# ChenWu98/cycle-diffusion

Measured on AMD Instinct MI355X. Metric: images/sec, SD-v1.4 512px CycleDiffusion 100+100 steps, 1/2/4/8 MI355X, higher is better.
Workload: dtype fp16; 1 GPU; C2: Stable-Diffusion-v1.4-shaped U-Net + KL-f8 VAE, 512x512, custom_steps=99 white_box_steps=100 eta=0.1 skip 0, 1 trial, encoder scale 1, decoder CFG 3; batch_per_gpu=4, global_batch=4, parallelism=dp1, steps_per_launch_set=5, launch_set_cap=16, launch_sets_in_flight_per_gpu=1, images_in_flight_per_gpu=20, distributed=single process, weights=synthetic(seed=0)

## Files before the change

cycle-diffusion_amd/_ffi.py:

```python
import ctypes as C
import os

import numpy as np

_HERE = os.path.dirname(os.path.abspath(__file__))
LIB_PATH = os.path.join(_HERE, "lib", "libcyclediff.so")

CD_NET_UNET_OPENAI, CD_NET_UNET_HO, CD_NET_VAE_KL, CD_NET_CLIP_TEXT, CD_NET_BERT_XTR = 1, 2, 3, 4, 5
CD_NET_OCLIP_TEXT, CD_NET_OCLIP_VISION, CD_NET_INCEPTION_FID = 6, 7, 8
CD_SCHED_DDIM, CD_SCHED_DDPM = 0, 1
CD_PREC_16, CD_PREC_F32, CD_PREC_F32X3 = 0, 1, 2
CD_MASK_QSAMPLE, CD_MASK_ENCODER = 0, 1
MASK_SOURCES = {"q_sample": CD_MASK_QSAMPLE, "encoder": CD_MASK_ENCODER}
ACT_NONE, ACT_SILU, ACT_GELU, ACT_GEGLU, ACT_QGELU, ACT_RELU = 0, 1, 2, 3, 4, 5


class NetDesc(C.Structure):
    _fields_ = [
        ("kind", C.c_int), ("image_size", C.c_int), ("in_channels", C.c_int), ("out_channels", C.c_int),
        ("model_channels", C.c_int), ("num_res_blocks", C.c_int),
        ("n_mult", C.c_int), ("channel_mult", C.c_int * 8),
        ("n_attn", C.c_int), ("attn", C.c_int * 8),
        ("num_heads", C.c_int), ("num_head_channels", C.c_int),
        ("use_spatial_transformer", C.c_int), ("context_dim", C.c_int), ("transformer_depth", C.c_int),
        ("use_scale_shift_norm", C.c_int), ("resblock_updown", C.c_int), ("conv_resample", C.c_int),
        ("z_channels", C.c_int), ("embed_dim", C.c_int), ("double_z", C.c_int),
        ("precision", C.c_int), ("n_embed", C.c_int), ("reserved", C.c_int * 6),
    ]


class StepCoef(C.Structure):
    _fields_ = [("sa", C.c_float), ("s1a", C.c_float), ("sap", C.c_float), ("dirc", C.c_float),
                ("sigma", C.c_float), ("r", C.c_float), ("t_mask", C.c_float), ("t", C.c_int32)]


STEP_COEF_DTYPE = np.dtype([("sa", "<f4"), ("s1a", "<f4"), ("sap", "<f4"), ("dirc", "<f4"), ("sigma", "<f4"),
                            ("r", "<f4"), ("t_mask", "<f4"), ("t", "<i4")])

_VP, _I, _F, _U64, _SZ, _I64 = C.c_void_p, C.c_int, C.c_float, C.c_uint64, C.c_size_t, C.c_int64

SIGNATURES = {
    "cd_last_error": [],
    "cd_version": [],
    "cd_act_format": [],
    "cd_engine_create": [_VP, _SZ, C.POINTER(_VP)],
    "cd_engine_destroy": [_VP],
    "cd_engine_synchronize": [_VP],
    "cd_engine_workspace_high_water": [_VP, C.POINTER(_SZ)],
    "cd_prof_enable": [_VP, _I],
    "cd_prof_collect": [_VP, C.POINTER(_I), C.POINTER(C.c_double), C.POINTER(C.c_double)],
    "cd_net_create": [_VP, C.POINTER(NetDesc), C.POINTER(_I)],
    "cd_net_param_count": [_VP, _I, C.POINTER(_I)],
    "cd_net_param_info": [_VP, _I, _I, C.c_char_p, _I, C.POINTER(_I), C.POINTER(_I64)],
    "cd_net_load_param": [_VP, _I, C.c_char_p, _VP, _I, C.POINTER(_I64)],
    "cd_net_missing_params": [_VP, _I, C.POINTER(_I), C.c_char_p, _I],
    "cd_unet_forward": [_VP, _I, _VP, _VP, _VP, _I, _I, _VP],
    "cd_text_encode": [_VP, _I, _VP, _I, _I, _VP],
    "cd_clip_text_features": [_VP, _I, _VP, _I, _I, _VP],
    "cd_clip_image_features": [_VP, _I, _VP, _I, _VP],
    "cd_inception_features": [_VP, _I, _VP, _I, _I, _VP],
    "cd_vae_encode": [_VP, _I, _VP, _VP, _U64, _I, _I, _I, _F, _VP],
    "cd_vae_decode": [_VP, _I, _VP, _I, _I, _F, _F, _F, _VP],
    "cd_dpm_encode": [_VP, _I, _I, _VP, _VP, _VP, _I, _F, _I, _I, _VP, _VP, _U64, _I, _VP],
    "cd_ddim_decode": [_VP, _I, _I, _VP, _I, _I, _VP, _VP, _I, _F, _I, _I, _VP, _VP, _U64, _VP],
    "cd_ddim_decode_v": [_VP, _I, _I, _VP, _I, _I, _VP, _VP, _I, _VP, _I, _I, _VP, _VP, _U64, _VP],
    "cd_ddim_invert": [_VP, _I, _I, _VP, _VP, _VP, _I, _F, _I, _I, _VP, _VP, _VP],
    "cd_cycle_translate": [_VP, _I, _I, _VP, _VP, _VP, _F, _VP, _VP, _F, _VP, _I, _I, _I, _I, _VP, _VP, _VP, _U64, _I, _VP,
                           _VP],
    "cd_ddim_decode_masked": [_VP, _I, _I, _VP, _I, _I, _VP, _VP, _I, _F, _VP, _I, _I, _VP, _VP, _U64, _VP, _VP, _I, _I, _VP, _VP,
                              _U64, _VP],
    "cd_cycle_translate_masked": [_VP, _I, _I, _VP, _VP, _VP, _F, _VP, _VP, _F, _VP, _I, _I, _I, _I, _VP, _VP, _VP, _U64, _I,
                                  _VP, _VP, _I, _I, _VP, _VP, _U64, _VP, _VP],
    "cd_cycle_translate_ctrl": [_VP, _I, _I, _VP, _VP, _VP, _F, _VP, _VP, _F, _VP, _I, _I, _I, _I, _VP, _VP, _VP, _U64, _I,
                                _VP, _VP, _I, _I, _VP, _VP, _U64, _VP, _VP, _VP, _I, _I, _VP, _VP],
    "cd_ilvr_decode": [_VP, _I, _I, _VP, _I, _I, _I, _I, _VP, _VP, _U64, _VP, _I, _I, _I, _VP, _VP, _U64, _VP],
    "cd_pix_refine": [_VP, _I, _I, _VP, _I, _I, _VP, _VP, _U64],
    "cd_op_pack_conv_weight": [_VP, _VP, _I, _I, _I, _I, _I, C.POINTER(_VP), C.POINTER(_I), C.POINTER(_I)],
    "cd_op_free": [_VP, _VP],
    "cd_op_conv2d": [_VP, _VP, _I, _VP, _I, _I, _I, _I, _VP, _I, _I, _I, _I, _I, _I, _I, _VP, _VP, _VP, _I, _I, _VP],
    "cd_op_conv2d_16": [_VP, _VP, _I, _VP, _I, _I, _I, _I, _VP, _I, _I, _I, _I, _I, _I, _I, _VP, _VP, _VP, _I, _I, _VP,
                        _VP],
    "cd_op_last_gemm_config": [_VP] + [C.POINTER(_I)] * 5,
    "cd_op_up_phase_reorder": [_VP, _VP, _I, _I, _I, _I, _VP],
    "cd_op_groupnorm": [_VP, _VP, _I, _I, _I, _I, _I, _F, _VP, _VP, _VP, _I, _VP],
    "cd_op_groupnorm_ex": [_VP, _VP, _I, _I, _VP, _I, _I, _I, _I, _I, _F, _VP, _VP, _VP, _I, _I, _VP, _VP, _I, _VP],
    "cd_op_layernorm": [_VP, _VP, _I, _I, _VP, _VP, _F, _VP],
    "cd_op_attention": [_VP, _VP, _VP, _VP, _I, _I, _I, _I, _I, _F, _I, _VP],
    "cd_op_cross_attention_ctrl": [_VP, _VP, _VP, _VP, _VP, _VP, _VP, _VP, _VP, _I, _I, _I, _I, _I, _I, _I, _I, _F, _VP],
    "cd_op_lowpass": [_VP, _VP, _I, _I, _I, _I, _VP],
    "cd_op_softmax_rows": [_VP, _VP, _I64, _I, _VP],
    "cd_op_timestep_embedding": [_VP, _VP, _I, _I, _I, _VP],
    "cd_op_sched_step": [_VP, _I, _I, _VP, _VP, _VP, _VP, _I, _F, _VP, _VP, _I, _I, _I, _I, _VP],
    "cd_op_sched_step_masked": [_VP, _I, _VP, _VP, _VP, _I, _F, _VP, _VP, _VP, _I, _I, _F, _F, _VP, _I, _I, _I, _I, _VP, _I],
    "cd_op_bench_conv": [_VP, _I, _I, _I, _I, _I, _I, _I, _I, _I, _I, _I, _I, C.POINTER(C.c_float)],
    "cd_op_bench_mfma_sustained": [_VP, _I, C.POINTER(C.c_float), C.POINTER(C.c_float)],
    "cd_op_probe": [_VP, _I, _VP, _VP, _SZ],
}
_RESTYPES = {"cd_last_error": C.c_char_p}

_lib = None


class EngineError(RuntimeError):
    pass


def load_library(build_if_missing=True):
    global _lib
    if _lib is not None:
        return _lib
    if not os.path.exists(LIB_PATH):
        if not build_if_missing:
            raise EngineError("libcyclediff.so has not been built: run `python -c 'import __graft_entry__ as g; g.build()'`")
        import importlib.util
        spec = importlib.util.spec_from_file_location("_cd_build", os.path.join(_HERE, "build.py"))
        mod = importlib.util.module_from_spec(spec)
        spec.loader.exec_module(mod)
        mod.build()
    os.environ.setdefault("CYCLEDIFF_TUNE_DEFAULT", os.path.join(_HERE, "tune_gfx950.txt"))
    lib = C.CDLL(os.environ.get("CYCLEDIFF_LIB") or LIB_PATH)
    for name, args in SIGNATURES.items():
        fn = getattr(lib, name)
        fn.argtypes = args
        fn.restype = _RESTYPES.get(name, C.c_int)
    _lib = lib
    return lib


def check(rc):
    if rc != 0:
        raise EngineError(load_library().cd_last_error().decode("utf-8", "replace"))


def ptr(t):
    if t is None:
        return None
    if not t.is_contiguous():
        raise EngineError("tensor crossing the C ABI must be contiguous")
    return C.c_void_p(t.data_ptr())


def coef_array(rows):
    arr = np.zeros(len(rows), dtype=STEP_COEF_DTYPE)
    for i, r in enumerate(rows):
        arr[i] = tuple(r)
    return arr
```

cycle-diffusion_amd/csrc/capi.hip:

```cpp
#include <stdlib.h>
#include <string.h>
#include <unistd.h>

#include <algorithm>

#include "engine.h"

using namespace cd;

struct StepPacer {
  static constexpr int kAhead = 2, kRing = kAhead + 1;
  hipEvent_t ev[kRing] = {nullptr, nullptr, nullptr};
  long n = 0;
  bool enabled = true;
  void init() {
    const char* e = getenv("CYCLEDIFF_HOST_PACING");
    enabled = !(e && e[0] == '0');
    for (auto& x : ev) HIP_CHECK(hipEventCreateWithFlags(&x, hipEventBlockingSync | hipEventDisableTiming));
  }
  static void sleep_until_done(hipEvent_t e) {
    for (;;) {
      const hipError_t q = hipEventQuery(e);
      if (q == hipSuccess) return;
      if (q != hipErrorNotReady) HIP_CHECK(q);
// ... 957 lines not shown
    const int r = R / down_n;
    iv.xp = iv.out = s.xt;
    iv.y = ref; iv.y_bmod = B_ref;
    iv.qtab = (const float2*)upload_table(h, qsample_coef_host, (size_t)K * 2 * sizeof(float));
    iv.gauss.seed = ref_seed;
    iv.B = B; iv.C = s.C; iv.R = R;
    iv.D = upload_taps(h, R, r);
    iv.U = upload_taps(h, r, R);
    iv.T = (float*)h->arena.alloc((size_t)B * s.C * r * r * sizeof(float));
    iv.xin = a.xin;
    iv.vec4 = (R % 4 == 0 && aligned16(ref) && aligned16(ref_noise)) ? 1 : 0;
  }
  HIP_CHECK(hipMemcpy2DAsync(s.xt, chw * 4, z, zbs * 4, chw * 4, B, hipMemcpyDeviceToDevice, h->st));
  if (!s.f32) launch_nchw_to_nhwc(h->st, s.xt, s.xin, B, s.C, s.HW, s.cpad, 1.f, 0.f, 0);
  for (int i = 0; i < K; ++i) {
    const int k = K - 1 - i;
    run_unet(h, s, k);
    const float* eps = (i < n_eps) ? z + (int64_t)(1 + i) * chw : nullptr;
    const float* nz = (!eps && noise_tail) ? noise_tail + (int64_t)(i - n_eps) * n : nullptr;
    a.geom.step = k; a.eps.p = eps;
    a.gauss.noise = nz; a.gauss.stream = (uint32_t)(0x1000 + i);
    launch_decode_step(h->st, sched_kind, a);
    if (k > range_t) {
      iv.qrow = k;
      iv.gauss.noise = ref_noise ? ref_noise + (int64_t)i * n : nullptr;
      iv.gauss.stream = (uint32_t)(0x5000 + i);
      launch_ilvr_down(h->st, iv);
      launch_ilvr_up_add(h->st, iv);
    }
    h->pacer.tick(h->st);
  }
  HIP_CHECK(hipMemcpyAsync(x_out, s.xt, (size_t)n * 4, hipMemcpyDeviceToDevice, h->st));
  CD_API_END
}

int cd_op_pack_conv_weight(cd_handle h, const float* w_host, int N, int Cin, int KH, int KW, int geglu,
                           void** packed_dev, int* Npad, int* Cpad) {
  CD_API_BEGIN
  enter_engine(h);
  CD_CHECK(h && w_host && packed_dev, "bad argument");
  static int counter = 0;
  ConvW* c = h->op_params.new_conv(N, Cin, KH, KW, false, geglu != 0);
  const std::string name = "op." + std::to_string(counter++);
  h->op_params.conv_weight(name, c);
  int64_t shape[4] = {N, Cin, KH, KW};
  h->op_params.load(h->st, name, w_host, 4, shape);
  *packed_dev = c;
  if (Npad) *Npad = c->Npad;
  if (Cpad) *Cpad = c->Cpad;
  CD_API_END
}

int cd_op_free(cd_handle, void*) { return 0; }

static void op_conv2d(cd_handle h, const float* x0, int C0, const float* x1, int C1, int B, int H, int W,
                      const void* packed_w, int N, int KH, int KW, int stride, int pad, int asym_pad, int up,
                      const float* bias, const float* rowvec, const float* resid, int act, int tile, bool out16,
                      float* y, float* stats) {
  CD_CHECK(h && x0 && packed_w && y, "bad argument");
  ArenaScope arena_scope(h->arena);
  Ctx c = h->ctx();
  if (up && out16) {
    ConvW* pw = (ConvW*)const_cast<void*>(packed_w);
    h->op_params.add_up_phase(pw);
    h->op_params.refresh_up_phase(h->st, pw);
  }
  ConvW w = *(const ConvW*)packed_w;
  CD_CHECK(w.N == N && w.KH == KH && w.KW == KW, "packed weight does not match the call");
  w.b = const_cast<float*>(bias);
  const int c0p = x1 ? C0 : round_up(C0, 32);
  Act a0 = alloc_act(c, B, H, W, c0p);
  launch_nchw_to_nhwc(h->st, x0, a0.p, B, C0, H * W, c0p, 1.f, 0.f, 0);
  Act a1;
  if (x1) {
    a1 = alloc_act(c, B, H, W, C1);
    launch_nchw_to_nhwc(h->st, x1, a1.p, B, C1, H * W, C1, 1.f, 0.f, 0);
  }
  ConvOpts o; o.stride = stride; o.pad = pad; o.asym = asym_pad != 0; o.up = up != 0; o.tile = tile;
  if (act & 0x400) {
    CD_CHECK(out16 && conv_ln_fold_available(c, w, (int64_t)B * H * W) , "LayerNorm fold needs tile 30 shapes");
    o.ln_fold = true;
    act &= ~0x400;
  }
  o.act = act;
  o.out_f32 = !out16;
  o.want_stats = stats != nullptr;
  const int Hin = up ? 2 * H : H, Win = up ? 2 * W : W;
  const int Ho = asym_pad ? (Hin + 1 - KH) / stride + 1 : (Hin + 2 * pad - KH) / stride + 1;
  const int Wo = asym_pad ? (Win + 1 - KW) / stride + 1 : (Win + 2 * pad - KW) / stride + 1;
  const int Nout = w.geglu ? N / 2 : N;
  if (rowvec) { o.rowvec = rowvec; o.rowvec_ld = N; o.rows_per_vec = Ho * Wo; }
  Act r;
  if (resid) {
    r = alloc_act(c, B, Ho, Wo, Nout);
    launch_nchw_to_nhwc(h->st, resid, r.p, B, Nout, Ho * Wo, Nout, 1.f, 0.f, 0);
    o.resid = &r;
  }
  Act out = conv_fwd(c, w, a0, x1 ? &a1 : nullptr, o);
  launch_nhwc_to_nchw(h->st, out.p, out16 ? 0 : 1, out.ld, y, B, Nout, Ho * Wo, 1.f, 0.f);
  if (stats) {
    CD_CHECK(out.stats, "this convolution produces no GroupNorm statistics (GEGLU, or rows %% 32 != 0)");
    HIP_CHECK(hipMemcpyAsync(stats, out.stats, (size_t)(out.rows() / 32) * 2 * Nout * sizeof(float),
                             hipMemcpyDeviceToDevice, h->st));
  }
}

int cd_op_conv2d(cd_handle h, const float* x0, int C0, const float* x1, int C1, int B, int H, int W,
                 const void* packed_w, int N, int KH, int KW, int stride, int pad, int asym_pad, int up,
                 const float* bias, const float* rowvec, const float* resid, int act, int tile, float* y) {
  CD_API_BEGIN
  enter_engine(h);
  op_conv2d(h, x0, C0, x1, C1, B, H, W, packed_w, N, KH, KW, stride, pad, asym_pad, up, bias, rowvec, resid, act, tile,
            false, y, nullptr);
  CD_API_END
}

int cd_op_conv2d_16(cd_handle h, const float* x0, int C0, const float* x1, int C1, int B, int H, int W,
                    const void* packed_w, int N, int KH, int KW, int stride, int pad, int asym_pad, int up,
                    const float* bias, const float* rowvec, const float* resid, int act, int tile, float* y,
                    float* stats) {
  CD_API_BEGIN
  enter_engine(h);
  op_conv2d(h, x0, C0, x1, C1, B, H, W, packed_w, N, KH, KW, stride, pad, asym_pad, up, bias, rowvec, resid, act, tile,
            true, y, stats);
  CD_API_END
}

int cd_op_up_phase_reorder(cd_handle h, const float* x, int B, int C, int H, int W, float* y) {
  CD_API_BEGIN
  enter_engine(h);
  CD_CHECK(h && x && y && B > 0 && H > 0 && W > 0 && C > 0 && C % 8 == 0, "bad argument");
  ArenaScope arena_scope(h->arena);
  Ctx c = h->ctx();
  Act a = alloc_act(c, 4 * B, H, W, C);
  launch_nchw_to_nhwc(h->st, x, a.p, 4 * B, C, H * W, C, 1.f, 0.f, 0);
  Act o = alloc_act(c, B, 2 * H, 2 * W, C);
  launch_up_phase_reorder(h->st, a.p, o.p, B, H, W, C, o.ld);
  launch_nhwc_to_nchw(h->st, o.p, 0, o.ld, y, B, C, 4 * H * W, 1.f, 0.f);
  CD_API_END
}

int cd_op_last_gemm_config(cd_handle h, int* tile_id, int* bk, int* splitk, int* chm, int* tile_group) {
  CD_API_BEGIN
  CD_CHECK(h, "bad argument");
  const GemmLaunchInfo li = conv_gemm_last_launch();
  if (tile_id) *tile_id = li.tile_id;
  if (bk) *bk = li.bk;
  if (splitk) *splitk = li.splitk;
  if (chm) *chm = li.chm;
  if (tile_group) *tile_group = li.tile_group;
  CD_API_END
}

int cd_op_groupnorm(cd_handle h, const float* x, int B, int C, int H, int W, int G, float eps,
                    const float* gamma, const float* beta, const float* film, int silu, float* y) {
  CD_API_BEGIN
  enter_engine(h);
  CD_CHECK(h && x && y && G == 32, "bad argument (G must be 32)");
  ArenaScope arena_scope(h->arena);
  Ctx c = h->ctx();
  Act a = alloc_act(c, B, H, W, C);
  launch_nchw_to_nhwc(h->st, x, a.p, B, C, H * W, C, 1.f, 0.f, 0);
  GNW w; w.g = const_cast<float*>(gamma); w.b = const_cast<float*>(beta); w.C = C; w.eps = eps;
  Act o = groupnorm_fwd(c, w, a, nullptr, silu != 0, film, film ? 2 * C : 0);
  launch_nhwc_to_nchw(h->st, o.p, 0, o.ld, y, B, C, H * W, 1.f, 0.f);
  CD_API_END
}

int cd_op_groupnorm_ex(cd_handle h, const float* x0, int C0, int pad0, const float* x1, int C1, int pad1, int B, int H,
                       int W, float eps, const float* gamma, const float* beta, const float* film, int film_ld, int silu,
                       const float* stats0, const float* stats1, int precision, void* y) {
  CD_API_BEGIN
  enter_engine(h);
  CD_CHECK(h && x0 && gamma && beta && y && B > 0 && H > 0 && W > 0 && C0 > 0 && pad0 >= 0 && pad1 >= 0, "bad argument");
  CD_CHECK(x1 ? C1 > 0 : (C1 == 0 && !stats1), "bad argument (second source)");
  CD_CHECK(precision >= 0 && precision <= 2 && film_ld >= 0, "bad argument (precision 0 = 16-bit, 1 = fp32, 2 = fp32 split)");
  const int align = precision ? 4 : 8;
  CD_CHECK((C0 + pad0) % align == 0 && (C1 + pad1) % align == 0, "row strides must be multiples of %d elements", align);
  ArenaScope arena_scope(h->arena);
  Ctx c = h->ctx();
  c.f32 = precision != 0; c.x3 = precision == 2;
  const int HW = H * W, C = C0 + C1;
  auto upload = [&](const float* x, int Cs, int pad, const float* stats) {
    Act a; a.B = B; a.H = H; a.W = W; a.C = Cs; a.ld = Cs + pad; a.f32 = c.f32;
    a.p = (bf16_t*)h->arena.alloc((size_t)B * HW * a.ld * (c.f32 ? sizeof(float) : sizeof(bf16_t)));
    const float* src = x;
    if (pad) {
      const size_t n = (size_t)B * a.ld * HW;
      float* t = (float*)h->arena.alloc(n * sizeof(float));
      launch_fill_f32(h->st, t, __builtin_nanf(""), (int64_t)n);
      HIP_CHECK(hipMemcpy2DAsync(t, (size_t)a.ld * HW * 4, x, (size_t)Cs * HW * 4, (size_t)Cs * HW * 4, B,
                                 hipMemcpyDeviceToDevice, h->st));
      src = t;
    }
    if (c.f32) launch_nchw_to_nhwc_f32(h->st, src, a.pf(), B, a.ld, HW, a.ld, 1.f, 0.f);
    else launch_nchw_to_nhwc(h->st, src, a.p, B, a.ld, HW, a.ld, 1.f, 0.f, 0);
    a.stats = const_cast<float*>(stats);
    return a;
  };
  Act a0 = upload(x0, C0, pad0, stats0);
  Act a1;
  if (x1) a1 = upload(x1, C1, pad1, stats1);
  GNW w; w.g = const_cast<float*>(gamma); w.b = const_cast<float*>(beta); w.C = C; w.eps = eps;
  Act o = groupnorm_fwd(c, w, a0, x1 ? &a1 : nullptr, silu != 0, film, film_ld);
  if (precision == 2) {
    CD_CHECK(o.split && o.ld == 2 * C, "groupnorm: split output expected");
    HIP_CHECK(hipMemcpyAsync(y, o.p, (size_t)B * HW * 2 * C * sizeof(bf16_t), hipMemcpyDeviceToDevice, h->st));
    HIP_CHECK(hipStreamSynchronize(h->st));
    h->check_overflow();
  } else {
    launch_nhwc_to_nchw(h->st, o.p, c.f32 ? 1 : 0, o.ld, (float*)y, B, C, HW, 1.f, 0.f);
  }
  CD_API_END
}

int cd_op_layernorm(cd_handle h, const float* x, int rows, int C, const float* gamma, const float* beta,
                    float eps, float* y) {
  CD_API_BEGIN
  enter_engine(h);
  CD_CHECK(h && x && y, "bad argument");
  ArenaScope arena_scope(h->arena);
  bf16_t* a = (bf16_t*)h->arena.alloc((size_t)rows * C * 2);
  bf16_t* o = (bf16_t*)h->arena.alloc((size_t)rows * C * 2);
  launch_nchw_to_nhwc(h->st, x, a, rows, C, 1, C, 1.f, 0.f, 0);
  launch_layernorm(h->st, a, C, o, C, rows, C, gamma, beta, eps);
  launch_nhwc_to_nchw(h->st, o, 0, C, y, rows, C, 1, 1.f, 0.f);
  CD_API_END
}

int cd_op_attention(cd_handle h, const float* q, const float* k, const float* v, int B, int H, int Tq,
                    int Tk, int D, float scale, int use_transpose_kernel, float* o) {
  CD_API_BEGIN
  enter_engine(h);
  CD_CHECK(h && q && k && v && o, "bad argument");
  ArenaScope arena_scope(h->arena);
  const int C = H * D, Tpad = round_up(Tk, 64);
  bf16_t* qb = (bf16_t*)h->arena.alloc((size_t)B * Tq * C * 2);
  bf16_t* kb = (bf16_t*)h->arena.alloc((size_t)B * Tk * C * 2);
  bf16_t* vb = (bf16_t*)h->arena.alloc((size_t)B * Tk * C * 2);
  bf16_t* ob = (bf16_t*)h->arena.alloc((size_t)B * Tq * C * 2);
  launch_nchw_to_nhwc(h->st, q, qb, B * Tq, C, 1, C, 1.f, 0.f, 0);
  launch_nchw_to_nhwc(h->st, k, kb, B * Tk, C, 1, C, 1.f, 0.f, 0);
  launch_nchw_to_nhwc(h->st, v, vb, B * Tk, C, 1, C, 1.f, 0.f, 0);
  AttnParams p;
  p.q = qb; p.k = kb; p.o = ob; p.B = B; p.H = H; p.Tq = Tq; p.Tk = Tk; p.D = D;
  p.ldq = C; p.ldk = C; p.ldo = C; p.q_bs = (int64_t)Tq * C; p.k_bs = (int64_t)Tk * C; p.o_bs = (int64_t)Tq * C;
  p.scale = scale;
  if (use_transpose_kernel) {
    bf16_t* vt = (bf16_t*)h->arena.alloc((size_t)B * C * Tpad * 2);
    launch_transpose_v(h->st, vb, C, (int64_t)Tk * C, vt, B, H, Tk, D, D, Tpad);
    p.vt = vt; p.vt_dpad = D; p.vt_tpad = Tpad;
  } else {
    p.v = vb; p.ldv = C; p.v_bs = (int64_t)Tk * C;
  }
  launch_attention(h->st, p);
  launch_nhwc_to_nchw(h->st, ob, 0, C, o, B * Tq, C, 1, 1.f, 0.f);
  CD_API_END
}

int cd_op_cross_attention_ctrl(cd_handle h, const float* q_own, const float* q_src, const float* k_own, const float* k_src,
                               const float* v_own, const float* mapper, const float* alpha, const float* weight, int B,
                               int B_src, int B_ctrl, int H, int Tq, int L, int L_buf, int D, float scale, float* o) {
  CD_API_BEGIN
  enter_engine(h);
  CD_CHECK(h && q_own && q_src && k_own && k_src && v_own && mapper && alpha && weight && o, "bad argument");
  CD_CHECK(B > 0 && B_src > 0 && B_ctrl > 0 && H > 0 && Tq > 0 && D > 0 && L > 0 && L_buf >= L, "bad argument");
  ArenaScope arena_scope(h->arena);
  const int C = H * D;
  auto to16 = [&](const float* src, int64_t rows) {
    bf16_t* d = (bf16_t*)h->arena.alloc((size_t)rows * C * 2);
    launch_nchw_to_nhwc(h->st, src, d, (int)rows, C, 1, C, 1.f, 0.f, 0);
    return d;
  };
  CtrlAttnParams p;
  p.q_own = to16(q_own, (int64_t)B * Tq); p.q_src = to16(q_src, (int64_t)B_src * Tq);
  p.k_own = to16(k_own, (int64_t)B * L_buf); p.k_src = to16(k_src, (int64_t)B_src * L_buf);
  const bf16_t* vb16 = to16(v_own, (int64_t)B * L);
  bf16_t* va = (bf16_t*)h->arena.alloc((size_t)B * L * C * 2);
  bf16_t* vb = (bf16_t*)h->arena.alloc((size_t)B * L * C * 2);
  launch_ctrl_values(h->st, vb16, mapper, alpha, weight, B, B_ctrl, L, C, va, vb);
  bf16_t* ob = (bf16_t*)h->arena.alloc((size_t)B * Tq * C * 2);
  p.va = va; p.vb = vb; p.o = ob;
  p.B = B; p.B_src = B_src; p.H = H; p.Tq = Tq; p.L = L; p.D = D;
  p.ldq = C; p.ldk = C; p.ldv = C; p.ldo = C;
  p.q_bs = (int64_t)Tq * C; p.k_bs = (int64_t)L_buf * C; p.v_bs = (int64_t)L * C; p.o_bs = (int64_t)Tq * C;
  p.scale = scale;
  launch_cross_attention_ctrl(h->st, p);
  launch_nhwc_to_nchw(h->st, ob, 0, C, o, B * Tq, C, 1, 1.f, 0.f);
  CD_API_END
}

int cd_op_lowpass(cd_handle h, const float* x, int B, int C, int R, int down_n, float* y) {
  CD_API_BEGIN
  enter_engine(h);
  CD_CHECK(h && x && y && B > 0 && C > 0 && R > 0, "bad argument");
  check_lowpass_geometry(R, down_n);
  ArenaScope arena_scope(h->arena);
  const int r = R / down_n;
  IlvrArgs iv;
  iv.out = y; iv.y = x; iv.y_bmod = B;
  iv.B = B; iv.C = C; iv.R = R;
  iv.D = upload_taps(h, R, r);
  iv.U = upload_taps(h, r, R);
  iv.T = (float*)h->arena.alloc((size_t)B * C * r * r * sizeof(float));
  iv.vec4 = (R % 4 == 0 && aligned16(x) && aligned16(y)) ? 1 : 0;
  launch_ilvr_down(h->st, iv);
// ... 255 lines not shown
```

cycle-diffusion_amd/csrc/conv_gemm.hip:

```cpp
#include <stdio.h>
#include <stdlib.h>
#include <string.h>

#include <algorithm>
#include <map>
#include <mutex>
#include <string>

#include "common.h"
#include "kernels.h"

namespace cd {

namespace gemm_detail {

#ifndef CD_EPI_STORE_AUX
#define CD_EPI_STORE_AUX 0
#endif
#ifndef CD_EPI_RESID_AUX
#define CD_EPI_RESID_AUX 0
#endif

typedef const __attribute__((address_space(1))) void* gptr_t;
typedef __attribute__((address_space(3))) void* lptr_t;

template <int BM, int BN, int BK, int WM, int WN, int NSTAGE>
struct TileCfg {
  static constexpr int NW = WM * WN;
  static constexpr int CPR = BK / 8;
  static constexpr int RPI = 64 / CPR;
  static constexpr int A_IPW = BM / RPI / NW;
  static constexpr int B_IPW = BN / RPI / NW;
  static constexpr int LPT = A_IPW + B_IPW;
  static constexpr int TM = BM / WM, TN = BN / WN;
  static constexpr int MT = TM / 32, NT = TN / 32;
  static constexpr int KS = BK / 16;
  static constexpr int SWZ_SHIFT = (CPR == 8) ? 1 : 2;
  static constexpr int CW = TN >= 64 ? 64 : TN;
  static constexpr int EPI_LD = CW + 4;
  static constexpr int PF = (MT * NT >= 8) ? 1 : 2;
  static constexpr int A_BYTES = BM * BK * 2, B_BYTES = BN * BK * 2;
  static constexpr int STAGE_BYTES = A_BYTES + B_BYTES;
  static constexpr int EPI_BYTES = NW * TM * EPI_LD * 4;
  static constexpr int LDS_BYTES = STAGE_BYTES * NSTAGE > EPI_BYTES ? STAGE_BYTES * NSTAGE : EPI_BYTES;
  static constexpr int TAB_BIAS_I = (BN / 4 + 63) / 64;
  static constexpr int TAB_RV_I = ((BM / 32) * (BN / 4) + 63) / 64;
  static constexpr bool HAS_TAB = LDS_BYTES + (TAB_BIAS_I + TAB_RV_I) * 1024 <= 160 * 1024;
  static constexpr int TAB_BYTES = HAS_TAB ? (TAB_BIAS_I + TAB_RV_I) * 1024 : 0;
  static_assert(NW == 4 || NW == 8 || NW == 16, "4, 8 or 16 waves");
  static_assert(A_IPW >= 1 && B_IPW >= 1, "tile too small for the wave count");
  static_assert(A_IPW * RPI * NW == BM && B_IPW * RPI * NW == BN, "tile rows must split evenly over waves");
  static_assert(MT >= 1 && NT >= 1, "wave tile");
  static_assert(NSTAGE >= 2 && NSTAGE <= 8, "ring depth");
  static_assert((NSTAGE - 2) * LPT <= 63, "vmcnt field");
  static_assert(LDS_BYTES + TAB_BYTES <= 160 * 1024, "LDS");
};

template <int N>
__device__ __forceinline__ void wait_vmcnt_barrier() {
  asm volatile("s_waitcnt vmcnt(%0)\n\ts_barrier" ::"n"(N) : "memory");
}

#ifdef CD_PROBE
__device__ __forceinline__ unsigned long long probe_time() {
  unsigned long long t;
  asm volatile("s_memtime %0\n\ts_waitcnt lgkmcnt(0)" : "=s"(t)::"memory");
  return t;
}
__device__ __forceinline__ unsigned long long probe_realtime() {
  unsigned long long t;
  asm volatile("s_memrealtime %0\n\ts_waitcnt lgkmcnt(0)" : "=s"(t)::"memory");
  return t;
}
#define CD_PROBE_ONLY(...) __VA_ARGS__
#else
#define CD_PROBE_ONLY(...)
#endif

__device__ __forceinline__ __amdgpu_buffer_rsrc_t uniform_rsrc(const void* base, int bytes) {
  const uint64_t u = (uint64_t)base;
  const uint32_t lo = (uint32_t)__builtin_amdgcn_readfirstlane((int)(uint32_t)u);
  const uint32_t hi = (uint32_t)__builtin_amdgcn_readfirstlane((int)(uint32_t)(u >> 32));
  return __builtin_amdgcn_make_buffer_rsrc((void*)(((uint64_t)hi << 32) | lo), 0, __builtin_amdgcn_readfirstlane(bytes), 0x00020000);
}

__device__ __forceinline__ bool fast_epilogue(const ConvGemmParams& p) {
  return p.act == ACT_NONE && !p.out_f32 && !p.resid_f32 && (p.N & 7) == 0 && (p.out_ld & 7) == 0 &&
         (((uintptr_t)p.out | (uintptr_t)p.resid | (uintptr_t)p.rowvec) & 15) == 0 && (p.o_bs & 7) == 0 &&
         (!p.resid || (p.resid_ld & 7) == 0) &&
         (!p.rowvec || ((p.rowvec_ld & 3) == 0 && (p.rows_per_vec >= p.M || (p.rows_per_vec & 31) == 0)));
}

template <int BM, int BN, int BK, int WM, int WN, int NSTAGE, bool CHM = false>
__global__ __launch_bounds__(64 * WM * WN, (WM * WN == 4 && BK == 32 && NSTAGE == 3 && BM * BN >= 128 * 256) ? 2 : 1) void k_conv_gemm(ConvGemmParams p) {
#if defined(__HIP_DEVICE_COMPILE__)
  using T = TileCfg<BM, BN, BK, WM, WN, NSTAGE>;
  constexpr int CPR = T::CPR, RPI = T::RPI, A_IPW = T::A_IPW, B_IPW = T::B_IPW, NW = T::NW;
  constexpr int MT = T::MT, NT = T::NT, KS = T::KS, TM = T::TM, TN = T::TN, LPT = T::LPT;
  extern __shared__ __attribute__((aligned(16))) char smem[];

  const int tid = threadIdx.x;
  const int lane = tid & 63;
  const int wave = __builtin_amdgcn_readfirstlane(tid >> 6);
  const int wm = wave / WN, wn = wave % WN;
  if constexpr (WM * WN == 4 && BK == 32 && NSTAGE == 3 && BM * BN >= 128 * 256) {
    if (p.dephase_ticks > 0 && (int)(blockIdx.x + gridDim.x * (blockIdx.y + gridDim.y * blockIdx.z)) < 2 * p.num_cus) {
      unsigned hwid;
      asm volatile("s_getreg_b32 %0, hwreg(HW_REG_HW_ID)" : "=s"(hwid));
      if (tid == 0) *(volatile int*)smem = (int)(hwid & 1u);
      __syncthreads();
      const int odd = *(volatile int*)smem;
      __syncthreads();
      if (odd) {
        unsigned long long t0, t1;
        asm volatile("s_memtime %0\n\ts_waitcnt lgkmcnt(0)" : "=s"(t0)::"memory");
        do {
          __builtin_amdgcn_s_sleep(32);
          asm volatile("s_memtime %0\n\ts_waitcnt lgkmcnt(0)" : "=s"(t1)::"memory");
        } while ((long long)(t1 - t0) < (long long)p.dephase_ticks);
      }
    }
  }
  CD_PROBE_ONLY(
  const unsigned long long pr_rt0 = probe_realtime();
  unsigned long long pr_t0 = probe_time(), pr_prol = 0, pr_first = 0, pr_wait = 0, pr_comp = 0, pr_maxw = 0, pr_loop = 0,
                     pr_drain = 0, pr_stage = 0, pr_rows = 0, pr_issued = 0, pr_last = 0;
  unsigned* pr_log = (unsigned*)(smem + T::LDS_BYTES + T::TAB_BYTES) + wave * 64;
  if (lane < 64) pr_log[lane] = 0;)

  const int tiles_n = (p.N + BN - 1) / BN;
  const int tiles_m = (p.M + BM - 1) / BM;
  const int ntiles = tiles_m * tiles_n;
  int tile;
  {
    const int bid = blockIdx.x;
    const int q = ntiles >> 3, r = ntiles & 7;
    const int xcd = bid & 7, loc = bid >> 3;
    tile = (xcd < r ? xcd * (q + 1) : r * (q + 1) + (xcd - r) * q) + loc;
  }
  const bool nmajor = (int64_t)p.N * p.Ktot > (int64_t)p.B * p.Hs * p.Ws * (p.C0 + p.C1);
  int tm, tn;
  if (p.tile_group > 0) {
    const int width = p.tile_group * tiles_n;
    const int grp = tile / width, within = tile - grp * width;
    const int first_m = grp * p.tile_group;
    const int gsz = (tiles_m - first_m) < p.tile_group ? (tiles_m - first_m) : p.tile_group;
    tn = within / gsz; tm = first_m + (within - tn * gsz);
  } else if (nmajor) { tn = tile / tiles_m; tm = tile - tn * tiles_m; }
  else { tm = tile / tiles_n; tn = tile - tm * tiles_n; }
  const int m0 = tm * BM, n0 = tn * BN;
  const int zb = blockIdx.z;

  constexpr unsigned kRange = 0x7fffffffu, kInvalid = 0x80000000u;
  const int HWo = p.Hout * p.Wout;
  const bool pow2 = ((HWo & (HWo - 1)) == 0) && ((p.Wout & (p.Wout - 1)) == 0);
  const int sh_hw = 31 - __builtin_clz(HWo), sh_w = 31 - __builtin_clz(p.Wout);
  int b_first = pow2 ? (m0 >> sh_hw) : (m0 / HWo);
  CD_PROBE_ONLY(if (p.dbg & 4) b_first = 0;)
  int pad_t = p.pad_t, pad_l = p.pad_l, w_ph = 0;
  if (p.up_phase) {
    const int ph = b_first & 3;
    b_first >>= 2;
    pad_t = 1 - (ph >> 1); pad_l = 1 - (ph & 1);
    w_ph = ph * p.w_ps;
  }
  const int64_t samp0 = (int64_t)b_first * p.Hs * p.Ws;
  const bf16_t* base0 = p.src0 + (int64_t)zb * p.a_bs + samp0 * p.ld0;
  const bf16_t* base1 = p.src1 ? p.src1 + (int64_t)zb * p.a_bs + samp0 * p.ld1 : base0;
  const __amdgpu_buffer_rsrc_t rsw =
      __builtin_amdgcn_make_buffer_rsrc((void*)(p.wgt + (int64_t)zb * p.w_bs + w_ph), 0, kRange, 0x00020000);

  const int srow = lane / CPR;
  const int pchunk = lane % CPR;
  int a_iy0[A_IPW], a_ix0[A_IPW], a_boff[A_IPW], a_lc8[A_IPW];
  unsigned a_voff[A_IPW];
  unsigned a_mk[A_IPW], a_base[A_IPW];
#pragma unroll
  for (int i = 0; i < A_IPW; ++i) {
    const int row = (i * NW + wave) * RPI + srow;
    int m = m0 + row;
    CD_PROBE_ONLY(if (p.dbg & 4) m = (m0 & 0x3ff) + row;)
    a_lc8[i] = (pchunk ^ ((row >> T::SWZ_SHIFT) & (CPR - 1))) * 8;
    a_voff[i] = kInvalid;
    a_mk[i] = 0; a_base[i] = 0;
    if (m < p.M) {
      int b, oy, ox;
      if (pow2) {
        b = m >> sh_hw;
        const int rem = m & (HWo - 1);
        oy = rem >> sh_w; ox = rem & (p.Wout - 1);
      } else {
        b = m / HWo;
        const int rem = m - b * HWo;
        oy = rem / p.Wout; ox = rem - oy * p.Wout;
      }
      if (p.up_phase) b >>= 2;
      a_iy0[i] = oy * p.stride - pad_t;
      a_ix0[i] = ox * p.stride - pad_l;
      a_boff[i] = (b - b_first) * p.Hs * p.Ws;
    } else {
      a_iy0[i] = -(1 << 28);
      a_ix0[i] = 0;
      a_boff[i] = 0;
    }
    if constexpr (CHM) {
      unsigned mk = 0;
      for (int r = 0; r < p.KH; ++r) mk |= ((unsigned)(a_iy0[i] + r) < (unsigned)p.Hin ? 1u : 0u) << r;
      for (int q = 0; q < p.KW; ++q) mk |= ((unsigned)(a_ix0[i] + q) < (unsigned)p.Win ? 1u : 0u) << (8 + q);
      a_mk[i] = mk;
    }
  }
  unsigned b_voff[B_IPW];
#pragma unroll
  for (int i = 0; i < B_IPW; ++i) {
    const int row = (i * NW + wave) * RPI + srow;
    const int lchunk = pchunk ^ ((row >> T::SWZ_SHIFT) & (CPR - 1));
    int nrow = n0 + row;
    if (nrow >= p.N) nrow = p.N - 1;
    b_voff[i] = (unsigned)((nrow * (p.ldw ? p.ldw : p.Ktot) + lchunk * 8) * 2);
  }

  const int Ctot = p.C0 + p.C1;
  const int nk = p.Ktot / BK;
  const int nsplit = gridDim.y, sidx = blockIdx.y;
  const int kper = (nk + nsplit - 1) / nsplit;
  const int kt0 = sidx * kper;
  const int kt1 = (kt0 + kper < nk) ? kt0 + kper : nk;
  int kr, kss, kc;
  if constexpr (CHM) {
    const int ntaps = p.KH * p.KW;
    const int slice = kt0 / ntaps, tap = kt0 - slice * ntaps;
    kc = slice * BK;
    kr = tap / p.KW;
    kss = tap - kr * p.KW;
  } else {
    const int k_el = kt0 * BK;
    const int tap = k_el / Ctot;
    kc = k_el - tap * Ctot;
    kr = tap / p.KW;
    kss = tap - kr * p.KW;
  }
  bool st_force = true;

  char* As = smem;
  char* Bs = smem + NSTAGE * T::A_BYTES;

  bool st_live = false;
  int st_soffa = 0, st_soffb = 0;
  const bf16_t* st_base = base0;
  auto prepare = [&](int kt) {
    st_live = kt < kt1;
    const int c_kc = kc, c_kr = kr, c_kss = kss;
    if constexpr (CHM) {
      const bool wk = c_kss + 1 >= p.KW;
      const bool wr = wk && (c_kr + 1 >= p.KH);
      kss = wk ? 0 : c_kss + 1;
      kr = wr ? 0 : c_kr + (wk ? 1 : 0);
      kc = c_kc + (wr ? BK : 0);
      if (st_live) {
        const int ld = (c_kc < p.C0) ? p.ld0 : p.ld1;
        if (st_force || ((c_kr | c_kss) == 0 && (c_kc == 0 || c_kc == p.C0))) {
          st_force = false;
#pragma unroll
          for (int i = 0; i < A_IPW; ++i) {
            const int pix = a_boff[i] + a_iy0[i] * p.Ws + a_ix0[i];
            a_base[i] = (unsigned)((pix * ld + a_lc8[i]) * 2);
          }
        }
        const unsigned dt = (unsigned)((c_kr * p.Ws + c_kss) * ld * 2);
#pragma unroll
        for (int i = 0; i < A_IPW; ++i) {
          const unsigned ok = (a_mk[i] >> c_kr) & (a_mk[i] >> (8 + c_kss)) & 1u;
          a_voff[i] = ok ? a_base[i] + dt : kInvalid;
        }
      }
    } else {
      kc += BK;
      if (kc >= Ctot) {
        kc = 0;
        if (++kss >= p.KW) { kss = 0; ++kr; }
      }
      if (st_live && (c_kc == 0 || c_kc == p.C0 || st_force)) {
        st_force = false;
        const int ld = (c_kc < p.C0) ? p.ld0 : p.ld1;
#pragma unroll
        for (int i = 0; i < A_IPW; ++i) {
          int iy = a_iy0[i] + c_kr, ix = a_ix0[i] + c_kss;
          const bool ok = ((unsigned)iy < (unsigned)p.Hin) && ((unsigned)ix < (unsigned)p.Win);
          if (p.up) { iy >>= 1; ix >>= 1; }
          const int pix = a_boff[i] + iy * p.Ws + ix;
          a_voff[i] = ok ? (unsigned)((pix * ld + a_lc8[i]) * 2) : kInvalid;
        }
      }
    }
    const bool first = c_kc < p.C0;
    st_base = first ? base0 : base1;
    st_soffa = (first ? c_kc : c_kc - p.C0) * 2;
    st_soffb = st_live ? (CHM ? ((c_kr * p.KW + c_kss) * Ctot + c_kc) * 2 : kt * (BK * 2)) : 0;
  };
  auto issue = [&](int idx, int buf) {
    if (idx < A_IPW) {
      const __amdgpu_buffer_rsrc_t rsa = __builtin_amdgcn_make_buffer_rsrc((void*)st_base, 0, kRange, 0x00020000);
      char* l = As + buf * T::A_BYTES + ((idx * NW + wave) * RPI) * (BK * 2);
      __builtin_amdgcn_raw_ptr_buffer_load_lds(rsa, (lptr_t)l, 16, st_live ? a_voff[idx < A_IPW ? idx : 0] : kInvalid,
                                               st_soffa, 0, 0);
    } else {
      const int i = idx - A_IPW;
      char* l = Bs + buf * T::B_BYTES + ((i * NW + wave) * RPI) * (BK * 2);
      __builtin_amdgcn_raw_ptr_buffer_load_lds(rsw, (lptr_t)l, 16, st_live ? b_voff[i < B_IPW ? i : 0] : kInvalid,
                                               st_soffb, 0, 0);
    }
  };

  f32x16 acc[MT][NT];
#pragma unroll
  for (int i = 0; i < MT; ++i)
#pragma unroll
    for (int j = 0; j < NT; ++j)
#pragma unroll
      for (int r = 0; r < 16; ++r) acc[i][j][r] = 0.0f;

  const int frow = lane & 31;
  const int fhalf = lane >> 5;

  constexpr int PF = T::PF, SYNC = KS - PF, NMF = MT * NT, HALF = NMF / 2;
  constexpr int SPREAD = (NSTAGE == 2) ? 1 : KS;
  static_assert(SYNC >= 0 && (NSTAGE - 1) * LPT <= 63, "fragment prefetch depth / vmcnt field");
#pragma unroll
  for (int s = 0; s < NSTAGE; ++s) {
    prepare(kt0 + s);
#pragma unroll
    for (int l = 0; l < LPT; ++l) issue(l, s);
  }
  constexpr int TAB_N = T::TAB_BIAS_I + T::TAB_RV_I;
  constexpr int TABI = T::HAS_TAB ? (TAB_N + NW - 1) / NW : 0;
  if constexpr (TABI > 0) {
    const bool fe = fast_epilogue(p);
    const bool tb = (fe || p.act == ACT_GEGLU) && p.bias != nullptr;
    char* tab = smem + T::LDS_BYTES;
    const __amdgpu_buffer_rsrc_t rsb = __builtin_amdgcn_make_buffer_rsrc(
        (void*)(tb ? (const void*)p.bias : (const void*)p.wgt), 0, tb ? p.N * 4 : 0, 0x00020000);
    const __amdgpu_buffer_rsrc_t rsv = __builtin_amdgcn_make_buffer_rsrc(
        (void*)((fe && p.rowvec) ? (const void*)p.rowvec : (const void*)p.wgt), 0, (fe && p.rowvec) ? kRange : 0, 0x00020000);
    const unsigned rpv = (unsigned)p.rows_per_vec;
    const bool rpv_pow2 = (rpv & (rpv - 1)) == 0;
    const int rpv_sh = 31 - __builtin_clz(rpv | 1u);
#pragma unroll
    for (int i = 0; i < TABI; ++i) {
      const int j = (i * NW + wave) % TAB_N;
// ... 3 lines not shown
      } else {
        const int c = (j - T::TAB_BIAS_I) * 64 + lane;
        const int blk = c / (BN / 4), c4 = c - blk * (BN / 4);
        const int m = m0 + blk * 32, nn = n0 + c4 * 4;
        int rvi = 0;
        if (p.rows_per_vec < p.M) rvi = rpv_pow2 ? (int)((unsigned)m >> rpv_sh) : m / p.rows_per_vec;
        const unsigned vo = (m < p.M && nn < p.N) ? (unsigned)((rvi * p.rowvec_ld + nn) * 4) : kInvalid;
        __builtin_amdgcn_raw_ptr_buffer_load_lds(rsv, (lptr_t)(tab + j * 1024), 16, vo, 0, 0, 0);
      }
    }
  }
  CD_PROBE_ONLY(pr_prol = probe_time(); pr_last = pr_prol;)
  static_assert((NSTAGE - 1) * LPT + TABI <= 63, "vmcnt field");
  wait_vmcnt_barrier<(NSTAGE - 1) * LPT + TABI>();
  CD_PROBE_ONLY(pr_first = probe_time(); pr_last = pr_first;)

  bf16x8 af[KS][MT], bfr[KS][NT];
  auto read_frags = [&](int slot, int ks) {
    const char* Ab = As + slot * T::A_BYTES;
    const char* Bb = Bs + slot * T::B_BYTES;
#pragma unroll
    for (int i = 0; i < MT; ++i) {
      const int row = wm * TM + i * 32 + frow;
      const int ch = (ks * 2 + fhalf) ^ ((row >> T::SWZ_SHIFT) & (CPR - 1));
      af[ks][i] = *(const bf16x8*)(Ab + row * (BK * 2) + ch * 16);
    }
#pragma unroll
    for (int j = 0; j < NT; ++j) {
      const int row = wn * TN + j * 32 + frow;
      const int ch = (ks * 2 + fhalf) ^ ((row >> T::SWZ_SHIFT) & (CPR - 1));
      bfr[ks][j] = *(const bf16x8*)(Bb + row * (BK * 2) + ch * 16);
    }
  };
#pragma unroll
  for (int q = 0; q < PF; ++q) read_frags(0, q);
  __builtin_amdgcn_sched_barrier(0);

  int cur = 0;
  int fill = 0;
  for (int kt = kt0; kt < kt1; ++kt) {
    const int nslot = (cur + 1 == NSTAGE) ? 0 : cur + 1;
#pragma unroll
    for (int ks = 0; ks < KS; ++ks) {
      const int jrel = (ks - SYNC + KS) % KS;
      auto mfma_range = [&](int lo, int hi) __attribute__((always_inline)) {
#pragma unroll
        for (int n = 0; n < NMF; ++n)
          if (n >= lo && n < hi) acc[n / NT][n % NT] = CD_MFMA_32x32x16(af[ks][n / NT], bfr[ks][n % NT], acc[n / NT][n % NT]);
      };
      if (ks == SYNC) {
        mfma_range(0, HALF);
        CD_PROBE_ONLY(const unsigned long long pr_arr = probe_time();)
        asm volatile("s_waitcnt vmcnt(%0) lgkmcnt(0)\n\ts_barrier" ::"n"((NSTAGE - 2) * LPT) : "memory");
        CD_PROBE_ONLY({
          const unsigned long long now = probe_time();
          pr_comp += pr_arr - pr_last; pr_wait += now - pr_arr; if (now - pr_arr > pr_maxw) pr_maxw = now - pr_arr;
          if (kt - kt0 < 32 && lane == 0) { pr_log[2 * (kt - kt0)] = (unsigned)(pr_arr - pr_t0); pr_log[2 * (kt - kt0) + 1] = (unsigned)(now - pr_t0); }
          pr_last = now;
        })
        prepare(kt + NSTAGE);
        fill = cur;
#pragma unroll
        for (int l = 0; l < LPT / SPREAD; ++l) issue(l, fill);
        mfma_range(HALF, NMF);
      } else {
        if (SPREAD > 1 && (ks > SYNC || kt != kt0)) {
#pragma unroll
          for (int l = (jrel * LPT) / SPREAD; l < ((jrel + 1) * LPT) / SPREAD; ++l) issue(l, fill);
        }
        mfma_range(0, NMF);
      }
      if (ks + PF < KS) read_frags(cur, ks + PF);
      else read_frags(nslot, ks + PF - KS);
      __builtin_amdgcn_sched_barrier(0);
    }
    cur = nslot;
  }
  CD_PROBE_ONLY(pr_loop = probe_time(); pr_comp += pr_loop - pr_last;)
  asm volatile("s_waitcnt vmcnt(0)" ::: "memory");
  __syncthreads();
  CD_PROBE_ONLY(pr_drain = probe_time();)

  if (nsplit > 1) {
    constexpr int TILE_BYTES = BM * BN * 4;
    constexpr int kSc1 = 16;
    typedef __attribute__((ext_vector_type(4))) unsigned int u32x4;
    float* part0 = p.sk_scratch + ((int64_t)zb * ntiles + tile) * nsplit * (BM * BN);
    const __amdgpu_buffer_rsrc_t rsp = __builtin_amdgcn_make_buffer_rsrc((void*)part0, 0, kRange, 0x00020000);
#pragma unroll
    for (int i = 0; i < MT; ++i)
#pragma unroll
      for (int j = 0; j < NT; ++j)
#pragma unroll
        for (int q = 0; q < 4; ++q) {
          const f32x4 v = {acc[i][j][4 * q], acc[i][j][4 * q + 1], acc[i][j][4 * q + 2], acc[i][j][4 * q + 3]};
          const int off = sidx * TILE_BYTES + (((i * NT + j) * 4 + q) * (64 * NW) + tid) * 16;
          __builtin_amdgcn_raw_buffer_store_b128(__builtin_bit_cast(u32x4, v), rsp, off, 0, kSc1);
        }
    asm volatile("s_waitcnt vmcnt(0)" ::: "memory");
    __syncthreads();
    int* flag = p.sk_flags + zb * ntiles + tile;
    if (tid == 0) *(volatile int*)smem = __hip_atomic_fetch_add(flag, 1, __ATOMIC_RELAXED, __HIP_MEMORY_SCOPE_AGENT);
    __syncthreads();
    const int arrived = *(volatile int*)smem;
    __syncthreads();
    if (arrived != nsplit - 1) return;
    if (tid == 0) __hip_atomic_store(flag, 0, __ATOMIC_RELAXED, __HIP_MEMORY_SCOPE_AGENT);
#pragma unroll
    for (int i = 0; i < MT; ++i)
#pragma unroll
      for (int j = 0; j < NT; ++j)
#pragma unroll
        for (int r = 0; r < 16; ++r) acc[i][j][r] = 0.0f;
    for (int sp = 0; sp < nsplit; ++sp) {
#pragma unroll
      for (int i = 0; i < MT; ++i)
#pragma unroll
        for (int j = 0; j < NT; ++j)
#pragma unroll
          for (int q = 0; q < 4; ++q) {
            const int off = sp * TILE_BYTES + (((i * NT + j) * 4 + q) * (64 * NW) + tid) * 16;
            const f32x4 v = __builtin_bit_cast(f32x4, __builtin_amdgcn_raw_buffer_load_b128(rsp, off, 0, kSc1));
            acc[i][j][4 * q] += v[0]; acc[i][j][4 * q + 1] += v[1];
            acc[i][j][4 * q + 2] += v[2]; acc[i][j][4 * q + 3] += v[3];
            if (q == 3 && MT * NT >= 8) __builtin_amdgcn_sched_barrier(0);
          }
    }
  }

  constexpr int CW = T::CW, CJ = CW / 32;
  int lane_ep = lane;
  asm volatile("" : "+v"(lane_ep));
  float* E = (float*)smem + wave * (TM * T::EPI_LD);
  const bool geglu = (p.act == ACT_GEGLU);
  char* outp = (char*)p.out + (int64_t)zb * p.o_bs * (p.out_f32 ? 4 : 2);
  if (p.alpha != 1.0f) {
#pragma unroll
    for (int i = 0; i < MT; ++i)
#pragma unroll
      for (int j = 0; j < NT; ++j)
#pragma unroll
        for (int r = 0; r < 16; ++r) acc[i][j][r] *= p.alpha;
  }
  if (T::HAS_TAB && fast_epilogue(p)) {
    constexpr int LD = T::EPI_LD, NRB = TM / 32;
    typedef __attribute__((ext_vector_type(4))) unsigned int u32x4e;
    const int mw = m0 + wm * TM;
    const bool has_res = p.resid != nullptr;
    int rows_ok = p.M - mw;
    rows_ok = rows_ok < 0 ? 0 : (rows_ok > TM ? TM : rows_ok);
    const int nblk = (p.M + 31) >> 5;
    int blk_ok = nblk - (mw >> 5);
    blk_ok = blk_ok < 0 ? 0 : (blk_ok > NRB ? NRB : blk_ok);
    const __amdgpu_buffer_rsrc_t rs_o = uniform_rsrc(outp + (int64_t)mw * p.out_ld * 2, rows_ok * p.out_ld * 2);
    const __amdgpu_buffer_rsrc_t rs_r =
        uniform_rsrc(has_res ? (const void*)(p.resid + (int64_t)zb * p.o_bs + (int64_t)mw * p.resid_ld) : (const void*)outp,
                     has_res ? rows_ok * p.resid_ld * 2 : 0);
    const __amdgpu_buffer_rsrc_t rs_s =
        uniform_rsrc(p.stats ? (const void*)(p.stats + ((int64_t)zb * nblk + (mw >> 5)) * 2 * p.N) : (const void*)outp,
                     p.stats ? blk_ok * 2 * p.N * 4 : 0);
    const float* TB = (const float*)(smem + T::LDS_BYTES) + wn * TN;
    const float* TR = (const float*)(smem + T::LDS_BYTES) + T::TAB_BIAS_I * 256 + (wm * NRB) * BN + wn * TN;
    constexpr bool PIPE = NW <= 8;
    u32x4e rq[PIPE ? 2 : 1][4];
    auto resid_issue = [&](int jcx, int rbx, u32x4e (&dst)[4]) __attribute__((always_inline)) {
      const int cwx = ((NT - jcx) < CJ ? (NT - jcx) : CJ) * 32, vprx = cwx / 8, rppx = 64 / vprx, npx = 32 / rppx;
      const int nx = n0 + wn * TN + jcx * 32 + (lane_ep % vprx) * 8;
      const unsigned vo = nx < p.N ? (unsigned)(((rbx * 32 + lane_ep / vprx) * p.resid_ld + nx) * 2) : kInvalid;
#pragma unroll
      for (int ps = 0; ps < 4; ++ps)
        if (ps < npx) dst[ps] = __builtin_amdgcn_raw_buffer_load_b128(rs_r, vo + (unsigned)(ps * rppx * p.resid_ld * 2), 0, CD_EPI_RESID_AUX);
    };
    if constexpr (PIPE) resid_issue(0, 0, rq[0]);
#pragma unroll
    for (int jc = 0; jc < NT; jc += CJ) {
      const int cj = (NT - jc) < CJ ? (NT - jc) : CJ;
      const int cw = cj * 32;
      const int RPP = 64 / (cw / 8), NP = 32 / RPP;
      const int vr = lane_ep / (cw / 8), col = (lane_ep % (cw / 8)) * 8;
      const int n = n0 + wn * TN + jc * 32 + col;
      CD_PROBE_ONLY(const unsigned long long pr_c0 = probe_time();)
      __builtin_amdgcn_wave_barrier();
#pragma unroll
      for (int i = 0; i < MT; ++i)
#pragma unroll
        for (int j = 0; j < CJ; ++j)
          if (j < cj) {
#pragma unroll
            for (int r = 0; r < 16; ++r) {
              const int row = i * 32 + (r & 3) + 8 * (r >> 2) + 4 * fhalf;
              E[row * LD + j * 32 + frow] = acc[i][jc + j][r];
            }
          }
      __builtin_amdgcn_wave_barrier();
      CD_PROBE_ONLY(const unsigned long long pr_c1 = probe_time(); pr_stage += pr_c1 - pr_c0;)
      const f32x4 b0 = *(const f32x4*)(TB + jc * 32 + col), b1 = *(const f32x4*)(TB + jc * 32 + col + 4);
      const unsigned vo_out = n < p.N ? (unsigned)((vr * p.out_ld + n) * 2) : kInvalid;
#pragma unroll
      for (int rb = 0; rb < NRB; ++rb) {
        const int kb = (jc / CJ) * NRB + rb;
        const int mb = mw + rb * 32;
        if constexpr (!PIPE) resid_issue(jc, rb, rq[0]);
        else if (rb + 1 < NRB) resid_issue(jc, rb + 1, rq[(kb + 1) & 1]);
        else if (jc + CJ < NT) resid_issue(jc + CJ, 0, rq[(kb + 1) & 1]);
        __builtin_amdgcn_sched_barrier(0);
        f32x4 lo[4], hi[4];
#pragma unroll
        for (int ps = 0; ps < 4; ++ps)
          if (ps < NP) {
            const float* er = E + (rb * 32 + ps * RPP + vr) * LD + col;
            lo[ps] = *(const f32x4*)er;
            hi[ps] = *(const f32x4*)(er + 4);
          }
        const f32x4 a0 = b0 + *(const f32x4*)(TR + rb * BN + jc * 32 + col);
        const f32x4 a1 = b1 + *(const f32x4*)(TR + rb * BN + jc * 32 + col + 4);
        constexpr bool KEEP = NW <= 8;
        float v[KEEP ? 4 : 1][8];
        float ssum[8], ssq[8];
#pragma unroll
        for (int e = 0; e < 8; ++e) { ssum[e] = 0.f; ssq[e] = 0.f; }
        const unsigned vo_blk = vo_out + (unsigned)(rb * 32 * p.out_ld * 2);
#pragma unroll
        for (int ps = 0; ps < 4; ++ps)
          if (ps < NP) {
            float* vp = v[KEEP ? ps : 0];
#pragma unroll
            for (int e = 0; e < 4; ++e) { vp[e] = lo[ps][e] + a0[e]; vp[4 + e] = hi[ps][e] + a1[e]; }
            if (has_res) {
              float rf[8];
              const u32x4e w = rq[PIPE ? (kb & 1) : 0][ps];
              unpack8(make_uint4(w[0], w[1], w[2], w[3]), rf);
#pragma unroll
              for (int e = 0; e < 8; ++e) vp[e] += rf[e];
            }
            const uint4 pk = pack8(vp);
            CD_PROBE_ONLY(if (!(p.dbg & 1)))
            __builtin_amdgcn_raw_buffer_store_b128((u32x4e){pk.x, pk.y, pk.z, pk.w}, rs_o,
                                                   vo_blk + (unsigned)(ps * RPP * p.out_ld * 2), 0, CD_EPI_STORE_AUX);
            if constexpr (!KEEP) {
              const float on = (mb + ps * RPP + vr) < p.M ? 1.0f : 0.0f;
#pragma unroll
              for (int e = 0; e < 8; ++e) { const float x = on * vp[e]; ssum[e] += x; ssq[e] += x * x; }
            }
          }
        float s_sum = 0.f, s_sq = 0.f;
        if (p.stats) {
          if constexpr (KEEP) {
            if (mb + 32 <= p.M) {
#pragma unroll
              for (int ps = 0; ps < 4; ++ps)
                if (ps < NP) {
#pragma unroll
                  for (int e = 0; e < 8; ++e) { ssum[e] += v[ps][e]; ssq[e] += v[ps][e] * v[ps][e]; }
                }
            } else {
#pragma unroll
              for (int ps = 0; ps < 4; ++ps)
                if (ps < NP) {
                  const float on = (mb + ps * RPP + vr) < p.M ? 1.0f : 0.0f;
#pragma unroll
                  for (int e = 0; e < 8; ++e) { const float x = on * v[ps][e]; ssum[e] += x; ssq[e] += x * x; }
                }
            }
          }
          float* S = E + rb * 32 * LD;
          __builtin_amdgcn_wave_barrier();
          *(f32x4*)(S + vr * cw + col) = (f32x4){ssum[0], ssum[1], ssum[2], ssum[3]};
          *(f32x4*)(S + vr * cw + col + 4) = (f32x4){ssum[4], ssum[5], ssum[6], ssum[7]};
          *(f32x4*)(S + 512 + vr * cw + col) = (f32x4){ssq[0], ssq[1], ssq[2], ssq[3]};
          *(f32x4*)(S + 512 + vr * cw + col + 4) = (f32x4){ssq[4], ssq[5], ssq[6], ssq[7]};
          __builtin_amdgcn_wave_barrier();
          if (cw == 64) {
#pragma unroll
            for (int k = 0; k < 8; ++k) { s_sum += S[k * 64 + lane_ep]; s_sq += S[512 + k * 64 + lane_ep]; }
          } else {
            const int arr = lane_ep >> 5, c = lane_ep & 31;
#pragma unroll
            for (int k = 0; k < 16; ++k) s_sum += S[arr * 512 + k * 32 + c];
          }
          __builtin_amdgcn_wave_barrier();
        }
        {
          const int nc0 = n0 + wn * TN + jc * 32;
          if (cw == 64) {
            const unsigned so = nc0 + lane_ep < p.N ? (unsigned)((rb * 2 * p.N + nc0 + lane_ep) * 4) : kInvalid;
            __builtin_amdgcn_raw_buffer_store_b32(__builtin_bit_cast(unsigned, s_sum), rs_s, so, 0, 0);
            __builtin_amdgcn_raw_buffer_store_b32(__builtin_bit_cast(unsigned, s_sq), rs_s, so + (unsigned)(p.N * 4), 0, 0);
          } else {
            const int arr = lane_ep >> 5, c = lane_ep & 31;
            const unsigned so = nc0 + c < p.N ? (unsigned)((rb * 2 * p.N + arr * p.N + nc0 + c) * 4) : kInvalid;
            __builtin_amdgcn_raw_buffer_store_b32(__builtin_bit_cast(unsigned, s_sum), rs_s, so, 0, 0);
          }
        }
      }
      CD_PROBE_ONLY(pr_rows += probe_time() - pr_c1;)
    }
  } else {
#pragma unroll
    for (int jc = 0; jc < NT; jc += CJ) {
      const int cj = (NT - jc) < CJ ? (NT - jc) : CJ;
      const int cw = cj * 32;
      CD_PROBE_ONLY(const unsigned long long pr_c0 = probe_time();)
      __builtin_amdgcn_wave_barrier();
#pragma unroll
      for (int i = 0; i < MT; ++i)
#pragma unroll
        for (int j = 0; j < CJ; ++j)
          if (j < cj) {
#pragma unroll
            for (int r = 0; r < 16; ++r) {
              const int row = i * 32 + (r & 3) + 8 * (r >> 2) + 4 * fhalf;
              E[row * T::EPI_LD + j * 32 + frow] = acc[i][jc + j][r];
            }
          }
      __builtin_amdgcn_wave_barrier();
      CD_PROBE_ONLY(const unsigned long long pr_c1 = probe_time(); pr_stage += pr_c1 - pr_c0;)
      const int vpr = geglu ? 4 : (cw / 8);
      const int rpp = 64 / vpr;
      int lane_g = lane_ep;
      asm volatile("" : "+v"(lane_g));
      const int vr = lane_g / vpr, vc = lane_g % vpr;
      const int col = vc * 8;
      const int n = n0 + wn * TN + jc * 32 + col;
      const int nvalid = (p.N - n) < 8 ? (p.N - n) : 8;
      if (geglu && cw == 64 && !p.out_f32 && !p.resid && !p.stats && !p.rowvec && (p.N & 63) == 0 && (p.out_ld & 7) == 0 &&
          (((uintptr_t)p.out) & 15) == 0 && (p.o_bs & 7) == 0) {
        constexpr int LD = T::EPI_LD;
        typedef __attribute__((ext_vector_type(4))) unsigned int u32x4e;
        float bias_v[8], bias_g[8];
        if constexpr (T::HAS_TAB) {
          const float* tb = (const float*)(smem + T::LDS_BYTES) + wn * TN + jc * 32 + col;
          const f32x4 x0 = *(const f32x4*)tb, x1 = *(const f32x4*)(tb + 4), g0 = *(const f32x4*)(tb + 32), g1 = *(const f32x4*)(tb + 36);
#pragma unroll
          for (int e = 0; e < 4; ++e) { bias_v[e] = x0[e]; bias_v[4 + e] = x1[e]; bias_g[e] = g0[e]; bias_g[4 + e] = g1[e]; }
        } else {
#pragma unroll
          for (int e = 0; e < 8; ++e) { bias_v[e] = p.bias ? p.bias[n + e] : 0.0f; bias_g[e] = p.bias ? p.bias[n + 32 + e] : 0.0f; }
        }
        const int mw = m0 + wm * TM;
        int rows_ok = p.M - mw;
        rows_ok = rows_ok < 0 ? 0 : (rows_ok > TM ? TM : rows_ok);
        const __amdgpu_buffer_rsrc_t rs_o = uniform_rsrc(outp + (int64_t)mw * p.out_ld * 2, rows_ok * p.out_ld * 2);
        const unsigned vo_out = n < p.N ? (unsigned)((vr * p.out_ld + (n / 64) * 32 + (n % 64)) * 2) : kInvalid;
#pragma unroll
        for (int rb = 0; rb < TM / 32; ++rb) {
          f32x4 vl[2], vh[2], gl[2], gh[2];
#pragma unroll
          for (int ps = 0; ps < 2; ++ps) {
            const float* er = E + (rb * 32 + ps * 16 + vr) * LD + col;
            vl[ps] = *(const f32x4*)er;        vh[ps] = *(const f32x4*)(er + 4);
            gl[ps] = *(const f32x4*)(er + 32); gh[ps] = *(const f32x4*)(er + 36);
          }
#pragma unroll
          for (int ps = 0; ps < 2; ++ps) {
            float v[8], va[8], ga[8];
#pragma unroll
            for (int e = 0; e < 4; ++e) {
              va[e] = vl[ps][e] + bias_v[e]; va[4 + e] = vh[ps][e] + bias_v[4 + e];
              ga[e] = gl[ps][e] + bias_g[e]; ga[4 + e] = gh[ps][e] + bias_g[4 + e];
            }
            mul_gelu8(va, ga, v);
            const uint4 pk = pack8(v);
            CD_PROBE_ONLY(if (!(p.dbg & 1)))
            __builtin_amdgcn_raw_buffer_store_b128((u32x4e){pk.x, pk.y, pk.z, pk.w}, rs_o,
                                                   vo_out + (unsigned)((rb * 32 + ps * 16) * p.out_ld * 2), 0, 0);
          }
        }
        CD_PROBE_ONLY(pr_rows += probe_time() - pr_c1;)
        continue;
      }
      float bias_v[8];
#pragma unroll
      for (int e = 0; e < 8; ++e) bias_v[e] = (p.bias && e < nvalid) ? p.bias[n + e] : 0.0f;
      float ssum[8], ssq[8];
#pragma unroll
      for (int e = 0; e < 8; ++e) { ssum[e] = 0.f; ssq[e] = 0.f; }
      for (int r0 = 0; r0 < TM; r0 += rpp) {
        const int row = r0 + vr;
        const int m = m0 + wm * TM + row;
        if (row < TM && m < p.M && n < p.N) {
        float v[8];
        {
          const f32x4 lo = *(const f32x4*)(E + row * T::EPI_LD + col);
          const f32x4 hi = *(const f32x4*)(E + row * T::EPI_LD + col + 4);
          v[0] = lo[0]; v[1] = lo[1]; v[2] = lo[2]; v[3] = lo[3];
          v[4] = hi[0]; v[5] = hi[1]; v[6] = hi[2]; v[7] = hi[3];
        }
#pragma unroll
        for (int e = 0; e < 8; ++e) v[e] += bias_v[e];
        int on = n;
        if (geglu) {
          float gt[8];
          const f32x4 lo = *(const f32x4*)(E + row * T::EPI_LD + col + 32);
          const f32x4 hi = *(const f32x4*)(E + row * T::EPI_LD + col + 36);
          gt[0] = lo[0]; gt[1] = lo[1]; gt[2] = lo[2]; gt[3] = lo[3];
          gt[4] = hi[0]; gt[5] = hi[1]; gt[6] = hi[2]; gt[7] = hi[3];
#pragma unroll
          for (int e = 0; e < 8; ++e) {
            const float gg = gt[e] + (p.bias ? p.bias[n + 32 + e] : 0.0f);
            v[e] = v[e] * gelu_fast(gg);
          }
          on = (n / 64) * 32 + (n % 64);
        } else {
          if (p.rowvec) {
            const int rvi = (p.rows_per_vec >= p.M) ? 0 : m / p.rows_per_vec;
            const float* rv = p.rowvec + (int64_t)rvi * p.rowvec_ld + n;
#pragma unroll
            for (int e = 0; e < 8; ++e) if (e < nvalid) v[e] += rv[e];
          }
          if (p.act == ACT_SILU) {
#pragma unroll
            for (int e = 0; e < 8; ++e) v[e] = silu_f(v[e]);
          } else if (p.act == ACT_GELU) {
#pragma unroll
            for (int e = 0; e < 8; ++e) {
              v[e] = gelu_fast(v[e]);
              if constexpr (NW == 16) {
                if (e == 3) asm volatile("" : "+v"(v[0]), "+v"(v[1]), "+v"(v[2]), "+v"(v[3]), "+v"(v[4]), "+v"(v[5]), "+v"(v[6]), "+v"(v[7]));
              }
            }
          } else if (p.act == ACT_QGELU) {
#pragma unroll
            for (int e = 0; e < 8; ++e) v[e] = v[e] / (1.0f + __expf(-1.702f * v[e]));
          } else if (p.act == ACT_RELU) {
#pragma unroll
            for (int e = 0; e < 8; ++e) v[e] = fmaxf(v[e], 0.0f);
          }
        }
        if (p.resid && p.resid_f32) {
          const float* rp = (const float*)p.resid + (int64_t)zb * p.o_bs + (int64_t)m * p.resid_ld + on;
          if (nvalid == 8 && ((p.resid_ld & 3) == 0)) {
            const f32x4 r0 = *(const f32x4*)rp, r1 = *(const f32x4*)(rp + 4);
#pragma unroll
            for (int e = 0; e < 4; ++e) { v[e] += r0[e]; v[4 + e] += r1[e]; }
          } else {
#pragma unroll
            for (int e = 0; e < 8; ++e) if (e < nvalid) v[e] += rp[e];
          }
        } else if (p.resid) {
          const bf16_t* rp = p.resid + (int64_t)zb * p.o_bs + (int64_t)m * p.resid_ld + on;
          if (nvalid == 8 && ((p.resid_ld & 7) == 0)) {
            float rr[8];
            unpack8(*(const uint4*)rp, rr);
#pragma unroll
            for (int e = 0; e < 8; ++e) v[e] += rr[e];
          } else {
#pragma unroll
            for (int e = 0; e < 8; ++e) if (e < nvalid) v[e] += bf2f(rp[e]);
          }
        }
        CD_PROBE_ONLY(if (!(p.dbg & 1)))
        if (p.out_f32) {
          float* op = (float*)outp + (int64_t)m * p.out_ld + on;
          if (nvalid == 8 && ((p.out_ld & 3) == 0)) {
            *(f32x4*)op = (f32x4){v[0], v[1], v[2], v[3]};
            *(f32x4*)(op + 4) = (f32x4){v[4], v[5], v[6], v[7]};
          } else {
#pragma unroll
            for (int e = 0; e < 8; ++e) if (e < nvalid) op[e] = v[e];
          }
        } else {
          bf16_t* op = (bf16_t*)outp + (int64_t)m * p.out_ld + on;
          if (nvalid == 8 && ((p.out_ld & 7) == 0)) {
            *(uint4*)op = pack8(v);
          } else {
#pragma unroll
            for (int e = 0; e < 8; ++e) if (e < nvalid) op[e] = f2bf(v[e]);
          }
        }
        CD_PROBE_ONLY(if (p.dbg & 1) { if (v[0] == 1.2345e-33f) ((float*)outp)[0] = v[1] + v[2] + v[3] + v[4] + v[5] + v[6] + v[7]; })
        if (p.stats) {
#pragma unroll
          for (int e = 0; e < 8; ++e) { ssum[e] += v[e]; ssq[e] += v[e] * v[e]; }
        }
        }
        if (p.stats && ((r0 + rpp) & 31) == 0) {
          for (int o = vpr; o < 64; o <<= 1) {
#pragma unroll
            for (int e = 0; e < 8; ++e) { ssum[e] += __shfl_xor(ssum[e], o); ssq[e] += __shfl_xor(ssq[e], o); }
          }
          const int rb = (m0 + wm * TM + r0 + rpp - 32) >> 5;
          if (vr == 0 && n < p.N && (rb << 5) < p.M) {
            float* sp = p.stats + ((int64_t)zb * ((p.M + 31) >> 5) + rb) * 2 * p.N + n;
#pragma unroll
            for (int e = 0; e < 8; ++e) if (e < nvalid) { sp[e] = ssum[e]; sp[p.N + e] = ssq[e]; }
          }
#pragma unroll
          for (int e = 0; e < 8; ++e) { ssum[e] = 0.f; ssq[e] = 0.f; }
        }
      }
      CD_PROBE_ONLY(pr_rows += probe_time() - pr_c1;)
    }
  }
  CD_PROBE_ONLY({
    pr_issued = probe_time();
    asm volatile("s_waitcnt vmcnt(0)" ::: "memory");
    const unsigned long long pr_done = probe_time();
    if (p.probe) {
      unsigned hwid, xcc;
      asm volatile("s_getreg_b32 %0, hwreg(HW_REG_HW_ID)" : "=s"(hwid));
      asm volatile("s_getreg_b32 %0, hwreg(HW_REG_XCC_ID)" : "=s"(xcc));
      unsigned long long* o = p.probe + ((size_t)(blockIdx.x + gridDim.x * (blockIdx.y + gridDim.y * blockIdx.z)) * NW + wave) * kProbeWords;
      if (lane == 0) {
        o[0] = pr_t0; o[1] = pr_prol; o[2] = pr_first; o[3] = pr_wait; o[4] = pr_comp; o[5] = pr_maxw; o[6] = pr_loop;
        o[7] = pr_drain; o[8] = pr_stage; o[9] = pr_rows; o[10] = pr_issued; o[11] = pr_done; o[12] = kt1 - kt0;
        o[13] = ((unsigned long long)xcc << 32) | hwid; o[14] = pr_rt0; o[15] = probe_realtime();
      }
      ((unsigned*)(o + 16))[lane] = pr_log[lane];
    }
  })
#endif
}


inline bool takes_channel_major(const ConvGemmParams& p) {
  const int64_t a_bytes = (int64_t)p.B * p.Hs * p.Ws * (p.C0 + p.C1) * 2;
  return p.korder != 0 && p.KH * p.KW > 1 && p.KH <= 8 && p.KW <= 8 && !p.up && !p.up_phase &&
         (p.korder == 2 || (p.Hs * p.Ws >= 4096 && a_bytes >= (32ll << 20)));
}

template <int BM, int BN, int BK, int WM, int WN, int NSTAGE>
int launch_cfg(hipStream_t st, const ConvGemmParams& p) {
  using T = TileCfg<BM, BN, BK, WM, WN, NSTAGE>;
  const int tiles = ceil_div(p.M, BM) * ceil_div(p.N, BN);
  const int split = p.splitk > 1 ? p.splitk : 1;
#ifdef CD_PROBE
  constexpr int kLds = T::LDS_BYTES + T::TAB_BYTES + T::NW * 256;
#else
  constexpr int kLds = T::LDS_BYTES + T::TAB_BYTES;
#endif
  const bool chm = takes_channel_major(p);
  static PerDeviceOnce attr_once;
  auto kern0 = k_conv_gemm<BM, BN, BK, WM, WN, NSTAGE, false>;
  auto kern1 = k_conv_gemm<BM, BN, BK, WM, WN, NSTAGE, true>;
  attr_once([&]() {
    HIP_CHECK(hipFuncSetAttribute((const void*)kern0, hipFuncAttributeMaxDynamicSharedMemorySize, kLds));
    HIP_CHECK(hipFuncSetAttribute((const void*)kern1, hipFuncAttributeMaxDynamicSharedMemorySize, kLds));
  });
  auto kern = chm ? kern1 : kern0;
  if (split > 1) {
    const SplitKWorkspace& ws = g_conv_splitk;
    CD_CHECK(p.sk_scratch && p.sk_flags, "conv_gemm: split-K without workspace");
    CD_CHECK((size_t)tiles * p.nbatch * split * BM * BN * 4 <= ws.scratch_bytes && tiles * p.nbatch <= ws.nflags,
             "conv_gemm: split-K workspace too small");
  }
  hipLaunchKernelGGL(kern, dim3(tiles, split, p.nbatch), dim3(64 * T::NW), kLds, st, p);
  return 0;
}

struct CfgInfo { int id, BM, BN, TN; const char* name; };
const CfgInfo kCfgs[] = {
    {1, 128, 128, 64, "128x128 w2x2 s2"},
    {2, 128, 64, 64, "128x64 w4x1 s2"},
    {3, 64, 64, 32, "64x64 w2x2 s2"},
    {4, 128, 128, 64, "128x128 w2x2 s3"},
    {5, 256, 128, 64, "256x128 w4x2 s3"},
    {6, 128, 256, 64, "128x256 w2x4 s3"},
    {7, 128, 64, 64, "128x64 w4x1 s4"},
    {8, 64, 64, 32, "64x64 w2x2 s4"},
    {9, 256, 64, 64, "256x64 w8x1 s4"},
    {10, 128, 128, 64, "128x128 w2x2 s4"},
    {11, 64, 128, 64, "64x128 w2x2 s4"},
    {12, 128, 64, 64, "128x64 w4x1 s3"},
    {13, 256, 64, 64, "256x64 w8x1 s3"},
    {14, 128, 128, 64, "128x128 w4x2 s3"},
    {15, 64, 64, 32, "64x64 w2x2 s8"},
    {16, 128, 64, 64, "128x64 w4x1 s6"},
    {17, 64, 128, 64, "64x128 w2x2 s6"},
    {18, 256, 128, 32, "256x128 w4x4 s3"},
    {19, 256, 128, 64, "256x128 w8x2 s3"},
    {20, 256, 320, 160, "256x320 w4x2 s2"},
    {21, 128, 320, 160, "128x320 w2x2 s2"},
    {22, 256, 256, 128, "256x256 w4x2 s2"},
    {23, 128, 320, 160, "128x320 w4x2 s2"},
    {24, 128, 256, 128, "128x256 w2x2 s3 bk32 x2/CU"},
    {25, 256, 128, 128, "256x128 w4x1 s3 bk32 x2/CU"},
};
inline bool cfg_needs_bk64(int id) { return id == 20 || id == 21 || id == 23; }
constexpr int kNumCfgs = sizeof(kCfgs) / sizeof(kCfgs[0]);
inline int bk32_alias(int id) { return id == 9 ? 7 : id == 13 ? 12 : id == 18 ? 5 : id == 19 ? 5 : id; }
inline bool cfg_always_bk32(int id) { return id == 24 || id == 25; }

}
thread_local SplitKWorkspace g_conv_splitk;
thread_local unsigned long long* g_conv_probe = nullptr;
namespace gemm_detail {

template <int BK>
int dispatch(hipStream_t st, const ConvGemmParams& p, int id) {
  switch (id) {
    case 1: return launch_cfg<128, 128, BK, 2, 2, 2>(st, p);
    case 2: return launch_cfg<128, 64, BK, 4, 1, 2>(st, p);
    case 3: return launch_cfg<64, 64, BK, 2, 2, 2>(st, p);
    case 4: return launch_cfg<128, 128, BK, 2, 2, 3>(st, p);
    case 5: return launch_cfg<256, 128, BK, 4, 2, 3>(st, p);
    case 6: return launch_cfg<128, 256, BK, 2, 4, 3>(st, p);
    case 7: return launch_cfg<128, 64, BK, 4, 1, 4>(st, p);
    case 8: return launch_cfg<64, 64, BK, 2, 2, 4>(st, p);
    case 9:
      if constexpr (BK == 64) return launch_cfg<256, 64, 64, 8, 1, 4>(st, p);
      else return launch_cfg<128, 64, 32, 4, 1, 4>(st, p);
     
    case 10: return launch_cfg<128, 128, BK, 2, 2, 4>(st, p);
    case 11: return launch_cfg<64, 128, BK, 2, 2, 4>(st, p);
    case 12: return launch_cfg<128, 64, BK, 4, 1, 3>(st, p);
    case 13:
      if constexpr (BK == 64) return launch_cfg<256, 64, 64, 8, 1, 3>(st, p);
      else return launch_cfg<128, 64, 32, 4, 1, 3>(st, p);
     
    case 14: return launch_cfg<128, 128, BK, 4, 2, 3>(st, p);
    case 15: return launch_cfg<64, 64, BK, 2, 2, 8>(st, p);
    case 16: return launch_cfg<128, 64, BK, 4, 1, 6>(st, p);
    case 17: return launch_cfg<64, 128, BK, 2, 2, 6>(st, p);
    case 18:
      if constexpr (BK == 64) return launch_cfg<256, 128, 64, 4, 4, 3>(st, p);
      else return launch_cfg<256, 128, 32, 4, 2, 3>(st, p);
     
    case 19:
      if constexpr (BK == 64) return launch_cfg<256, 128, 64, 8, 2, 3>(st, p);
      else return launch_cfg<256, 128, 32, 4, 2, 3>(st, p);
     
    case 20: case 21: case 22: case 23:
      if constexpr (BK == 64) {
        if (id == 20) return launch_cfg<256, 320, 64, 4, 2, 2>(st, p);
        else if (id == 21) return launch_cfg<128, 320, 64, 2, 2, 2>(st, p);
        else if (id == 22) return launch_cfg<256, 256, 64, 4, 2, 2>(st, p);
        else return launch_cfg<128, 320, 64, 4, 2, 2>(st, p);
      } else {
        if (id == 22) return launch_cfg<256, 256, 32, 4, 2, 4>(st, p);
        CD_CHECK(false, "conv_gemm: tile configuration %d needs channel counts that are multiples of 64", id);
      }
      return 0;
    case 24: return launch_cfg<128, 256, 32, 2, 2, 3>(st, p);
    case 25: return launch_cfg<256, 128, 32, 4, 1, 3>(st, p);
    default: CD_CHECK(false, "conv_gemm: unknown tile configuration %d", id);
  }
  return 0;
}

thread_local const char* g_last_cfg = "";
thread_local GemmLaunchInfo g_last_launch;

int device_cu_count() {
  static std::atomic<int> ncu_of[64];
  int dev = 0;
  if (hipGetDevice(&dev) != hipSuccess) return 256;
  int n = ncu_of[dev & 63].load(std::memory_order_relaxed);
  if (!n) {
    hipDeviceProp_t prop;
    n = (hipGetDeviceProperties(&prop, dev) == hipSuccess && prop.multiProcessorCount > 0) ? prop.multiProcessorCount : 256;
    ncu_of[dev & 63].store(n, std::memory_order_relaxed);
  }
  return n;
}

int pick_config(const ConvGemmParams& p) {
  const int64_t ncu = device_cu_count();
  const int64_t t128 = (int64_t)ceil_div(p.M, 128) * ceil_div(p.N, 128) * p.nbatch;
  const int64_t t12864 = (int64_t)ceil_div(p.M, 128) * ceil_div(p.N, 64) * p.nbatch;
  if (p.act == ACT_GEGLU) return (2 * t128 >= 3 * ncu) ? 1 : 2;
  if (2 * t128 >= 3 * ncu && p.N % 128 == 0) return 1;
  if (t128 >= 2 * ncu) return 1;
  if (t12864 >= ncu) return 2;
  return 3;
}

}
using namespace gemm_detail;

const char* conv_gemm_last_config() { return g_last_cfg; }
GemmLaunchInfo conv_gemm_last_launch() { return g_last_launch; }

thread_local KernelProfiler* g_conv_prof = nullptr;

void KernelProfiler::next_pair(hipEvent_t* a, hipEvent_t* b, double fl, const std::string& what) {
  labels.push_back(what);
  if (used + 2 > (int)events.size()) {
    const size_t old = events.size();
    events.resize(old + 1024);
    for (size_t i = old; i < events.size(); ++i) HIP_CHECK(hipEventCreate(&events[i]));
  }
  *a = events[used]; *b = events[used + 1];
  used += 2;
  flops.push_back(fl);
}
void KernelProfiler::collect(int* launches, double* total_ms, double* total_flops) {
  double ms = 0, fl = 0;
  for (int i = 0; i + 1 < used; i += 2) {
    HIP_CHECK(hipEventSynchronize(events[i + 1]));
    float t = 0;
    HIP_CHECK(hipEventElapsedTime(&t, events[i], events[i + 1]));
    ms += t; fl += flops[i / 2];
    if (verbose) {
      auto& e = per_shape[labels[i / 2]];
      e.n += 1; e.ms += t; e.flops += flops[i / 2];
    }
  }
  if (verbose) {
    std::vector<std::pair<std::string, Entry>> v(per_shape.begin(), per_shape.end());
    std::sort(v.begin(), v.end(), [](const auto& x, const auto& y) { return x.second.ms > y.second.ms; });
    fprintf(stderr, "[conv_gemm] %d launches %.3f ms %.1f TFLOP/s\n", used / 2, ms, fl / ms * 1e-9);
    for (auto& kv : v)
      fprintf(stderr, "  %-58s n=%4d %8.3f ms %7.1f us/launch %7.1f TF/s\n", kv.first.c_str(), kv.second.n,
              kv.second.ms, kv.second.ms / kv.second.n * 1e3, kv.second.flops / kv.second.ms * 1e-9);
    per_shape.clear();
  }
  *launches = used / 2; *total_ms = ms; *total_flops = fl;
  used = 0; flops.clear(); labels.clear();
}
KernelProfiler::~KernelProfiler() { for (auto e : events) (void)hipEventDestroy(e); }

ConvTuner g_conv_tuner;

namespace {
struct ShapeKey {
  int v[14];
  bool operator<(const ShapeKey& o) const { return memcmp(v, o.v, sizeof(v)) < 0; }
};
const char* tune_cache_path() {
  static const char* p = getenv("CYCLEDIFF_TUNE_CACHE");
  return (p && p[0]) ? p : nullptr;
}
std::map<ShapeKey, int>& tune_table() {
  static std::map<ShapeKey, int> t;
  static bool loaded = false;
  if (!loaded) {
    loaded = true;
    const char* paths[2] = {getenv("CYCLEDIFF_TUNE_DEFAULT"), tune_cache_path()};
    for (const char* path : paths) {
      if (!path || !path[0]) continue;
      if (FILE* f = fopen(path, "r")) {
        ShapeKey k; int val;
        for (;;) {
          int got = 0;
          for (int i = 0; i < 14; ++i) got += fscanf(f, "%d", &k.v[i]);
          got += fscanf(f, "%d", &val);
          if (got != 15) break;
          t[k] = val;
        }
        fclose(f);
      }
    }
  }
  return t;
}
void tune_cache_append(const ShapeKey& k, int val) {
  const char* path = tune_cache_path();
  if (!path) return;
  if (FILE* f = fopen(path, "a")) {
    for (int i = 0; i < 14; ++i) fprintf(f, "%d ", k.v[i]);
    fprintf(f, "%d\n", val);
    fclose(f);
  }
}

std::mutex g_tune_mu;

int tuned_config(hipStream_t st, const ConvGemmParams& p, bool k64) {
  std::lock_guard<std::mutex> lock(g_tune_mu);
  ConvTuner& tu = g_conv_tuner;
  if (!tu.enabled || !tu.scratch) return pick_config(p);
  const int nout = (p.act == ACT_GEGLU) ? p.N / 2 : p.N;
  const size_t need = (size_t)p.M * nout * (p.out_f32 ? 4 : 2) * p.nbatch;
  if (need > tu.scratch_bytes) return pick_config(p);
  ShapeKey key = {{p.M, p.N, p.Ktot, p.KH, p.C0, p.C1, p.stride, p.up | (p.up_phase << 1), p.act, p.nbatch, p.out_f32, p.Hout, p.Wout,
                   (p.resid ? 1 : 0) | (p.rowvec ? 2 : 0)}};
  auto& tab = tune_table();
  auto it = tab.find(key);
  if (it != tab.end()) return it->second;
  ConvGemmParams q = p;
  q.out = tu.scratch; q.out_ld = nout; q.o_bs = (int64_t)p.M * nout;
  if (p.resid && p.nbatch > 1) q.resid = nullptr;
  hipEvent_t e0, e1;
  HIP_CHECK(hipEventCreate(&e0)); HIP_CHECK(hipEventCreate(&e1));
  int best = pick_config(p);
  float best_ms = 1e30f;
  const SplitKWorkspace& sk = g_conv_splitk;
  const int64_t t128 = (int64_t)ceil_div(p.M, 128) * ceil_div(p.N, 128) * p.nbatch;
  const int nk = p.Ktot / (k64 ? 64 : 32);
  static const int kSplits[] = {1, 2, 3, 4, 6, 8, 12, 16};
  static const bool tune_splitk = [] { const char* e = getenv("CYCLEDIFF_TUNE_SPLITK"); return e && e[0] == '1'; }();
  const int nbk = (k64 && p.Ktot <= 1280) ? 2 : 1;
  for (int bi = 0; bi < nbk; ++bi)
  for (int i = 0; i < kNumCfgs; ++i)
  for (int si = 0; si < 8; ++si) {
    const CfgInfo& c = kCfgs[i];
    const int split = kSplits[si];
    const bool use64 = k64 && bi == 0;
    if (bi == 1 && split > 1) continue;
    if (split > 1 && !tune_splitk) continue;
    if (p.act == ACT_GEGLU && (c.TN % 64) != 0) continue;
    if (c.BM >= 256 && p.M < 256) continue;
    if (cfg_needs_bk64(c.id) && !use64) continue;
    if ((c.id == 24 || c.id == 25) && bi == 1) continue;
    if (c.BN == 320 && (p.N % 320) != 0) continue;
    const int64_t tiles = (int64_t)ceil_div(p.M, c.BM) * ceil_div(p.N, c.BN) * p.nbatch;
    if (split > 1) {
      if (!sk.scratch || tiles >= device_cu_count() || nk < 4 * split || tiles * split > 2048) continue;
      if ((size_t)tiles * split * c.BM * c.BN * 4 > sk.scratch_bytes || tiles > sk.nflags) continue;
    }
    q.splitk = split; q.sk_scratch = sk.scratch; q.sk_flags = sk.flags;
    auto run = [&]() { if (use64) dispatch<64>(st, q, c.id); else dispatch<32>(st, q, c.id); };
    auto timed = [&](int reps) {
      HIP_CHECK(hipEventRecord(e0, st));
      for (int r = 0; r < reps; ++r) run();
      HIP_CHECK(hipEventRecord(e1, st));
      HIP_CHECK(hipEventSynchronize(e1));
      float t = 0;
      HIP_CHECK(hipEventElapsedTime(&t, e0, e1));
      return t / reps;
    };
    run();
    float ms = timed(2);
    const int reps = (int)fminf(24.f, fmaxf(2.f, 0.4f / fmaxf(ms, 1e-3f)));
    ms = fminf(ms, fminf(timed(reps), timed(reps)));
    if (ms < best_ms) { best_ms = ms; best = c.id | (split << 8) | ((k64 && !use64) ? (1 << 16) : 0); }
  }
  if (lin_stream_supports(q)) {
    auto timed = [&](int reps) {
      HIP_CHECK(hipEventRecord(e0, st));
      for (int r = 0; r < reps; ++r) launch_lin_stream(st, q);
      HIP_CHECK(hipEventRecord(e1, st));
      HIP_CHECK(hipEventSynchronize(e1));
      float t = 0;
      HIP_CHECK(hipEventElapsedTime(&t, e0, e1));
      return t / reps;
    };
    q.splitk = 0;
    launch_lin_stream(st, q);
    float ms = timed(2);
    const int reps = (int)fminf(24.f, fmaxf(2.f, 0.4f / fmaxf(ms, 1e-3f)));
    ms = fminf(ms, fminf(timed(reps), timed(reps)));
    if (ms < best_ms) { best_ms = ms; best = kLinStreamTile; }
  }
  (void)hipEventDestroy(e0); (void)hipEventDestroy(e1);
  tab[key] = best;
  tune_cache_append(key, best);
  ++tu.shapes_tuned;
  return best;
}
}

void launch_conv_gemm(hipStream_t st, const ConvGemmParams& p) {
  const int Ctot = p.C0 + p.C1;
  CD_CHECK(p.C0 % 32 == 0 && p.C1 % 32 == 0, "conv_gemm: channels must be multiples of 32 (C0=%d C1=%d)", p.C0, p.C1);
  CD_CHECK(p.Ktot == p.KH * p.KW * Ctot, "conv_gemm: Ktot mismatch");
  CD_CHECK(p.zeros != nullptr, "conv_gemm: zero page missing");
  CD_CHECK(p.M > 0 && p.N > 0, "conv_gemm: empty problem");
  CD_CHECK(((uintptr_t)p.src0 & 15) == 0 && ((uintptr_t)p.wgt & 15) == 0, "conv_gemm: 16-B alignment");
  CD_CHECK((p.ld0 % 8) == 0 && (p.src1 == nullptr || (p.ld1 % 8) == 0), "conv_gemm: ld must be a multiple of 8");
  if (p.act == ACT_GEGLU) CD_CHECK(p.N % 64 == 0, "GEGLU needs packed N %% 64 == 0");
  if (p.up_phase)
    CD_CHECK(p.KH == 2 && p.KW == 2 && p.stride == 1 && !p.up && !p.src1 && p.nbatch == 1 && p.Hout == p.Hs && p.Wout == p.Ws &&
                 (p.Hs * p.Ws) % 256 == 0 && p.M == 4 * p.B * p.Hs * p.Ws && p.w_ps > 0 && p.Hin == p.Hs && p.Win == p.Ws,
             "conv_gemm: phase form of an x2 conv on %d x %d", p.Hs, p.Ws);
  bool k64 = (p.C0 % 64 == 0) && (p.C1 % 64 == 0);
  if (p.ln_fold) CD_CHECK(p.tile == kLinStreamTile, "conv_gemm: a LayerNorm-folded layer runs on lin_stream only");
  int id = p.tile ? p.tile : tuned_config(st, p, k64);
  if (id & (1 << 16)) k64 = false;
  ConvGemmParams pk = p;
  id &= 0xffff;
  if ((id >> 8) > 1) pk.splitk = id >> 8;
  id &= 0xff;
  if (pk.splitk > 1 && !pk.sk_scratch) { pk.sk_scratch = g_conv_splitk.scratch; pk.sk_flags = g_conv_splitk.flags; }
  pk.probe = g_conv_probe;
  static const int korder_env = [] { const char* e = getenv("CYCLEDIFF_KORDER"); return e ? atoi(e) : -1; }();
  if (korder_env >= 0) pk.korder = korder_env;
  static const int tg_env = [] { const char* e = getenv("CYCLEDIFF_TILE_GROUP"); return e ? atoi(e) : 8; }();
  static const int tg_min_n = [] { const char* e = getenv("CYCLEDIFF_TILE_GROUP_MIN_N"); return e ? atoi(e) : 2048; }();
  if (tg_env > 0 && p.N >= tg_min_n && p.nbatch == 1) pk.tile_group = tg_env;
#ifdef CD_PROBE
  if (const char* e = getenv("CYCLEDIFF_PROBE_DBG")) pk.dbg = atoi(e);
  static const int dephase_env = [] { const char* e = getenv("CYCLEDIFF_DEPHASE_TICKS"); return e ? atoi(e) : 0; }();
  pk.dephase_ticks = dephase_env;
  pk.num_cus = device_cu_count();
  if (pk.dbg & 2) pk.stats = nullptr;
#endif
  static const CfgInfo kLinStreamCfg = {kLinStreamTile, 256, 64, 64, "lin_stream 256 x N, K = 320"};
  const CfgInfo* ci = nullptr;
  if (id == kLinStreamTile) {
    if (lin_stream_supports(pk)) ci = &kLinStreamCfg;
    else { CD_CHECK(!p.tile, "conv_gemm: lin_stream does not support this problem"); id = pick_config(p); }
  }
  for (int i = 0; i < kNumCfgs && !ci; ++i) if (kCfgs[i].id == id) ci = &kCfgs[i];
  CD_CHECK(ci, "conv_gemm: unknown tile configuration %d", id);
  if (p.act == ACT_GEGLU && (ci->TN % 64) != 0) { id = 2; ci = &kCfgs[1]; }
  if (cfg_needs_bk64(id)) CD_CHECK(k64, "conv_gemm: tile configuration %d needs channel counts that are multiples of 64", id);
  g_last_cfg = ci->name;
  {
    GemmLaunchInfo li;
    const bool lin = id == kLinStreamTile;
    li.bk = (lin || (k64 && !cfg_always_bk32(id))) ? 64 : 32;
    li.tile_id = li.bk == 32 ? bk32_alias(id) : id;
    li.splitk = pk.splitk > 1 ? pk.splitk : 1;
    li.chm = !lin && takes_channel_major(pk) ? 1 : 0;
    li.tile_group = lin ? 0 : pk.tile_group;
    g_last_launch = li;
  }
  static const bool trace = [] { const char* e = getenv("CYCLEDIFF_GEMM_TRACE"); return e && e[0] == '1'; }();
  if (trace) {
    const bool chm = id != kLinStreamTile && takes_channel_major(pk);
    fprintf(stderr, "[gemm_trace] %d %d %d %d %d %d %d %d %d %d %d %d | %s x%d\n", p.M, p.N, p.Ktot, p.KH, p.stride, p.up | (p.up_phase << 1),
            p.src1 ? 1 : 0, p.nbatch, p.act, p.resid ? 1 : 0, p.out_f32, chm ? 1 : 0, ci->name, pk.splitk > 1 ? pk.splitk : 1);
  }
  KernelProfiler* prof = g_conv_prof;
  hipEvent_t e0 = nullptr, e1 = nullptr;
  if (prof && prof->enabled) {
    char what[112] = "";
    if (prof->verbose)
      snprintf(what, sizeof(what), "M%d N%d K%d k%d s%d%s%s z%d act%d | %s x%d", p.M, p.N, p.Ktot, p.KH, p.stride,
               p.up ? " up" : (p.up_phase ? " up-phase" : ""), p.src1 ? " cat" : "", p.nbatch, p.act, ci->name, pk.splitk > 1 ? pk.splitk : 1);
    if (prof->verbose && !k64) strncat(what, " bk32", sizeof(what) - strlen(what) - 1);
    prof->next_pair(&e0, &e1, 2.0 * (double)p.M * (double)p.N * (double)p.Ktot * (double)p.nbatch * p.prof_flop_scale,
                    what);
    (void)hipEventRecord(e0, st);
  }
  struct Closer {
    hipEvent_t e; hipStream_t s;
    ~Closer() { if (e) (void)hipEventRecord(e, s); }
  } closer{e1, st};
  if (id == kLinStreamTile) launch_lin_stream(st, pk);
  else if (k64) dispatch<64>(st, pk, id);
  else dispatch<32>(st, pk, id);
}

int conv_gemm_num_configs() { return kNumCfgs; }
const char* conv_gemm_config_name(int id) {
  for (int i = 0; i < kNumCfgs; ++i) if (kCfgs[i].id == id) return kCfgs[i].name;
  return "?";
}

__global__ void k_repack_weight(const float* __restrict__ w, bf16_t* __restrict__ out, int N, int Cin,
                                int KH, int KW, int Npad, int Cpad, int geglu, int64_t src_row_offset) {
  const int64_t total = (int64_t)Npad * KH * KW * Cpad;
  for (int64_t i = blockIdx.x * (int64_t)blockDim.x + threadIdx.x; i < total;
       i += (int64_t)gridDim.x * blockDim.x) {
    const int c = (int)(i % Cpad);
    int64_t t = i / Cpad;
    const int s = (int)(t % KW); t /= KW;
    const int r = (int)(t % KH); t /= KH;
    const int np = (int)t;
    int n = np;
    if (geglu) {
      const int blk = np / 64, within = np % 64;
      n = (within < 32) ? blk * 32 + within : N / 2 + blk * 32 + (within - 32);
    }
    float v = 0.0f;
    if (np < N && c < Cin) v = w[(((int64_t)(n + src_row_offset) * Cin + c) * KH + r) * KW + s];
    out[i] = f2bf(v);
  }
}

__global__ void k_up_phase_weights(const bf16_t* __restrict__ w, bf16_t* __restrict__ out, int Npad, int Cpad) {
  const int64_t total = (int64_t)16 * Npad * Cpad;
  for (int64_t i = blockIdx.x * (int64_t)blockDim.x + threadIdx.x; i < total;
       i += (int64_t)gridDim.x * blockDim.x) {
    const int c = (int)(i % Cpad);
    int64_t t = i / Cpad;
    const int dx = (int)(t & 1), dy = (int)((t >> 1) & 1); t >>= 2;
    const int n = (int)(t % Npad);
    const int ph = (int)(t / Npad);
    const int a = ph >> 1, b = ph & 1;
    const int r0 = dy ? 1 + a : 0, r1 = dy ? 2 : a;
    const int s0 = dx ? 1 + b : 0, s1 = dx ? 2 : b;
    float v = 0.0f;
    for (int r = r0; r <= r1; ++r)
      for (int s = s0; s <= s1; ++s) v += bf2f(w[((int64_t)n * 9 + r * 3 + s) * Cpad + c]);
    out[i] = f2bf(v);
  }
}

void launch_up_phase_weights(hipStream_t st, const bf16_t* w, bf16_t* out, int Npad, int Cpad) {
  const int64_t total = (int64_t)16 * Npad * Cpad;
  int grid = (int)((total + 255) / 256);
  if (grid > 4096) grid = 4096;
  hipLaunchKernelGGL(k_up_phase_weights, dim3(grid), dim3(256), 0, st, w, out, Npad, Cpad);
}

void launch_repack_weight(hipStream_t st, const float* w, bf16_t* out, int N, int Cin, int KH,
                          int KW, int Npad, int Cpad, int geglu, int64_t src_row_offset) {
  const int64_t total = (int64_t)Npad * KH * KW * Cpad;
  int grid = (int)((total + 255) / 256);
  if (grid > 4096) grid = 4096;
  hipLaunchKernelGGL(k_repack_weight, dim3(grid), dim3(256), 0, st, w, out, N, Cin, KH, KW, Npad,
                     Cpad, geglu, src_row_offset);
}

}
```

cycle-diffusion_amd/csrc/engine.hip:

```cpp
#include <stdlib.h>

#include "engine.h"

#include <string.h>

namespace cd {

Arena::~Arena() { if (base_) (void)hipFree(base_); }
void Arena::init(size_t bytes) {
  if (base_) { (void)hipFree(base_); base_ = nullptr; }
  HIP_CHECK(hipMalloc((void**)&base_, bytes));
  cap_ = bytes; off_ = 0; high_ = 0;
}
void* Arena::alloc(size_t bytes) {
  size_t a = (off_ + 255) & ~(size_t)255;
  CD_CHECK(a + bytes <= cap_, "workspace arena exhausted: need %zu more bytes (capacity %zu); "
           "create the engine with a larger workspace", a + bytes - cap_, cap_);
  off_ = a + bytes;
  if (off_ > high_) high_ = off_;
  return base_ + a;
}

ParamStore::~ParamStore() {
  for (void* p : allocs_) (void)hipFree(p);
// ... 101 lines not shown
  d.targets.push_back(t);
}

template <typename OutT>
__global__ void k_pack_rows(const float* __restrict__ w, OutT* __restrict__ out, int rows, int Cin,
                            int KH, int KW, int Cpad, int dst_row0, int src_base, int grp,
                            int grp_stride, int geglu, int Ntot, float scale) {
  const int64_t total = (int64_t)rows * KH * KW * Cpad;
  for (int64_t i = blockIdx.x * (int64_t)blockDim.x + threadIdx.x; i < total;
       i += (int64_t)gridDim.x * blockDim.x) {
    const int c = (int)(i % Cpad);
    int64_t t = i / Cpad;
    const int s = (int)(t % KW); t /= KW;
    const int r = (int)(t % KH); t /= KH;
    const int j = (int)t;
    int jj = j;
    if (geglu) {
      const int blk = j / 64, within = j % 64;
      jj = (within < 32) ? blk * 32 + within : Ntot / 2 + blk * 32 + (within - 32);
    }
    const int src = src_base + (jj / grp) * grp_stride + (jj % grp);
    float v = 0.f;
    if (c < Cin) v = w[(((int64_t)src * Cin + c) * KH + r) * KW + s] * scale;
    const int64_t o = ((int64_t)(dst_row0 + j) * KH * KW + (int64_t)r * KW + s) * Cpad + c;
    if constexpr (sizeof(OutT) == 4) out[o] = v;
    else out[o] = f2bf(v);
  }
}

void ParamStore::load(hipStream_t st, const std::string& name, const float* host, int ndim,
                      const int64_t* shape) {
  ++version;
  auto it = by_name_.find(name);
  CD_CHECK(it != by_name_.end(), "unknown parameter name '%s'", name.c_str());
  ParamDecl& d = *it->second;
  int64_t n = 1, nd = 1;
  for (int i = 0; i < ndim; ++i) n *= shape[i];
  for (auto s : d.shape) nd *= s;
  bool ok = (n == nd) && ndim >= 1 && shape[0] == d.shape[0];
  if (ok && d.shape.size() >= 2 && ndim >= 2) ok = (shape[1] == d.shape[1]);
  CD_CHECK(ok, "parameter %s: shape mismatch (got %lld elements, ndim %d; expected %lld)", name.c_str(),
           (long long)n, ndim, (long long)nd);
  const size_t bytes = (size_t)n * sizeof(float);
  if (bytes > staging_bytes_) {
    if (staging_) HIP_CHECK(hipFree(staging_));
    staging_bytes_ = bytes < (1u << 20) ? (1u << 20) : bytes;
    HIP_CHECK(hipMalloc((void**)&staging_, staging_bytes_));
  }
  HIP_CHECK(hipStreamSynchronize(st));
  if (d.transposed) {
    const int64_t K = d.shape[0], N = d.shape[1];
    std::vector<float> tr((size_t)n);
    for (int64_t k = 0; k < K; ++k)
      for (int64_t j = 0; j < N; ++j) tr[(size_t)j * K + k] = host[(size_t)k * N + j];
    HIP_CHECK(hipMemcpy(staging_, tr.data(), bytes, hipMemcpyHostToDevice));
  } else {
    HIP_CHECK(hipMemcpy(staging_, host, bytes, hipMemcpyHostToDevice));
  }
  for (const PackTarget& t : d.targets) {
    if (t.kind == PackTarget::MATRIX_BF16) {
      const ConvW* c = t.conv;
      const int64_t total = (int64_t)t.rows * c->KH * c->KW * c->Cpad;
      int grid = (int)((total + 255) / 256);
      if (grid > 8192) grid = 8192;
      if (c->f32)
        hipLaunchKernelGGL(k_pack_rows<float>, dim3(grid), dim3(256), 0, st, staging_, (float*)c->w, t.rows, c->Cin,
                           c->KH, c->KW, c->Cpad, t.dst_row0, t.src_base, t.grp, t.grp_stride, t.geglu ? 1 : 0, c->N,
                           t.scale);
      else
        hipLaunchKernelGGL(k_pack_rows<bf16_t>, dim3(grid), dim3(256), 0, st, staging_, c->w, t.rows, c->Cin, c->KH,
                           c->KW, c->Cpad, t.dst_row0, t.src_base, t.grp, t.grp_stride, t.geglu ? 1 : 0, c->N, t.scale);
      if (c->wfrag) launch_pack_wfrag(st, c->w, c->Ktot(), c->wfrag, c->Npad);
      if (c->w3) launch_pack_w3(st, (const float*)c->w, c->w3, c->Npad, c->KH * c->KW, c->Cpad, overflow);
    } else {
      const int K = (t.kind == PackTarget::MATRIX_F32) ? t.K : 1;
      std::vector<float> tmp((size_t)t.rows * K);
      for (int j = 0; j < t.rows; ++j) {
        int jj = j;
        if (t.geglu) {
          const int blk = j / 64, within = j % 64;
          jj = (within < 32) ? blk * 32 + within : t.geglu_N / 2 + blk * 32 + (within - 32);
        }
        const int src = t.src_base + (jj / t.grp) * t.grp_stride + (jj % t.grp);
        memcpy(&tmp[(size_t)j * K], host + (size_t)src * K, (size_t)K * sizeof(float));
      }
      HIP_CHECK(hipMemcpy(t.fdst + (size_t)t.dst_off * K, tmp.data(), tmp.size() * sizeof(float),
                          hipMemcpyHostToDevice));
    }
  }
  HIP_CHECK(hipStreamSynchronize(st));
  d.loaded = true;
}

int ParamStore::missing(std::string* first) const {
  int n = 0;
  for (auto& d : decls_)
    if (!d->loaded) {
      if (n == 0 && first) *first = d->name;
      ++n;
    }
  return n;
}

Act alloc_act(Ctx& c, int B, int H, int W, int C, bool with_stats) {
  Act a; a.B = B; a.H = H; a.W = W; a.C = C; a.ld = C; a.f32 = c.f32;
  a.p = (bf16_t*)c.arena->alloc((size_t)B * H * W * C * (c.f32 ? sizeof(float) : sizeof(bf16_t)));
  if ((!c.f32 || c.x3) && with_stats && ((H * W) % 32) == 0)
    a.stats_buf = (float*)c.arena->alloc((size_t)(B * H * W / 32) * 2 * C * sizeof(float));
  return a;
}

static Act conv_split_fwd(Ctx& c, const ConvW& w, const Act& x, const ConvOpts& o) {
  CD_CHECK(c.f32 && c.x3 && w.w3 && (!w.geglu || o.raw_geglu), "conv: split input outside the split-fp16 mode");
  CD_CHECK(x.C == w.Cpad && x.ld == 2 * x.C, "conv: split input of %d channels (ld %d) against Cpad %d", x.C, x.ld, w.Cpad);
  CD_CHECK(!o.ln_fold && (!o.resid || (o.resid->f32 && !o.resid->split)), "conv: split-mode operands");
  ConvGemmParams p;
  p.src0 = x.p; p.C0 = 2 * x.C; p.ld0 = x.ld;
  p.src1 = x.p; p.C1 = x.C; p.ld1 = x.ld;
  p.B = x.B; p.Hs = x.H; p.Ws = x.W; p.up = o.up ? 1 : 0;
  p.Hin = o.up ? x.H * 2 : x.H; p.Win = o.up ? x.W * 2 : x.W;
  p.KH = w.KH; p.KW = w.KW; p.stride = o.stride;
  if (o.asym) { p.pad_t = 0; p.pad_l = 0; p.Hout = (p.Hin + 1 - w.KH) / o.stride + 1; p.Wout = (p.Win + 1 - w.KW) / o.stride + 1; }
  else {
    p.pad_t = o.pad; p.pad_l = o.pad;
    p.Hout = (p.Hin + 2 * o.pad - w.KH) / o.stride + 1;
    p.Wout = (p.Win + 2 * o.pad - w.KW) / o.stride + 1;
  }
  p.M = x.B * p.Hout * p.Wout;
  p.wgt = w.w3; p.Ktot = 3 * w.Ktot(); p.N = w.N;
  p.alpha = o.alpha * (1.0f / (kX3ActScale * kX3WgtScale)); p.bias = w.b;
  p.rowvec = o.rowvec; p.rowvec_ld = o.rowvec_ld; p.rows_per_vec = o.rows_per_vec;
  p.act = o.act;
  Act y; y.B = x.B; y.H = p.Hout; y.W = p.Wout; y.C = w.N; y.f32 = true;
  if (o.out) { y.p = (bf16_t*)o.out; y.ld = o.out_ld; }
  else { y.ld = w.N; y.p = (bf16_t*)c.arena->alloc((size_t)p.M * w.N * 4); }
  if (o.resid) {
    CD_CHECK(o.resid->rows() == p.M && o.resid->C == w.N, "conv: residual shape mismatch");
    p.resid = o.resid->p; p.resid_ld = o.resid->ld; p.resid_f32 = 1;
  }
  p.out = y.p; p.out_ld = y.ld; p.out_f32 = 1;
  p.zeros = c.zeros; p.tile = o.tile;
  p.prof_flop_scale = 1.0f / 3.0f;
  if (((p.Hout * p.Wout) % 32) == 0) {
    if (o.out && o.out_stats) y.stats_buf = o.out_stats;
    else if (!o.out && o.want_stats)
      y.stats_buf = (float*)c.arena->alloc((size_t)(p.M / 32) * 2 * w.N * sizeof(float));
    p.stats = y.stats_buf;
    y.stats = y.stats_buf;
  }
  launch_conv_gemm(c.st, p);
  return y;
}

bool conv_up_phase_taken(const Ctx& c, const ConvW& w, const Act& x, const Act* x2, const ConvOpts& o) {
  if (!o.up || c.f32 || x.split || x2 || !w.wphase || w.KH != 3 || w.KW != 3 || o.stride != 1 || o.pad != 1 || o.asym ||
      o.resid || o.out_f32 || o.ln_fold || w.geglu || o.act != ACT_NONE)
    return false;
  if ((x.H * x.W) % 256 != 0 || w.N % 8 != 0 || (o.out && o.out_ld % 8 != 0)) return false;
  const char* e = getenv("CYCLEDIFF_UP_PHASE");
  return !(e && e[0] == '0');
}

static Act conv_up_phase_fwd(Ctx& c, const ConvW& w, const Act& x, const ConvOpts& o) {
  ConvGemmParams p;
  p.src0 = x.p; p.C0 = round_up(x.C, 32); p.ld0 = x.ld;
  CD_CHECK(p.C0 == w.Cpad && x.ld >= p.C0, "conv: input channels %d do not match weight Cpad %d", p.C0, w.Cpad);
  p.B = x.B; p.Hs = x.H; p.Ws = x.W; p.Hin = x.H; p.Win = x.W; p.Hout = x.H; p.Wout = x.W;
  p.KH = 2; p.KW = 2; p.stride = 1; p.pad_t = 1; p.pad_l = 1;
  p.up_phase = 1; p.w_ps = w.Npad * 4 * w.Cpad;
  p.M = 4 * x.B * x.H * x.W;
  p.wgt = w.wphase; p.Ktot = 4 * w.Cpad; p.N = w.N;
  p.alpha = o.alpha; p.bias = w.b;
  p.rowvec = o.rowvec; p.rowvec_ld = o.rowvec_ld; p.rows_per_vec = o.rows_per_vec;
  Act y; y.B = x.B; y.H = 2 * x.H; y.W = 2 * x.W; y.C = w.N; y.f32 = false;
  if (o.out) { y.p = (bf16_t*)o.out; y.ld = o.out_ld; }
  else { y.ld = w.N; y.p = (bf16_t*)c.arena->alloc((size_t)p.M * w.N * 2); }
  if (o.out && o.out_stats) y.stats_buf = o.out_stats;
  else if (!o.out && o.want_stats) y.stats_buf = (float*)c.arena->alloc((size_t)(p.M / 32) * 2 * w.N * sizeof(float));
  p.stats = y.stats_buf;
  y.stats = y.stats_buf;
  const size_t mk = c.arena->mark();
  bf16_t* tmp = (bf16_t*)c.arena->alloc((size_t)p.M * w.N * 2);
  p.out = tmp; p.out_ld = w.N;
  p.zeros = c.zeros; p.tile = o.tile;
  launch_conv_gemm(c.st, p);
  launch_up_phase_reorder(c.st, tmp, y.p, x.B, x.H, x.W, w.N, y.ld);
  c.arena->release(mk);
  return y;
}

Act conv_fwd(Ctx& c, const ConvW& w, const Act& x, const Act* x2, const ConvOpts& o) {
  if (conv_up_phase_taken(c, w, x, x2, o)) return conv_up_phase_fwd(c, w, x, o);
  if (x.split) {
    CD_CHECK(!x2, "conv: a split activation cannot be concatenated");
    return conv_split_fwd(c, w, x, o);
  }
  ConvGemmParams p;
  CD_CHECK(w.f32 == c.f32 && x.f32 == c.f32 && (!x2 || x2->f32 == c.f32) && (!o.resid || o.resid->f32 == c.f32),
           "conv: operand precision does not match the running network");
  CD_CHECK((!x2 || !x2->split) && (!o.resid || !o.resid->split), "conv: split activation as a second source / residual");
  p.src0 = x.p; p.C0 = round_up(x.C, 32); p.ld0 = x.ld;
  if (x2) {
    CD_CHECK(x2->B == x.B && x2->H == x.H && x2->W == x.W, "conv: concat sources differ in shape");
    p.src1 = x2->p; p.C1 = x2->C; p.ld1 = x2->ld;
    CD_CHECK(x.C % 32 == 0 && x2->C % 32 == 0, "conv: concat channels must be multiples of 32");
  }
  CD_CHECK(p.C0 + p.C1 == w.Cpad, "conv: input channels %d+%d do not match weight Cpad %d", p.C0, p.C1, w.Cpad);
  CD_CHECK(x.ld >= p.C0, "conv: source row shorter than padded channel count");
  p.B = x.B; p.Hs = x.H; p.Ws = x.W; p.up = o.up ? 1 : 0;
  p.Hin = o.up ? x.H * 2 : x.H; p.Win = o.up ? x.W * 2 : x.W;
  p.KH = w.KH; p.KW = w.KW; p.stride = o.stride;
  if (o.asym) { p.pad_t = 0; p.pad_l = 0; p.Hout = (p.Hin + 1 - w.KH) / o.stride + 1; p.Wout = (p.Win + 1 - w.KW) / o.stride + 1; }
  else {
    p.pad_t = o.pad; p.pad_l = o.pad;
    p.Hout = (p.Hin + 2 * o.pad - w.KH) / o.stride + 1;
    p.Wout = (p.Win + 2 * o.pad - w.KW) / o.stride + 1;
  }
  p.M = x.B * p.Hout * p.Wout;
  p.wgt = w.w; p.wgt_frag = w.wfrag; p.Ktot = w.Ktot(); p.N = w.N;
  p.alpha = o.alpha; p.bias = w.b;
  p.rowvec = o.rowvec; p.rowvec_ld = o.rowvec_ld; p.rows_per_vec = o.rows_per_vec;
  const bool fuse_geglu = w.geglu && !o.raw_geglu;
  p.act = fuse_geglu ? ACT_GEGLU : o.act;
  const int Nout = fuse_geglu ? w.N / 2 : w.N;
  Act y; y.B = x.B; y.H = p.Hout; y.W = p.Wout; y.C = Nout; y.f32 = c.f32;
  if (o.out) { y.p = (bf16_t*)o.out; y.ld = o.out_ld; }
  else {
    y.ld = Nout;
    y.p = (bf16_t*)c.arena->alloc((size_t)p.M * Nout * ((o.out_f32 || c.f32) ? 4 : 2));
  }
  if (o.resid) {
    CD_CHECK(o.resid->rows() == p.M && o.resid->C == Nout, "conv: residual shape mismatch");
    p.resid = o.resid->p; p.resid_ld = o.resid->ld;
  }
  p.out = y.p; p.out_ld = y.ld; p.out_f32 = o.out_f32 ? 1 : 0;
  p.zeros = c.zeros; p.tile = o.tile;
  if (o.ln_fold) { p.ln_fold = 1; p.ln_eps = o.ln_eps; p.tile = kLinStreamTile; }
  if (c.f32) {
    p.out_f32 = 1;
    launch_conv_gemm_f32(c.st, p);
    return y;
  }
  if (!w.geglu && !o.out_f32 && ((p.Hout * p.Wout) % 32) == 0) {
    if (o.out && o.out_stats) y.stats_buf = o.out_stats;
    else if (!o.out && o.want_stats)
      y.stats_buf = (float*)c.arena->alloc((size_t)(p.M / 32) * 2 * Nout * sizeof(float));
    p.stats = y.stats_buf;
    y.stats = y.stats_buf;
  }
  launch_conv_gemm(c.st, p);
  return y;
}

bool conv_ln_fold_available(const Ctx& c, const ConvW& w, int64_t rows) {
  static const bool on = [] { const char* e = getenv("CYCLEDIFF_LN_FOLD"); return !(e && e[0] == '0'); }();
  static const int64_t min_rows = [] { const char* e = getenv("CYCLEDIFF_LN_FOLD_MIN_ROWS"); return e ? atoll(e) : 32768ll; }();
  return on && !c.f32 && w.wfrag && w.KH == 1 && w.KW == 1 && w.Cpad == 320 && rows >= min_rows && rows % 32 == 0 &&
         w.N % 64 == 0 && w.N <= 2560;
}

Act groupnorm_fwd(Ctx& c, const GNW& w, const Act& x, const Act* x2, bool silu, const float* film,
                  int film_ld) {
  GroupNormParams p;
  p.x = x.p; p.C0 = x.C; p.ld0 = x.ld;
  if (x2) { p.x1 = x2->p; p.C1 = x2->C; p.ld1 = x2->ld; }
  const int C = p.C0 + p.C1;
  CD_CHECK(C == w.C, "groupnorm: channels %d != weight %d", C, w.C);
  p.B = x.B; p.HW = x.H * x.W; p.G = 32; p.eps = w.eps; p.gamma = w.g; p.beta = w.b;
  p.film = film; p.film_ld = film_ld; p.silu = silu ? 1 : 0;
  Act y = alloc_act(c, x.B, x.H, x.W, C);
  p.y = y.p;
  if (c.f32) {
    CD_CHECK(x.f32 && (!x2 || x2->f32) && !x.split && (!x2 || !x2->split), "groupnorm: operand precision");
    if (c.x3) { p.split_out = 1; p.overflow = c.overflow; y.split = true; y.ld = 2 * C; }
    if (x.stats && x.ld == x.C && (!x2 || (x2->stats && x2->ld == x2->C))) {
      p.pre0 = x.stats;
      p.pre1 = x2 ? x2->stats : nullptr;
    }
    const size_t mk = c.arena->mark();
    void* ws = c.arena->alloc(groupnorm_f32_workspace(p.B, p.HW, C));
    launch_groupnorm_f32(c.st, p, ws);
    c.arena->release(mk);
    return y;
  }
  p.S = groupnorm_slabs(p.B, p.HW, C);
  const size_t part_floats = round_up((size_t)p.B * p.S * p.G * 2, (size_t)64);
  CD_CHECK(part_floats + (size_t)p.B * 2 * C <= c.gn_partial_floats, "groupnorm: workspace too small");
  p.partial = c.gn_partial;
  p.coef = c.gn_partial + part_floats;
  if (x.stats && x.ld == x.C && (!x2 || (x2->stats && x2->ld == x2->C))) {
    p.pre0 = x.stats;
    p.pre1 = x2 ? x2->stats : nullptr;
  }
  launch_groupnorm(c.st, p);
  return y;
}

Act avgpool2_fwd(Ctx& c, const Act& x) {
  if (x.split) {
    Act y = alloc_act(c, x.B, x.H / 2, x.W / 2, x.C);
    y.split = true; y.ld = 2 * x.C;
    launch_avgpool2_split(c.st, x.p, y.p, x.B, x.H, x.W, x.C, c.overflow);
    return y;
  }
  CD_CHECK(x.ld == x.C, "avgpool: dense input expected");
  Act y = alloc_act(c, x.B, x.H / 2, x.W / 2, x.C);
  if (c.f32) launch_avgpool2_f32(c.st, x.pf(), y.pf(), x.B, x.H, x.W, x.C);
  else launch_avgpool2(c.st, x.p, y.p, x.B, x.H, x.W, x.C);
  return y;
}
Act upsample2_fwd(Ctx& c, const Act& x) {
  CD_CHECK(x.ld == x.C && !x.split, "upsample: dense input expected");
  Act y = alloc_act(c, x.B, x.H * 2, x.W * 2, x.C);
  if (c.f32) launch_upsample2_f32(c.st, x.pf(), y.pf(), x.B, x.H, x.W, x.C);
  else launch_upsample2(c.st, x.p, y.p, x.B, x.H, x.W, x.C);
  return y;
}
Act attention_f32_fwd(Ctx& c, const Act& qk, const Act& v, int H, int D, float scale, const float* obias) {
  CD_CHECK(c.f32 && qk.f32 && v.f32 && !qk.split && !v.split && qk.C == 2 * H * D && v.C == H * D,
           "attention_f32: operands");
  Act o = alloc_act(c, qk.B, qk.H, qk.W, H * D);
  const int T = qk.H * qk.W;
  if (D <= 160 && (D % 4) == 0 && (qk.ld % 4) == 0 && (v.ld % 4) == 0) {
    launch_flash_f32(c.st, qk.pf(), qk.ld, (int64_t)T * qk.ld, qk.pf() + H * D, qk.ld, (int64_t)T * qk.ld, v.pf(), v.ld,
                     (int64_t)T * v.ld, o.pf(), o.ld, (int64_t)T * o.ld, qk.B, H, T, T, D, scale * 1.44269504088896340736f, 0,
                     c.overflow, obias);
    return o;
  }
  launch_attention_f32(c.st, qk.pf(), qk.ld, qk.pf() + H * D, qk.ld, v.pf(), v.ld, o.pf(), o.ld, qk.B, H, T, D, scale, obias);
  return o;
}

Act layernorm_fwd(Ctx& c, const LNW& w, const Act& x) {
  CD_CHECK(x.C == w.C, "layernorm: channels");
  if (c.f32) {
    CD_CHECK(x.f32 && !x.split, "layernorm_f32: operand precision");
    Act y = alloc_act(c, x.B, x.H, x.W, x.C);
// ... 69 lines not shown
```

cycle-diffusion_amd/csrc/kernels.h:

```cpp
#pragma once
#include <map>
#include <string>
#include <vector>

#include "common.h"

namespace cd {

struct StepCoef {
  float sa, s1a, sap, dirc, sigma, r, t_mask;
  int t;
};
enum { SCHED_DDIM = 0, SCHED_DDPM = 1 };

struct EpsHat {
  const float* p = nullptr;
  int64_t sb = 0, sc = 0, sp = 0;
  int cfg = 0;
  float g = 1.f;
  const float* gvec = nullptr;
};

struct StepGeom {
  int B = 0, C = 0, HW = 0;
  const StepCoef* tab = nullptr;
  int step = 0;
};
struct GaussSrc {
  const float* noise = nullptr;
  uint64_t seed = 0;
  uint32_t stream = 0;
};
struct XinOut {
  bf16_t* xin = nullptr;
  int cpad = 0;
  int dup = 0;
};
struct EpsIn {
  const float* p = nullptr;
  int64_t bstride = 0;
  int bmod = 0;
};
struct ZSlot {
  float* p = nullptr;
  int64_t bstride = 0;
};
struct StepArgs {
  const float* x0 = nullptr;
  float* xt = nullptr;
  EpsHat eh;
  StepGeom geom;
  GaussSrc gauss;
  XinOut xin;
  EpsIn eps;
  ZSlot z;
  int is_last = 0;
};

struct MaskBlend {
  const float* mask = nullptr;
  const float* src = nullptr;
  int mask_bmod = 1, src_bmod = 1;
  const float2* qtab = nullptr;
  int qrow = 0;
  GaussSrc gauss;
};

void launch_init_xt(hipStream_t st, const StepArgs& a);
void launch_encode_step(hipStream_t st, int kind, const StepArgs& a);
void launch_decode_step(hipStream_t st, int kind, const StepArgs& a, const MaskBlend* mk = nullptr, bool blend = false);
void launch_mask_blend_init(hipStream_t st, const StepArgs& a, const MaskBlend& mk);

struct LowpassTaps {
  const float* w = nullptr;
  const int* first = nullptr;
  int n_out = 0, n_in = 0, P = 0;
};
struct IlvrArgs {
  const float* xp = nullptr;
  float* out = nullptr;
  const float* y = nullptr;
  int y_bmod = 1;
  const float2* qtab = nullptr;
  int qrow = 0;
  GaussSrc gauss;
  float* T = nullptr;
  int B = 0, C = 0, R = 0;
  LowpassTaps D, U;
  XinOut xin;
  int vec4 = 0;
};
constexpr int kIlvrMaxR = 1024;
void build_lowpass_taps(int n_in, int n_out, std::vector<float>& w, std::vector<int>& first, int& P);
void launch_ilvr_down(hipStream_t st, const IlvrArgs& a);
void launch_ilvr_up_add(hipStream_t st, const IlvrArgs& a);

enum { ACT_NONE = 0, ACT_SILU = 1, ACT_GELU = 2, ACT_GEGLU = 3, ACT_QGELU = 4, ACT_RELU = 5 };

struct ConvGemmParams {
  const bf16_t* src0 = nullptr;
  const bf16_t* src1 = nullptr;
  int C0 = 0, C1 = 0;
  int ld0 = 0, ld1 = 0;
  int B = 1, Hs = 1, Ws = 1;
  int up = 0;
  int Hin = 1, Win = 1;
  int KH = 1, KW = 1, stride = 1, pad_t = 0, pad_l = 0;
  int Hout = 1, Wout = 1;
  int M = 0;
  const bf16_t* wgt = nullptr;
  const bf16_t* wgt_frag = nullptr;
  int Ktot = 0, N = 0;
  int ldw = 0;
  int nbatch = 1;
  int64_t a_bs = 0, w_bs = 0, o_bs = 0;
  float alpha = 1.0f;
  const float* bias = nullptr;
  const float* rowvec = nullptr;
  int rowvec_ld = 0, rows_per_vec = 1;
  const bf16_t* resid = nullptr;
  int resid_ld = 0;
  int resid_f32 = 0;
  int act = ACT_NONE;
  void* out = nullptr;
  int out_ld = 0;
  int out_f32 = 0;
  float* stats = nullptr;
  const bf16_t* zeros = nullptr;
  int ln_fold = 0;
  float ln_eps = 1e-5f;
  int tile = 0;
  float prof_flop_scale = 1.f;
  int splitk = 0;
  float* sk_scratch = nullptr;
  int* sk_flags = nullptr;
  unsigned long long* probe = nullptr;
  int korder = 1;
  int tile_group = 0;
  int dephase_ticks = 0;
  int num_cus = 256;
  int dbg = 0;
  int up_phase = 0;
  int w_ps = 0;
};
constexpr int kProbeWords = 48;
extern thread_local unsigned long long* g_conv_probe;
struct SplitKWorkspace {
  float* scratch = nullptr;
  size_t scratch_bytes = 0;
  int* flags = nullptr;
  int nflags = 0;
};
extern thread_local SplitKWorkspace g_conv_splitk;
void launch_conv_gemm(hipStream_t st, const ConvGemmParams& p);
const char* conv_gemm_last_config();
struct GemmLaunchInfo {
  int tile_id = 0;
  int bk = 0;
  int splitk = 1;
  int chm = 0;
  int tile_group = 0;
};
GemmLaunchInfo conv_gemm_last_launch();
void launch_up_phase_weights(hipStream_t st, const bf16_t* w, bf16_t* out, int Npad, int Cpad);
int conv_gemm_num_configs();
const char* conv_gemm_config_name(int id);

struct LinStreamParams {
  const bf16_t* a = nullptr; int lda = 0;
  const bf16_t* wfrag = nullptr;
  const float* bias = nullptr;
  const bf16_t* resid = nullptr; int ldr = 0;
  bf16_t* out = nullptr; int ldo = 0;
  float* stats = nullptr;
  int M = 0, N = 0;
  float ln_eps = 1e-5f;
  int geglu_direct = 0;
};
constexpr int kLinStreamTile = 30;
bool lin_stream_supports(const ConvGemmParams& p);
void launch_lin_stream(hipStream_t st, const ConvGemmParams& p);
void launch_fold_ln(hipStream_t st, const bf16_t* w, int ldw, const float* gamma, const float* beta, const float* bias,
                    bf16_t* w_out, float* bias_out, int N, int Kc);
void launch_pack_wfrag(hipStream_t st, const bf16_t* w, int ldw, bf16_t* out, int N);

struct KernelProfiler {
  bool enabled = false;
  std::vector<hipEvent_t> events;
  std::vector<double> flops;
  std::vector<std::string> labels;
  int used = 0;
  bool verbose = false;
  struct Entry { int n = 0; double ms = 0, flops = 0; };
  std::map<std::string, Entry> per_shape;
  void next_pair(hipEvent_t* a, hipEvent_t* b, double fl, const std::string& what);
  void collect(int* launches, double* total_ms, double* total_flops);
  ~KernelProfiler();
};
extern thread_local KernelProfiler* g_conv_prof;

struct ConvTuner {
  bool enabled = false;
  void* scratch = nullptr;
  size_t scratch_bytes = 0;
  int shapes_tuned = 0;
};
extern ConvTuner g_conv_tuner;

void launch_repack_weight(hipStream_t st, const float* w, bf16_t* out, int N, int Cin, int KH,
                          int KW, int Npad, int Cpad, int geglu, int64_t src_row_offset);

struct GroupNormParams {
  const bf16_t* x = nullptr;
  const bf16_t* x1 = nullptr;
  int C0 = 0, C1 = 0, ld0 = 0, ld1 = 0;
  int B = 0, HW = 0, G = 32;
  float eps = 1e-5f;
  const float* gamma = nullptr;
  const float* beta = nullptr;
  const float* film = nullptr;
  int film_ld = 0;
  int silu = 0;
  int split_out = 0;
  int* overflow = nullptr;
  bf16_t* y = nullptr;
  float* partial = nullptr;
  int S = 0;
  float* coef = nullptr;
  const float* pre0 = nullptr;
  const float* pre1 = nullptr;
};
int groupnorm_slabs(int B, int HW, int C);
void launch_groupnorm(hipStream_t st, const GroupNormParams& p);

void launch_layernorm(hipStream_t st, const bf16_t* x, int ldx, bf16_t* y, int ldy, int rows,
                      int C, const float* gamma, const float* beta, float eps);
void launch_softmax_rows(hipStream_t st, const float* s, int lds, bf16_t* p, int ldp, int64_t rows,
                         int cols);

struct AttnParams {
  const bf16_t* q = nullptr;
  const bf16_t* k = nullptr;
  const bf16_t* v = nullptr;
  const bf16_t* vt = nullptr;
  int ldv = 0; int64_t v_bs = 0;
  bf16_t* o = nullptr;
  int B = 0, H = 0, Tq = 0, Tk = 0, D = 0;
  int ldq = 0, ldk = 0, ldo = 0;
  int64_t q_bs = 0, k_bs = 0, o_bs = 0;
  int vt_dpad = 0, vt_tpad = 0;
  float scale = 1.0f;
  int q_log2 = 0;
  const float* obias = nullptr;
  int causal = 0;
};
void launch_attention(hipStream_t st, const AttnParams& p);
constexpr int kCtrlKeys = 96;
struct CtrlAttnParams {
  const bf16_t* q_own = nullptr;
  const bf16_t* q_src = nullptr;
  const bf16_t* k_own = nullptr;
  const bf16_t* k_src = nullptr;
  const bf16_t* va = nullptr;
  const bf16_t* vb = nullptr;
  bf16_t* o = nullptr;
  int B = 0, B_src = 0, H = 0, Tq = 0, L = 0, D = 0;
  int ldq = 0, ldk = 0, ldv = 0, ldo = 0;
  int64_t q_bs = 0, k_bs = 0, v_bs = 0, o_bs = 0;
  float scale = 1.0f;
  int q_log2 = 0;
};
void launch_cross_attention_ctrl(hipStream_t st, const CtrlAttnParams& p);
void launch_ctrl_values(hipStream_t st, const bf16_t* v, const float* M, const float* alpha, const float* w, int rows,
                        int B_ctrl, int L, int C, bf16_t* va, bf16_t* vb);
void launch_transpose_v(hipStream_t st, const bf16_t* v, int ldv, int64_t v_bs, bf16_t* vt, int B,
                        int H, int Tk, int D, int Dpad, int Tpad);

void launch_mfma_sustained(hipStream_t st, int target_ms, float* tflops, float* ghz);

void launch_nchw_to_nhwc(hipStream_t st, const float* x, bf16_t* y, int B, int C, int HW, int Cpad,
                         float scale, float shift, int dup);
void launch_nhwc_to_nchw(hipStream_t st, const void* x, int x_f32, int ldx, float* y, int B, int C,
                         int HW, float scale, float shift);
void launch_timestep_embedding(hipStream_t st, const StepCoef* tab, int step, const float* t_explicit,
                               float* out, int B, int dim, int mode);
void launch_vec_linear(hipStream_t st, const float* x, int ldx, const float* W, const float* bias,
                       float* y, int ldy, int B, int K, int N, int silu_in, int silu_out);
void launch_avgpool2(hipStream_t st, const bf16_t* x, bf16_t* y, int B, int H, int W, int C);
void launch_upsample2(hipStream_t st, const bf16_t* x, bf16_t* y, int B, int H, int W, int C);
void launch_up_phase_reorder(hipStream_t st, const bf16_t* x, bf16_t* y, int B, int H, int W, int C, int ldy);
void launch_posterior_sample(hipStream_t st, const float* mom, int ld, const float* noise,
                             uint64_t seed, float* z, int B, int zc, int HW, float scale,
                             int use_mean);
void launch_vq_quantize(hipStream_t st, const float* z, float in_mul, const float* codebook, int n_embed, int zc,
                        int B, int HW, bf16_t* out, int Cpad);
void launch_fill_f32(hipStream_t st, float* p, float v, int64_t n);
void launch_vit_tokens(hipStream_t st, const bf16_t* patch, const float* cls, const float* pos, bf16_t* out, int B,
                       int T, int D);
void launch_gather_eot(hipStream_t st, const bf16_t* x, const int* ids, bf16_t* out, int B, int L, int D);
void launch_embed_tokens(hipStream_t st, const int* ids, const float* tok, const float* pos, bf16_t* out, int B,
                         int L, int D, int vocab);
void launch_conv_gemm_f32(hipStream_t st, const ConvGemmParams& p);
size_t groupnorm_f32_workspace(int B, int HW, int C);
void launch_groupnorm_f32(hipStream_t st, const GroupNormParams& p, void* workspace);
void launch_attention_f32(hipStream_t st, const float* q, int ldq, const float* k, int ldk, const float* v, int ldv,
                          float* o, int ldo, int B, int H, int T, int D, float scale, const float* obias);
void launch_nchw_to_nhwc_f32(hipStream_t st, const float* x, float* y, int B, int C, int HW, int Cpad, float scale,
                             float shift, int split = 0, int* overflow = nullptr);
void launch_avgpool2_f32(hipStream_t st, const float* x, float* y, int B, int H, int W, int C);
void launch_flash_f32(hipStream_t st, const float* q, int ldq, int64_t q_bs, const float* k, int ldk, int64_t k_bs,
                      const float* v, int ldv, int64_t v_bs, float* o, int ldo, int64_t o_bs, int B, int H, int Tq, int Tk,
                      int D, float qmul, int split, int* overflow, const float* obias = nullptr);
void launch_layernorm_f32(hipStream_t st, const float* x, int ldx, float* y, int64_t rows, int C, const float* gamma,
                          const float* beta, float eps, int split, int* overflow);
// ... 14 lines not shown
```

cycle-diffusion_amd/csrc/nets_ho_vae.hip:

```cpp
#include <limits.h>

#include <algorithm>

#include "engine.h"

namespace cd {

namespace {

GNW mk_gn(ParamStore& ps, const std::string& pfx, int C) {
  GNW g; g.C = C; g.eps = 1e-6f;
  g.g = ps.new_vec(C, 1.f); g.b = ps.new_vec(C, 0.f);
  ps.vec(pfx + ".weight", g.g, C);
  ps.vec(pfx + ".bias", g.b, C);
  return g;
}
ConvW* mk_conv(ParamStore& ps, const std::string& pfx, int N, int Cin, int k, bool bias = true) {
  ConvW* c = ps.new_conv(N, Cin, k, k, bias);
  ps.conv_weight(pfx + ".weight", c, 4);
  if (bias) ps.conv_bias(pfx + ".bias", c);
  return c;
}

struct RnW {
// ... 38 lines not shown
  Act out = alloc_act(c, x.B, x.H, x.W, r.cout, true);
  const size_t mk = c.arena->mark();
  Act h = groupnorm_fwd(c, r.n1, x, x2, true);
  ConvOpts o1; o1.want_stats = true;
  if (r.emb_off >= 0) {
    o1.rowvec = proj + r.emb_off; o1.rowvec_ld = proj_ld;
    o1.rows_per_vec = t_shared ? INT_MAX : x.H * x.W;
  }
  Act h2 = conv_fwd(c, *r.c1, h, nullptr, o1);
  Act h3 = groupnorm_fwd(c, r.n2, h2, nullptr, true);
  Act skip;
  if (r.nin) { ConvOpts os; os.pad = 0; skip = conv_fwd(c, *r.nin, x, x2, os); }
  else { CD_CHECK(!x2, "identity shortcut with concat input"); skip = x; }
  ConvOpts o2; o2.resid = &skip; o2.out = out.p; o2.out_ld = out.ld; o2.out_stats = out.stats_buf;
  conv_fwd(c, *r.c2, h3, nullptr, o2);
  out.stats = out.stats_buf;
  c.arena->release(mk);
  return out;
}

void vt_gemm2(Ctx& c, const ConvW& wv, const bf16_t* x, int ldx, int B, int T, int Tpad, bf16_t* vt) {
  ConvGemmParams p;
  p.src0 = wv.w; p.C0 = wv.Cpad; p.ld0 = wv.Cpad;
  p.B = 1; p.Hs = wv.N; p.Ws = 1; p.Hin = wv.N; p.Win = 1; p.Hout = wv.N; p.Wout = 1;
  p.M = wv.N;
  p.wgt = x; p.Ktot = wv.Cpad; p.ldw = ldx; p.N = T;
  p.nbatch = B; p.a_bs = 0; p.w_bs = (int64_t)T * ldx; p.o_bs = (int64_t)wv.N * Tpad;
  p.out = vt; p.out_ld = Tpad; p.zeros = c.zeros;
  launch_conv_gemm(c.st, p);
}

Act at_fwd(Ctx& c, const AtW& a, const Act& x) {
  const int B = x.B, T = x.H * x.W, C = a.C;
  Act out = alloc_act(c, B, x.H, x.W, C, true);
  const size_t mk = c.arena->mark();
  ConvOpts p0; p0.pad = 0;
  Act n = groupnorm_fwd(c, a.norm, x, nullptr, false);
  Act qk = conv_fwd(c, *a.qk, n, nullptr, p0);
  if (c.f32) {
    Act v = conv_fwd(c, *a.v, n, nullptr, p0);
    Act o = attention_f32_fwd(c, qk, v, 1, C, 1.0f / sqrtf((float)C), a.vbias);
    ConvOpts po; po.pad = 0; po.resid = &x; po.out = out.p; po.out_ld = out.ld;
    conv_fwd(c, *a.proj, o, nullptr, po);
    c.arena->release(mk);
    return out;
  }
  const int Tpad = round_up(T, 64);
  bf16_t* vt = (bf16_t*)c.arena->alloc((size_t)B * C * Tpad * 2);
  if (Tpad != T) HIP_CHECK(hipMemsetAsync(vt, 0, (size_t)B * C * Tpad * 2, c.st));
  vt_gemm2(c, *a.v, n.p, n.ld, B, T, Tpad, vt);
  const float scale = 1.0f / sqrtf((float)C);
  Act o = alloc_act(c, B, x.H, x.W, C);
  if (C <= 160) {
    AttnParams p;
    p.q = qk.p; p.k = qk.p + C; p.vt = vt; p.o = o.p;
    p.B = B; p.H = 1; p.Tq = T; p.Tk = T; p.D = C;
    p.ldq = qk.ld; p.ldk = qk.ld; p.ldo = o.ld;
    p.q_bs = (int64_t)T * qk.ld; p.k_bs = (int64_t)T * qk.ld; p.o_bs = (int64_t)T * o.ld;
    p.vt_dpad = C; p.vt_tpad = Tpad; p.scale = scale; p.obias = a.vbias;
    launch_attention(c.st, p);
  } else {
    CD_CHECK(T % 32 == 0, "AttnBlock: token count %d must be a multiple of 32", T);
    float* S = (float*)c.arena->alloc((size_t)B * T * T * 4);
    bf16_t* P = (bf16_t*)c.arena->alloc((size_t)B * T * T * 2);
    ConvGemmParams g;
    g.src0 = qk.p; g.C0 = C; g.ld0 = qk.ld; g.B = 1; g.Hs = T; g.Ws = 1; g.Hin = T; g.Win = 1;
    g.Hout = T; g.Wout = 1; g.M = T;
    g.wgt = qk.p + C; g.Ktot = C; g.ldw = qk.ld; g.N = T;
    g.nbatch = B; g.a_bs = (int64_t)T * qk.ld; g.w_bs = (int64_t)T * qk.ld; g.o_bs = (int64_t)T * T;
    g.alpha = scale; g.out = S; g.out_ld = T; g.out_f32 = 1; g.zeros = c.zeros;
    launch_conv_gemm(c.st, g);
    launch_softmax_rows(c.st, S, T, P, T, (int64_t)B * T, T);
    ConvGemmParams h;
    h.src0 = P; h.C0 = T; h.ld0 = T; h.B = 1; h.Hs = T; h.Ws = 1; h.Hin = T; h.Win = 1;
    h.Hout = T; h.Wout = 1; h.M = T;
    h.wgt = vt; h.Ktot = T; h.ldw = Tpad; h.N = C;
    h.nbatch = B; h.a_bs = (int64_t)T * T; h.w_bs = (int64_t)C * Tpad; h.o_bs = (int64_t)T * C;
    h.bias = a.vbias; h.out = o.p; h.out_ld = o.ld; h.zeros = c.zeros;
    launch_conv_gemm(c.st, h);
  }
  ConvOpts po; po.pad = 0; po.resid = &x; po.out = out.p; po.out_ld = out.ld; po.out_stats = out.stats_buf;
  conv_fwd(c, *a.proj, o, nullptr, po);
  out.stats = out.stats_buf;
  c.arena->release(mk);
  return out;
}

class VAEKL : public VAE {
 public:
  explicit VAEKL(const cd_net_desc& d);
  void encode_moments(Ctx& c, const bf16_t* img, int B, int R, float* moments) override;
  void decode(Ctx& c, const bf16_t* z, int B, int h, float* img) override;
 private:
  int ch_, nres_, nlev_;
  std::vector<int> mult_;
  ConvW* e_in_ = nullptr; std::vector<std::vector<RnW>> e_blk_; std::vector<ConvW*> e_down_;
  RnW e_m1_, e_m2_; AtW e_at_; GNW e_no_; ConvW* e_out_ = nullptr; ConvW* quant_ = nullptr;
  ConvW* pq_ = nullptr; ConvW* d_in_ = nullptr; RnW d_m1_, d_m2_; AtW d_at_;
  std::vector<std::vector<RnW>> d_blk_; std::vector<ConvW*> d_up_; GNW d_no_; ConvW* d_out_ = nullptr;
  int in_ch_, out_ch_, embed_, moments_;
};

VAEKL::VAEKL(const cd_net_desc& d) {
  desc = d;
  f32 = d.precision == CD_PREC_F32 || d.precision == CD_PREC_F32X3;
  x3 = d.precision == CD_PREC_F32X3;
  params.f32 = f32; params.x3 = x3;
  CD_CHECK(!(f32 && d.n_embed > 0), "the VQ first stage (codebook lookup on 16-bit rows) runs in the 16-bit format only");
  ch_ = d.model_channels; nres_ = d.num_res_blocks; nlev_ = d.n_mult;
  for (int i = 0; i < nlev_; ++i) mult_.push_back(d.channel_mult[i]);
  z_channels = d.z_channels; embed_ = d.embed_dim; in_ch_ = d.in_channels; out_ch_ = d.out_channels;
  factor = 1 << (nlev_ - 1);
  CD_CHECK((d.double_z != 0) != (d.n_embed > 0), "first stage must be either KL (double_z) or VQ (n_embed > 0)");
  CD_CHECK(d.n_attn == 0, "attn_resolutions inside the VAE levels are not used by the f4 / f8 configs");
  const int zmul = d.double_z ? 2 : 1;
  moments_ = zmul * z_channels;
  moments_channels = zmul * embed_;
  n_embed = d.n_embed;
  e_in_ = mk_conv(params, "encoder.conv_in", ch_, in_ch_, 3);
  int bin = ch_;
  e_blk_.resize(nlev_); e_down_.assign(nlev_, nullptr);
  for (int l = 0; l < nlev_; ++l) {
    const int bout = ch_ * mult_[l];
    for (int b = 0; b < nres_; ++b) {
      e_blk_[l].push_back(mk_rn(params, "encoder.down." + std::to_string(l) + ".block." + std::to_string(b), bin, bout));
      bin = bout;
    }
    if (l != nlev_ - 1) e_down_[l] = mk_conv(params, "encoder.down." + std::to_string(l) + ".downsample.conv", bin, bin, 3);
  }
  e_m1_ = mk_rn(params, "encoder.mid.block_1", bin, bin);
  e_at_ = mk_at(params, "encoder.mid.attn_1", bin);
  e_m2_ = mk_rn(params, "encoder.mid.block_2", bin, bin);
  e_no_ = mk_gn(params, "encoder.norm_out", bin);
  e_out_ = mk_conv(params, "encoder.conv_out", moments_, bin, 3);
  quant_ = mk_conv(params, "quant_conv", zmul * embed_, moments_, 1);
  if (n_embed > 0) {
    float* cb = params.new_vec(n_embed * embed_);
    params.mat_f32("quantize.embedding.weight", cb, n_embed, embed_);
    codebook = cb;
  }
  pq_ = mk_conv(params, "post_quant_conv", z_channels, embed_, 1);
  bin = ch_ * mult_[nlev_ - 1];
  d_in_ = mk_conv(params, "decoder.conv_in", bin, z_channels, 3);
  d_m1_ = mk_rn(params, "decoder.mid.block_1", bin, bin);
  d_at_ = mk_at(params, "decoder.mid.attn_1", bin);
  d_m2_ = mk_rn(params, "decoder.mid.block_2", bin, bin);
  d_blk_.resize(nlev_); d_up_.assign(nlev_, nullptr);
  for (int l = nlev_ - 1; l >= 0; --l) {
    const int bout = ch_ * mult_[l];
    for (int b = 0; b <= nres_; ++b) {
      d_blk_[l].push_back(mk_rn(params, "decoder.up." + std::to_string(l) + ".block." + std::to_string(b), bin, bout));
      bin = bout;
    }
    if (l != 0) d_up_[l] = mk_conv(params, "decoder.up." + std::to_string(l) + ".upsample.conv", bin, bin, 3);
  }
  d_no_ = mk_gn(params, "decoder.norm_out", bin);
  d_out_ = mk_conv(params, "decoder.conv_out", out_ch_, bin, 3);
}

void VAEKL::encode_moments(Ctx& c, const bf16_t* img, int B, int R, float* moments) {
  const size_t mk = c.arena->mark();
  c.f32 = f32; c.x3 = x3;
  const size_t esz = f32 ? 4 : 2;
  Act x; x.p = (bf16_t*)img; x.B = B; x.H = R; x.W = R; x.C = round_up(in_ch_, 32); x.ld = x.C; x.f32 = f32;
  if (x3) { x.split = true; x.ld = 2 * x.C; }
  ConvOpts o3; o3.want_stats = true;
  Act h = conv_fwd(c, *e_in_, x, nullptr, o3);
  for (int l = 0; l < nlev_; ++l) {
    for (auto& r : e_blk_[l]) h = rn_fwd(c, r, h, nullptr, nullptr, 0, true);
    if (e_down_[l]) { ConvOpts od; od.stride = 2; od.asym = true; od.want_stats = true; h = conv_fwd(c, *e_down_[l], h, nullptr, od); }
  }
  h = rn_fwd(c, e_m1_, h, nullptr, nullptr, 0, true);
  h = at_fwd(c, e_at_, h);
  h = rn_fwd(c, e_m2_, h, nullptr, nullptr, 0, true);
  Act n = groupnorm_fwd(c, e_no_, h, nullptr, true);
  const int cp = round_up(moments_, 32);
  Act mo = alloc_act(c, B, h.H, h.W, cp);
  HIP_CHECK(hipMemsetAsync(mo.p, 0, (size_t)mo.rows() * cp * esz, c.st));
  ConvOpts oo; oo.out = mo.p; oo.out_ld = cp;
  conv_fwd(c, *e_out_, n, nullptr, oo);
  ConvOpts oq; oq.pad = 0; oq.out_f32 = true; oq.out = moments; oq.out_ld = moments_channels;
  conv_fwd(c, *quant_, mo, nullptr, oq);
  c.arena->release(mk);
  c.f32 = false; c.x3 = false;
}

void VAEKL::decode(Ctx& c, const bf16_t* z, int B, int hl, float* img) {
  const size_t mk = c.arena->mark();
  c.f32 = f32; c.x3 = x3;
  Act x; x.p = (bf16_t*)z; x.B = B; x.H = hl; x.W = hl; x.C = round_up(embed_, 32); x.ld = x.C; x.f32 = f32;
  if (x3) { x.split = true; x.ld = 2 * x.C; }
  const int cp = round_up(z_channels, 32);
  Act zq = alloc_act(c, B, hl, hl, cp);
  HIP_CHECK(hipMemsetAsync(zq.p, 0, (size_t)zq.rows() * cp * (f32 ? 4 : 2), c.st));
  ConvOpts oq; oq.pad = 0; oq.out = zq.p; oq.out_ld = cp;
  conv_fwd(c, *pq_, x, nullptr, oq);
  ConvOpts o3; o3.want_stats = true;
  Act h = conv_fwd(c, *d_in_, zq, nullptr, o3);
  h = rn_fwd(c, d_m1_, h, nullptr, nullptr, 0, true);
  h = at_fwd(c, d_at_, h);
  h = rn_fwd(c, d_m2_, h, nullptr, nullptr, 0, true);
  for (int l = nlev_ - 1; l >= 0; --l) {
    for (auto& r : d_blk_[l]) h = rn_fwd(c, r, h, nullptr, nullptr, 0, true);
    if (d_up_[l]) { ConvOpts ou; ou.up = true; ou.want_stats = true; h = conv_fwd(c, *d_up_[l], h, nullptr, ou); }
  }
  Act n = groupnorm_fwd(c, d_no_, h, nullptr, true);
  ConvOpts oo; oo.out_f32 = true; oo.out = img; oo.out_ld = out_ch_;
  conv_fwd(c, *d_out_, n, nullptr, oo);
  c.arena->release(mk);
  c.f32 = false; c.x3 = false;
}

class UNetHo : public UNet {
 public:
  explicit UNetHo(const cd_net_desc& d);
  int kind() const override { return CD_NET_UNET_HO; }
  void forward(Ctx& c, const UNetIO& io) override;
  size_t workspace_hint(int B) const override {
    return (size_t)B * image_size * image_size * ch_ * 8 * 2 * 24 + (64u << 20);
  }
 private:
  int ch_, nres_, nlev_, temb_ch_;
  std::vector<int> mult_;
  TimeEmb te_;
  ConvW* cin_ = nullptr;
  struct Lvl { std::vector<RnW> blk; std::vector<AtW> att; ConvW* resamp = nullptr; };
  std::vector<Lvl> down_, up_;
  RnW m1_, m2_; AtW mat_;
  GNW no_; ConvW* cout_ = nullptr;
};

UNetHo::UNetHo(const cd_net_desc& d) {
  desc = d;
  f32 = d.precision == CD_PREC_F32 || d.precision == CD_PREC_F32X3;
  x3 = d.precision == CD_PREC_F32X3;
  params.f32 = f32; params.x3 = x3;
  ch_ = d.model_channels; nres_ = d.num_res_blocks; nlev_ = d.n_mult; temb_ch_ = 4 * ch_;
  image_size = d.image_size; out_channels = d.out_channels; in_cpad = round_up(d.in_channels, 32);
  CD_CHECK(ch_ % 32 == 0, "ch must be a multiple of 32");
  CD_CHECK(d.conv_resample, "resamp_with_conv=False is not used by the reference configs");
  for (int i = 0; i < nlev_; ++i) mult_.push_back(d.channel_mult[i]);
  auto has_attn = [&](int res) { for (int i = 0; i < d.n_attn; ++i) if (d.attn[i] == res) return true; return false; };
  std::vector<std::pair<std::string, RnW*>> temb_users;
  cin_ = mk_conv(params, "conv_in", ch_, d.in_channels, 3);
  int res = d.image_size, bin = ch_;
  std::vector<int> in_mult{1};
  for (int m : mult_) in_mult.push_back(m);
  down_.resize(nlev_);
  for (int l = 0; l < nlev_; ++l) {
    bin = ch_ * in_mult[l];
    const int bout = ch_ * mult_[l];
    down_[l].blk.reserve(nres_); down_[l].att.reserve(nres_);
    for (int b = 0; b < nres_; ++b) {
      const std::string pfx = "down." + std::to_string(l);
      down_[l].blk.push_back(mk_rn(params, pfx + ".block." + std::to_string(b), bin, bout));
      temb_users.push_back({pfx + ".block." + std::to_string(b), &down_[l].blk.back()});
      bin = bout;
      if (has_attn(res)) down_[l].att.push_back(mk_at(params, pfx + ".attn." + std::to_string(b), bin));
    }
    if (l != nlev_ - 1) {
      down_[l].resamp = mk_conv(params, "down." + std::to_string(l) + ".downsample.conv", bin, bin, 3);
      res /= 2;
    }
  }
  m1_ = mk_rn(params, "mid.block_1", bin, bin); temb_users.push_back({"mid.block_1", &m1_});
  mat_ = mk_at(params, "mid.attn_1", bin);
  m2_ = mk_rn(params, "mid.block_2", bin, bin); temb_users.push_back({"mid.block_2", &m2_});
  up_.resize(nlev_);
  for (int l = nlev_ - 1; l >= 0; --l) {
    const int bout = ch_ * mult_[l];
    int skip_in = ch_ * mult_[l];
    up_[l].blk.reserve(nres_ + 1); up_[l].att.reserve(nres_ + 1);
    for (int b = 0; b <= nres_; ++b) {
      if (b == nres_) skip_in = ch_ * in_mult[l];
      const std::string pfx = "up." + std::to_string(l);
      up_[l].blk.push_back(mk_rn(params, pfx + ".block." + std::to_string(b), bin + skip_in, bout));
      temb_users.push_back({pfx + ".block." + std::to_string(b), &up_[l].blk.back()});
      bin = bout;
      if (has_attn(res)) up_[l].att.push_back(mk_at(params, pfx + ".attn." + std::to_string(b), bin));
    }
    if (l != 0) {
      up_[l].resamp = mk_conv(params, "up." + std::to_string(l) + ".upsample.conv", bin, bin, 3);
      res *= 2;
    }
  }
  no_ = mk_gn(params, "norm_out", bin);
  cout_ = mk_conv(params, "conv_out", d.out_channels, bin, 3);
  te_.mode = 1; te_.dim = ch_; te_.hidden = temb_ch_;
  te_.w0 = params.new_vec(temb_ch_ * ch_); te_.b0 = params.new_vec(temb_ch_);
  te_.w1 = params.new_vec(temb_ch_ * temb_ch_); te_.b1 = params.new_vec(temb_ch_);
  params.mat_f32("temb.dense.0.weight", te_.w0, temb_ch_, ch_);
  params.vec("temb.dense.0.bias", te_.b0, temb_ch_);
  params.mat_f32("temb.dense.1.weight", te_.w1, temb_ch_, temb_ch_);
  params.vec("temb.dense.1.bias", te_.b1, temb_ch_);
  int total = 0;
  for (auto& u : temb_users) { u.second->emb_off = total; total += u.second->cout; }
  te_.proj_total = total;
  te_.proj_w = params.new_vec(total * temb_ch_);
  te_.proj_b = params.new_vec(total);
  for (auto& u : temb_users) {
    params.mat_f32(u.first + ".temb_proj.weight", te_.proj_w, u.second->cout, temb_ch_, u.second->emb_off);
    params.bias_rows(u.first + ".temb_proj.bias", u.second->cout, te_.proj_b, u.second->emb_off, u.second->cout, 0,
                     u.second->cout, 0);
  }
}

void UNetHo::forward(Ctx& c, const UNetIO& io) {
  const size_t mk0 = c.arena->mark();
  c.f32 = f32; c.x3 = x3;
  const int B = io.B, R = image_size;
  const int tB = io.t_shared ? 1 : B;
  float* sinu = (float*)c.arena->alloc((size_t)tB * ch_ * 4);
  float* e1 = (float*)c.arena->alloc((size_t)tB * temb_ch_ * 4);
  float* emb = (float*)c.arena->alloc((size_t)tB * temb_ch_ * 4);
  float* proj = (float*)c.arena->alloc((size_t)tB * te_.proj_total * 4);
  launch_timestep_embedding(c.st, io.tab, io.step, io.t_explicit, sinu, tB, ch_, 1);
  launch_vec_linear(c.st, sinu, ch_, te_.w0, te_.b0, e1, temb_ch_, tB, ch_, temb_ch_, 0, 1);
  launch_vec_linear(c.st, e1, temb_ch_, te_.w1, te_.b1, emb, temb_ch_, tB, temb_ch_, temb_ch_, 0, 0);
  launch_vec_linear(c.st, emb, temb_ch_, te_.proj_w, te_.proj_b, proj, te_.proj_total, tB, temb_ch_,
                    te_.proj_total, 1, 0);
  const int pl = te_.proj_total;
  Act x; x.p = (bf16_t*)io.xin; x.B = B; x.H = R; x.W = R; x.C = in_cpad; x.ld = in_cpad; x.f32 = f32;
  if (x3) { x.split = true; x.ld = 2 * in_cpad; }
  ConvOpts o3; o3.want_stats = true;
  std::vector<Act> hs;
  hs.push_back(conv_fwd(c, *cin_, x, nullptr, o3));
  for (int l = 0; l < nlev_; ++l) {
    for (int b = 0; b < nres_; ++b) {
      Act h = rn_fwd(c, down_[l].blk[b], hs.back(), nullptr, proj, pl, io.t_shared);
      if (!down_[l].att.empty()) h = at_fwd(c, down_[l].att[b], h);
      hs.push_back(h);
    }
    if (down_[l].resamp) {
      ConvOpts od; od.stride = 2; od.asym = true; od.want_stats = true;
      hs.push_back(conv_fwd(c, *down_[l].resamp, hs.back(), nullptr, od));
    }
  }
  Act h = hs.back();
  h = rn_fwd(c, m1_, h, nullptr, proj, pl, io.t_shared);
  h = at_fwd(c, mat_, h);
  h = rn_fwd(c, m2_, h, nullptr, proj, pl, io.t_shared);
  for (int l = nlev_ - 1; l >= 0; --l) {
    for (int b = 0; b <= nres_; ++b) {
      Act skip = hs.back(); hs.pop_back();
      h = rn_fwd(c, up_[l].blk[b], h, &skip, proj, pl, io.t_shared);
      if (!up_[l].att.empty()) h = at_fwd(c, up_[l].att[b], h);
    }
    if (up_[l].resamp) { ConvOpts ou; ou.up = true; ou.want_stats = true; h = conv_fwd(c, *up_[l].resamp, h, nullptr, ou); }
  }
  Act n = groupnorm_fwd(c, no_, h, nullptr, true);
  ConvOpts oo; oo.out_f32 = true; oo.out = io.out; oo.out_ld = io.out_ld;
  conv_fwd(c, *cout_, n, nullptr, oo);
  c.arena->release(mk0);
  c.f32 = false; c.x3 = false;
}

}
// ... 6 lines not shown
```

include/cyclediff.h:

```cpp
#ifndef CYCLEDIFF_H
#define CYCLEDIFF_H
#include <stddef.h>
#include <stdint.h>

#ifdef __cplusplus
extern "C" {
#endif

typedef struct cd_engine* cd_handle;

enum { CD_NET_UNET_OPENAI = 1, CD_NET_UNET_HO = 2, CD_NET_VAE_KL = 3, CD_NET_CLIP_TEXT = 4, CD_NET_BERT_XTR = 5,
       CD_NET_OCLIP_TEXT = 6, CD_NET_OCLIP_VISION = 7, CD_NET_INCEPTION_FID = 8 };
enum { CD_SCHED_DDIM = 0, CD_SCHED_DDPM = 1 };
enum { CD_PREC_16 = 0, CD_PREC_F32 = 1, CD_PREC_F32X3 = 2 };
enum { CD_MASK_QSAMPLE = 0, CD_MASK_ENCODER = 1 };

typedef struct cd_net_desc {
  int kind;
  int image_size;
  int in_channels, out_channels;
  int model_channels;
  int num_res_blocks;
  int n_mult;  int channel_mult[8];
  int n_attn;  int attn[8];
  int num_heads;
  int num_head_channels;
  int use_spatial_transformer, context_dim, transformer_depth;
  int use_scale_shift_norm, resblock_updown, conv_resample;
  int z_channels, embed_dim, double_z;
  int precision;
  int n_embed;
  int reserved[6];
} cd_net_desc;

typedef struct cd_step_coef {
  float sa, s1a, sap, dirc, sigma, r, t_mask;
  int32_t t;
} cd_step_coef;

const char* cd_last_error(void);
int cd_version(void);
int cd_act_format(void);

int cd_engine_create(void* hip_stream, size_t workspace_bytes, cd_handle* out);
int cd_engine_destroy(cd_handle h);
int cd_engine_workspace_high_water(cd_handle h, size_t* bytes);
int cd_engine_synchronize(cd_handle h);
int cd_prof_enable(cd_handle h, int on);
int cd_prof_collect(cd_handle h, int* launches, double* total_ms, double* total_flops);

int cd_net_create(cd_handle h, const cd_net_desc* desc, int* net_id);
int cd_net_param_count(cd_handle h, int net, int* n);
int cd_net_param_info(cd_handle h, int net, int index, char* name, int name_cap, int* ndim, int64_t shape[4]);
int cd_net_load_param(cd_handle h, int net, const char* name, const float* data_host, int ndim,
                      const int64_t* shape);
int cd_net_missing_params(cd_handle h, int net, int* n_missing, char* first_name, int name_cap);

int cd_unet_forward(cd_handle h, int net, const float* x, const float* t, const float* ctx, int B,
                    int ctx_len, float* eps_out);

int cd_text_encode(cd_handle h, int net, const int32_t* tokens, int B, int L, float* out);

int cd_inception_features(cd_handle h, int net, const float* img, int B, int stop_block, float* out);
int cd_clip_text_features(cd_handle h, int net, const int32_t* tokens, int B, int L, float* out);
int cd_clip_image_features(cd_handle h, int net, const float* img, int B, float* out);

int cd_vae_encode(cd_handle h, int net, const float* img, const float* noise, uint64_t seed, int B, int R,
                  int sample, float scale, float* z0);
int cd_vae_decode(cd_handle h, int net, const float* z0, int B, int hlat, float scale, float out_mul,
                  float out_add, float* img);

int cd_dpm_encode(cd_handle h, int net, int sched_kind, const float* x0, const float* ctx_c,
                  const float* ctx_uc, int ctx_len, float guidance, int B, int K,
                  const cd_step_coef* coef_host, const float* noise, uint64_t seed,
                  int last_uses_x0, float* z_out);

int cd_ddim_decode(cd_handle h, int net, int sched_kind, const float* z, int z_slots, int n_eps,
                   const float* ctx_c, const float* ctx_uc, int ctx_len, float guidance, int B, int K,
                   const cd_step_coef* coef_host, const float* noise_tail, uint64_t seed, float* x_out);

int cd_ddim_decode_v(cd_handle h, int net, int sched_kind, const float* z, int z_slots, int n_eps,
                     const float* ctx_c, const float* ctx_uc, int ctx_len, const float* guidance_per_sample, int B,
                     int K, const cd_step_coef* coef_host, const float* noise_tail, uint64_t seed, float* x_out);

int cd_ddim_invert(cd_handle h, int net, int sched_kind, const float* x0, const float* ctx_c, const float* ctx_uc,
                   int ctx_len, float guidance, int B, int K, const cd_step_coef* coef_host, float* x_out,
                   float* traj_out);

int cd_cycle_translate(cd_handle h, int net, int sched_kind, const float* x0, const float* enc_ctx_c,
                       const float* enc_ctx_uc, float enc_guidance, const float* dec_ctx_c, const float* dec_ctx_uc,
                       float dec_guidance, const float* dec_guidance_per_sample, int ctx_len, int B, int n_dec, int K,
                       const cd_step_coef* coef_enc_host, const cd_step_coef* coef_dec_host, const float* noise,
                       uint64_t seed, int last_uses_x0, float* z_out, float* x_out);

int cd_ddim_decode_masked(cd_handle h, int net, int sched_kind, const float* z, int z_slots, int n_eps, const float* ctx_c,
                          const float* ctx_uc, int ctx_len, float guidance, const float* guidance_per_sample, int B, int K,
                          const cd_step_coef* coef_host, const float* noise_tail, uint64_t seed, const float* mask,
                          const float* x0, int B_mask, int mask_source, const float* qsample_coef_host,
                          const float* mask_noise, uint64_t mask_seed, float* x_out);

int cd_cycle_translate_masked(cd_handle h, int net, int sched_kind, const float* x0, const float* enc_ctx_c,
                              const float* enc_ctx_uc, float enc_guidance, const float* dec_ctx_c, const float* dec_ctx_uc,
                              float dec_guidance, const float* dec_guidance_per_sample, int ctx_len, int B, int n_dec, int K,
                              const cd_step_coef* coef_enc_host, const cd_step_coef* coef_dec_host, const float* noise,
                              uint64_t seed, int last_uses_x0, const float* mask, const float* mask_x0, int B_mask,
                              int mask_source, const float* qsample_coef_host, const float* mask_noise, uint64_t mask_seed,
                              float* z_out, float* x_out);

int cd_cycle_translate_ctrl(cd_handle h, int net, int sched_kind, const float* x0, const float* enc_ctx_c,
                            const float* enc_ctx_uc, float enc_guidance, const float* dec_ctx_c, const float* dec_ctx_uc,
                            float dec_guidance, const float* dec_guidance_per_sample, int ctx_len, int B, int n_dec, int K,
                            const cd_step_coef* coef_enc_host, const cd_step_coef* coef_dec_host, const float* noise,
                            uint64_t seed, int last_uses_x0, const float* mask, const float* mask_x0, int B_mask,
                            int mask_source, const float* qsample_coef_host, const float* mask_noise, uint64_t mask_seed,
                            const float* mapper, const float* alpha, const float* weight, int B_ctrl, int n_ctrl,
                            float* z_out, float* x_out);

int cd_ilvr_decode(cd_handle h, int net, int sched_kind, const float* z, int z_slots, int n_eps, int B, int K,
                   const cd_step_coef* coef_host, const float* noise_tail, uint64_t seed, const float* ref, int B_ref,
                   int down_n, int range_t, const float* qsample_coef_host, const float* ref_noise, uint64_t ref_seed,
                   float* x_out);

int cd_pix_refine(cd_handle h, int net, int sched_kind, float* x, int B, int R,
                  const cd_step_coef* coef_host, const float* noise, uint64_t seed);

int cd_op_pack_conv_weight(cd_handle h, const float* w_host, int N, int Cin, int KH, int KW, int geglu,
                           void** packed_dev, int* Npad, int* Cpad);
int cd_op_free(cd_handle h, void* dev);
int cd_op_conv2d(cd_handle h, const float* x0, int C0, const float* x1, int C1, int B, int H, int W,
                 const void* packed_w, int N, int KH, int KW, int stride, int pad, int asym_pad, int up,
                 const float* bias, const float* rowvec, const float* resid, int act, int tile, float* y);
int cd_op_conv2d_16(cd_handle h, const float* x0, int C0, const float* x1, int C1, int B, int H, int W,
                    const void* packed_w, int N, int KH, int KW, int stride, int pad, int asym_pad, int up,
                    const float* bias, const float* rowvec, const float* resid, int act, int tile, float* y,
                    float* stats);
int cd_op_last_gemm_config(cd_handle h, int* tile_id, int* bk, int* splitk, int* chm, int* tile_group);
int cd_op_up_phase_reorder(cd_handle h, const float* x, int B, int C, int H, int W, float* y);
int cd_op_groupnorm(cd_handle h, const float* x, int B, int C, int H, int W, int G, float eps,
                    const float* gamma, const float* beta, const float* film, int silu, float* y);
int cd_op_groupnorm_ex(cd_handle h, const float* x0, int C0, int pad0, const float* x1, int C1, int pad1, int B, int H,
                       int W, float eps, const float* gamma, const float* beta, const float* film, int film_ld, int silu,
                       const float* stats0, const float* stats1, int precision, void* y);
int cd_op_layernorm(cd_handle h, const float* x, int rows, int C, const float* gamma, const float* beta,
                    float eps, float* y);
int cd_op_attention(cd_handle h, const float* q, const float* k, const float* v, int B, int H, int Tq,
                    int Tk, int D, float scale, int use_transpose_kernel, float* o);
int cd_op_cross_attention_ctrl(cd_handle h, const float* q_own, const float* q_src, const float* k_own, const float* k_src,
                               const float* v_own, const float* mapper, const float* alpha, const float* weight, int B,
                               int B_src, int B_ctrl, int H, int Tq, int L, int L_buf, int D, float scale, float* o);
int cd_op_lowpass(cd_handle h, const float* x, int B, int C, int R, int down_n, float* y);
int cd_op_softmax_rows(cd_handle h, const float* s, int64_t rows, int cols, float* p);
int cd_op_timestep_embedding(cd_handle h, const float* t, int B, int dim, int mode, float* out);
int cd_op_sched_step(cd_handle h, int mode, int sched_kind, const cd_step_coef* coef_host, const float* x0,
                     float* xt, const float* eps_hat, int cfg, float guidance, const float* noise,
                     const float* eps_in, int is_last, int B, int C, int HW, float* z_slot);
int cd_op_sched_step_masked(cd_handle h, int mode, const cd_step_coef* coef_host, float* x, const float* eps_hat, int cfg,
                            float guidance, const float* eps_in, const float* mask, const float* src, int B_mask,
                            int mask_source, float qa, float qb, const float* mask_noise, int blend, int B, int C, int HW,
                            void* xin16_out, int cfg_dup);
int cd_op_bench_conv(cd_handle h, int B, int H, int W, int C0, int C1, int N, int k, int stride, int up,
                     int act, int tile, int iters, float* ms_out);
int cd_op_bench_mfma_sustained(cd_handle h, int target_ms, float* tflops_out, float* ghz_out);
int cd_op_probe(cd_handle h, int which, const void* in, void* out, size_t n);

#ifdef __cplusplus
}
#endif
#endif
```

Measured before the change: 3.573 images/s.

## Store phase-form upsample conv output directly in image order, extend to VAE decoder

Adds an UPD variant of the conv GEMM kernel whose epilogue scatters each sub-pixel phase's output rows straight to their interleaved image positions and remaps the GroupNorm stats blocks. This removes the temporary buffer and separate up_phase_reorder pass. It also adds a second phase ordering (phase-major) so small resolutions with H*W not a multiple of 256 can use the phase form. The VAE decoder upsample convs now register phase weights and take this path. Scattered 16-byte stores may coalesce worse, and the index math adds epilogue cost.

```diff
diff --git a/cycle-diffusion_amd/_ffi.py b/cycle-diffusion_amd/_ffi.py
--- a/cycle-diffusion_amd/_ffi.py
+++ b/cycle-diffusion_amd/_ffi.py
@@ -81,6 +81,7 @@
     "cd_op_conv2d_16": [_VP, _VP, _I, _VP, _I, _I, _I, _I, _VP, _I, _I, _I, _I, _I, _I, _I, _VP, _VP, _VP, _I, _I, _VP,
                         _VP],
     "cd_op_last_gemm_config": [_VP] + [C.POINTER(_I)] * 5,
+    "cd_op_last_gemm_up_phase": [_VP] + [C.POINTER(_I)] * 2,
     "cd_op_up_phase_reorder": [_VP, _VP, _I, _I, _I, _I, _VP],
     "cd_op_groupnorm": [_VP, _VP, _I, _I, _I, _I, _I, _F, _VP, _VP, _VP, _I, _VP],
     "cd_op_groupnorm_ex": [_VP, _VP, _I, _I, _VP, _I, _I, _I, _I, _I, _F, _VP, _VP, _VP, _I, _I, _VP, _VP, _I, _VP],
diff --git a/cycle-diffusion_amd/csrc/capi.hip b/cycle-diffusion_amd/csrc/capi.hip
--- a/cycle-diffusion_amd/csrc/capi.hip
+++ b/cycle-diffusion_amd/csrc/capi.hip
@@ -1133,6 +1133,15 @@
   CD_API_END
 }
 
+int cd_op_last_gemm_up_phase(cd_handle h, int* up_phase, int* up_direct) {
+  CD_API_BEGIN
+  CD_CHECK(h, "bad argument");
+  const GemmLaunchInfo li = conv_gemm_last_launch();
+  if (up_phase) *up_phase = li.up_phase;
+  if (up_direct) *up_direct = li.up_direct;
+  CD_API_END
+}
+
 int cd_op_groupnorm(cd_handle h, const float* x, int B, int C, int H, int W, int G, float eps,
                     const float* gamma, const float* beta, const float* film, int silu, float* y) {
   CD_API_BEGIN
diff --git a/cycle-diffusion_amd/csrc/conv_gemm.hip b/cycle-diffusion_amd/csrc/conv_gemm.hip
--- a/cycle-diffusion_amd/csrc/conv_gemm.hip
+++ b/cycle-diffusion_amd/csrc/conv_gemm.hip
@@ -91,7 +91,7 @@
          (!p.rowvec || ((p.rowvec_ld & 3) == 0 && (p.rows_per_vec >= p.M || (p.rows_per_vec & 31) == 0)));
 }
 
-template <int BM, int BN, int BK, int WM, int WN, int NSTAGE, bool CHM = false>
+template <int BM, int BN, int BK, int WM, int WN, int NSTAGE, bool CHM = false, bool UPD = false>
 __global__ __launch_bounds__(64 * WM * WN, (WM * WN == 4 && BK == 32 && NSTAGE == 3 && BM * BN >= 128 * 256) ? 2 : 1) void k_conv_gemm(ConvGemmParams p) {
 #if defined(__HIP_DEVICE_COMPILE__)
   using T = TileCfg<BM, BN, BK, WM, WN, NSTAGE>;
@@ -158,9 +158,18 @@
   int b_first = pow2 ? (m0 >> sh_hw) : (m0 / HWo);
   CD_PROBE_ONLY(if (p.dbg & 4) b_first = 0;)
   int pad_t = p.pad_t, pad_l = p.pad_l, w_ph = 0;
+  int m_ph = 0;
   if (p.up_phase) {
-    const int ph = b_first & 3;
+    int ph = b_first & 3;
     b_first >>= 2;
+    if constexpr (UPD) {
+      if (p.up_phase == 2) {
+        const int rows_pp = p.B * HWo;
+        ph = m0 / rows_pp;
+        m_ph = ph * rows_pp;
+        b_first = (m0 - m_ph) >> sh_hw;
+      }
+    }
     pad_t = 1 - (ph >> 1); pad_l = 1 - (ph & 1);
     w_ph = ph * p.w_ps;
   }
@@ -185,7 +194,13 @@
     a_mk[i] = 0; a_base[i] = 0;
     if (m < p.M) {
       int b, oy, ox;
-      if (pow2) {
+      if constexpr (UPD) {
+        const int md = m - m_ph;
+        b = md >> sh_hw;
+        if (p.up_phase != 2) b >>= 2;
+        const int rem = md & (HWo - 1);
+        oy = rem >> sh_w; ox = rem & (p.Wout - 1);
+      } else if (pow2) {
         b = m >> sh_hw;
         const int rem = m & (HWo - 1);
         oy = rem >> sh_w; ox = rem & (p.Wout - 1);
@@ -194,7 +209,7 @@
         const int rem = m - b * HWo;
         oy = rem / p.Wout; ox = rem - oy * p.Wout;
       }
-      if (p.up_phase) b >>= 2;
+      if (!UPD && p.up_phase) b >>= 2;
       a_iy0[i] = oy * p.stride - pad_t;
       a_ix0[i] = ox * p.stride - pad_l;
       a_boff[i] = (b - b_first) * p.Hs * p.Ws;
@@ -504,13 +519,36 @@
     const int nblk = (p.M + 31) >> 5;
     int blk_ok = nblk - (mw >> 5);
     blk_ok = blk_ok < 0 ? 0 : (blk_ok > NRB ? NRB : blk_ok);
-    const __amdgpu_buffer_rsrc_t rs_o = uniform_rsrc(outp + (int64_t)mw * p.out_ld * 2, rows_ok * p.out_ld * 2);
+    int u_ph = 0, u_r0 = 0, u_nimg = 1, u_shhw = 0, u_shw = 0, u_hw = 1;
+    int64_t u_img = 0;
+    if constexpr (UPD) {
+      u_hw = p.Hs * p.Ws;
+      u_shhw = 31 - __builtin_clz(u_hw); u_shw = 31 - __builtin_clz(p.Ws);
+      int mr = mw;
+      if (p.up_phase == 2) {
+        const int rows_pp = p.B * u_hw;
+        u_ph = mw / rows_pp;
+        mr = mw - u_ph * rows_pp;
+        u_img = mr >> u_shhw;
+      } else {
+        u_ph = (mw >> u_shhw) & 3;
+        u_img = mw >> (u_shhw + 2);
+      }
+      u_r0 = mr & (u_hw - 1);
+      u_nimg = ((u_r0 + TM - 1) >> u_shhw) + 1;
+      if (u_nimg > p.B - (int)u_img) u_nimg = p.B - (int)u_img;
+    }
+    const __amdgpu_buffer_rsrc_t rs_o =
+        UPD ? uniform_rsrc(outp + u_img * (4 * u_hw) * p.out_ld * 2, u_nimg * (4 * u_hw) * p.out_ld * 2)
+            : uniform_rsrc(outp + (int64_t)mw * p.out_ld * 2, rows_ok * p.out_ld * 2);
     const __amdgpu_buffer_rsrc_t rs_r =
         uniform_rsrc(has_res ? (const void*)(p.resid + (int64_t)zb * p.o_bs + (int64_t)mw * p.resid_ld) : (const void*)outp,
                      has_res ? rows_ok * p.resid_ld * 2 : 0);
     const __amdgpu_buffer_rsrc_t rs_s =
-        uniform_rsrc(p.stats ? (const void*)(p.stats + ((int64_t)zb * nblk + (mw >> 5)) * 2 * p.N) : (const void*)outp,
-                     p.stats ? blk_ok * 2 * p.N * 4 : 0);
+        UPD ? uniform_rsrc(p.stats ? (const void*)(p.stats + u_img * (u_hw >> 3) * 2 * p.N) : (const void*)outp,
+                           p.stats ? u_nimg * (u_hw >> 3) * 2 * p.N * 4 : 0)
+            : uniform_rsrc(p.stats ? (const void*)(p.stats + ((int64_t)zb * nblk + (mw >> 5)) * 2 * p.N) : (const void*)outp,
+                           p.stats ? blk_ok * 2 * p.N * 4 : 0);
     const float* TB = (const float*)(smem + T::LDS_BYTES) + wn * TN;
     const float* TR = (const float*)(smem + T::LDS_BYTES) + T::TAB_BIAS_I * 256 + (wm * NRB) * BN + wn * TN;
     constexpr bool PIPE = NW <= 8;
@@ -547,7 +585,7 @@
       __builtin_amdgcn_wave_barrier();
       CD_PROBE_ONLY(const unsigned long long pr_c1 = probe_time(); pr_stage += pr_c1 - pr_c0;)
       const f32x4 b0 = *(const f32x4*)(TB + jc * 32 + col), b1 = *(const f32x4*)(TB + jc * 32 + col + 4);
-      const unsigned vo_out = n < p.N ? (unsigned)((vr * p.out_ld + n) * 2) : kInvalid;
+      const unsigned vo_out = n < p.N ? (unsigned)(((UPD ? 0 : vr * p.out_ld) + n) * 2) : kInvalid;
 #pragma unroll
       for (int rb = 0; rb < NRB; ++rb) {
         const int kb = (jc / CJ) * NRB + rb;
@@ -571,7 +609,7 @@
         float ssum[8], ssq[8];
 #pragma unroll
         for (int e = 0; e < 8; ++e) { ssum[e] = 0.f; ssq[e] = 0.f; }
-        const unsigned vo_blk = vo_out + (unsigned)(rb * 32 * p.out_ld * 2);
+        const unsigned vo_blk = UPD ? vo_out : vo_out + (unsigned)(rb * 32 * p.out_ld * 2);
 #pragma unroll
         for (int ps = 0; ps < 4; ++ps)
           if (ps < NP) {
@@ -586,9 +624,15 @@
               for (int e = 0; e < 8; ++e) vp[e] += rf[e];
             }
             const uint4 pk = pack8(vp);
+            unsigned vo_row = (unsigned)(ps * RPP * p.out_ld * 2);
+            if constexpr (UPD) {
+              const int q = u_r0 + rb * 32 + ps * RPP + vr, r = q & (u_hw - 1);
+              const int pix = ((q >> u_shhw) << (u_shhw + 2)) + 2 * r + ((r >> u_shw) << (u_shw + 1)) +
+                              (((u_ph >> 1) << (u_shw + 1)) + (u_ph & 1));
+              vo_row = (unsigned)(pix * p.out_ld * 2);
+            }
             CD_PROBE_ONLY(if (!(p.dbg & 1)))
-            __builtin_amdgcn_raw_buffer_store_b128((u32x4e){pk.x, pk.y, pk.z, pk.w}, rs_o,
-                                                   vo_blk + (unsigned)(ps * RPP * p.out_ld * 2), 0, CD_EPI_STORE_AUX);
+            __builtin_amdgcn_raw_buffer_store_b128((u32x4e){pk.x, pk.y, pk.z, pk.w}, rs_o, vo_blk + vo_row, 0, CD_EPI_STORE_AUX);
             if constexpr (!KEEP) {
               const float on = (mb + ps * RPP + vr) < p.M ? 1.0f : 0.0f;
 #pragma unroll
@@ -634,13 +678,18 @@
         }
         {
           const int nc0 = n0 + wn * TN + jc * 32;
+          int sblk = rb;
+          if constexpr (UPD) {
+            const int q = u_r0 + rb * 32;
+            sblk = (q >> u_shhw) * (u_hw >> 3) + u_ph * (u_hw >> 5) + ((q & (u_hw - 1)) >> 5);
+          }
           if (cw == 64) {
-            const unsigned so = nc0 + lane_ep < p.N ? (unsigned)((rb * 2 * p.N + nc0 + lane_ep) * 4) : kInvalid;
+            const unsigned so = nc0 + lane_ep < p.N ? (unsigned)((sblk * 2 * p.N + nc0 + lane_ep) * 4) : kInvalid;
             __builtin_amdgcn_raw_buffer_store_b32(__builtin_bit_cast(unsigned, s_sum), rs_s, so, 0, 0);
             __builtin_amdgcn_raw_buffer_store_b32(__builtin_bit_cast(unsigned, s_sq), rs_s, so + (unsigned)(p.N * 4), 0, 0);
           } else {
             const int arr = lane_ep >> 5, c = lane_ep & 31;
-            const unsigned so = nc0 + c < p.N ? (unsigned)((rb * 2 * p.N + arr * p.N + nc0 + c) * 4) : kInvalid;
+            const unsigned so = nc0 + c < p.N ? (unsigned)((sblk * 2 * p.N + arr * p.N + nc0 + c) * 4) : kInvalid;
             __builtin_amdgcn_raw_buffer_store_b32(__builtin_bit_cast(unsigned, s_sum), rs_s, so, 0, 0);
           }
         }
@@ -890,6 +939,16 @@
     HIP_CHECK(hipFuncSetAttribute((const void*)kern1, hipFuncAttributeMaxDynamicSharedMemorySize, kLds));
   });
   auto kern = chm ? kern1 : kern0;
+  if (p.up_direct) {
+    if constexpr (T::HAS_TAB) {
+      static PerDeviceOnce upd_once;
+      auto kern2 = k_conv_gemm<BM, BN, BK, WM, WN, NSTAGE, false, true>;
+      upd_once([&]() { HIP_CHECK(hipFuncSetAttribute((const void*)kern2, hipFuncAttributeMaxDynamicSharedMemorySize, kLds)); });
+      kern = kern2;
+    } else {
+      CD_CHECK(false, "conv_gemm: this tile configuration cannot store a phase-form launch in image order");
+    }
+  }
   if (split > 1) {
     const SplitKWorkspace& ws = g_conv_splitk;
     CD_CHECK(p.sk_scratch && p.sk_flags, "conv_gemm: split-K without workspace");
@@ -932,6 +991,7 @@
 constexpr int kNumCfgs = sizeof(kCfgs) / sizeof(kCfgs[0]);
 inline int bk32_alias(int id) { return id == 9 ? 7 : id == 13 ? 12 : id == 18 ? 5 : id == 19 ? 5 : id; }
 inline bool cfg_always_bk32(int id) { return id == 24 || id == 25; }
+inline bool cfg_lacks_tables(int id, bool bk64) { return id == 9 && bk64; }
 
 }
 thread_local SplitKWorkspace g_conv_splitk;
@@ -1146,6 +1206,7 @@
     if (cfg_needs_bk64(c.id) && !use64) continue;
     if ((c.id == 24 || c.id == 25) && bi == 1) continue;
     if (c.BN == 320 && (p.N % 320) != 0) continue;
+    if (p.up_direct && cfg_lacks_tables(c.id, use64)) continue;
     const int64_t tiles = (int64_t)ceil_div(p.M, c.BM) * ceil_div(p.N, c.BN) * p.nbatch;
     if (split > 1) {
       if (!sk.scratch || tiles >= device_cu_count() || nk < 4 * split || tiles * split > 2048) continue;
@@ -1202,10 +1263,22 @@
   CD_CHECK(((uintptr_t)p.src0 & 15) == 0 && ((uintptr_t)p.wgt & 15) == 0, "conv_gemm: 16-B alignment");
   CD_CHECK((p.ld0 % 8) == 0 && (p.src1 == nullptr || (p.ld1 % 8) == 0), "conv_gemm: ld must be a multiple of 8");
   if (p.act == ACT_GEGLU) CD_CHECK(p.N % 64 == 0, "GEGLU needs packed N %% 64 == 0");
-  if (p.up_phase)
+  if (p.up_phase) {
+    const int hw = p.Hs * p.Ws;
     CD_CHECK(p.KH == 2 && p.KW == 2 && p.stride == 1 && !p.up && !p.src1 && p.nbatch == 1 && p.Hout == p.Hs && p.Wout == p.Ws &&
-                 (p.Hs * p.Ws) % 256 == 0 && p.M == 4 * p.B * p.Hs * p.Ws && p.w_ps > 0 && p.Hin == p.Hs && p.Win == p.Ws,
-             "conv_gemm: phase form of an x2 conv on %d x %d", p.Hs, p.Ws);
+                 (p.up_phase == 1 ? hw % 256 == 0 : (p.up_phase == 2 && p.up_direct && hw % 32 == 0 && (p.B * hw) % 256 == 0 && !p.rowvec)) &&
+                 p.M == 4 * p.B * hw && p.w_ps > 0 && p.Hin == p.Hs && p.Win == p.Ws,
+             "conv_gemm: phase form %d of an x2 conv on %d x %d x %d", p.up_phase, p.B, p.Hs, p.Ws);
+    if (p.up_direct) {
+      const int64_t span = (int64_t)4 * hw * p.out_ld * 2 * (hw >= 256 ? 1 : 128 / hw + 1);
+      CD_CHECK((p.Hs & (p.Hs - 1)) == 0 && (p.Ws & (p.Ws - 1)) == 0 && p.act == ACT_NONE && !p.out_f32 && !p.resid && (p.N & 7) == 0 &&
+                   (p.out_ld & 7) == 0 && (((uintptr_t)p.out | (uintptr_t)p.rowvec) & 15) == 0 && span <= 0x7fffffffll &&
+                   (!p.rowvec || ((p.rowvec_ld & 3) == 0 && (p.rows_per_vec >= p.M || (p.rows_per_vec & 31) == 0))),
+               "conv_gemm: image-order store of a phase-form launch on %d x %d, N %d", p.Hs, p.Ws, p.N);
+    }
+  } else {
+    CD_CHECK(!p.up_direct, "conv_gemm: up_direct without up_phase");
+  }
   bool k64 = (p.C0 % 64 == 0) && (p.C1 % 64 == 0);
   if (p.ln_fold) CD_CHECK(p.tile == kLinStreamTile, "conv_gemm: a LayerNorm-folded layer runs on lin_stream only");
   int id = p.tile ? p.tile : tuned_config(st, p, k64);
@@ -1234,6 +1307,7 @@
     if (lin_stream_supports(pk)) ci = &kLinStreamCfg;
     else { CD_CHECK(!p.tile, "conv_gemm: lin_stream does not support this problem"); id = pick_config(p); }
   }
+  if (pk.up_direct && id != kLinStreamTile && cfg_lacks_tables(id, k64)) id = 13;
   for (int i = 0; i < kNumCfgs && !ci; ++i) if (kCfgs[i].id == id) ci = &kCfgs[i];
   CD_CHECK(ci, "conv_gemm: unknown tile configuration %d", id);
   if (p.act == ACT_GEGLU && (ci->TN % 64) != 0) { id = 2; ci = &kCfgs[1]; }
@@ -1247,6 +1321,7 @@
     li.splitk = pk.splitk > 1 ? pk.splitk : 1;
     li.chm = !lin && takes_channel_major(pk) ? 1 : 0;
     li.tile_group = lin ? 0 : pk.tile_group;
+    li.up_phase = pk.up_phase; li.up_direct = pk.up_direct;
     g_last_launch = li;
   }
   static const bool trace = [] { const char* e = getenv("CYCLEDIFF_GEMM_TRACE"); return e && e[0] == '1'; }();
diff --git a/cycle-diffusion_amd/csrc/engine.hip b/cycle-diffusion_amd/csrc/engine.hip
--- a/cycle-diffusion_amd/csrc/engine.hip
+++ b/cycle-diffusion_amd/csrc/engine.hip
@@ -277,11 +277,21 @@
   return y;
 }
 
+static bool up_phase_direct(const Act& x, int out_ld) {
+  if ((x.H & (x.H - 1)) != 0 || (x.W & (x.W - 1)) != 0) return false;
+  if ((int64_t)4 * x.H * x.W * out_ld * 2 * (x.H * x.W >= 256 ? 1 : 128 / (x.H * x.W) + 1) > 0x7fffffffll) return false;
+  const char* e = getenv("CYCLEDIFF_UP_PHASE_DIRECT");
+  return !(e && e[0] == '0');
+}
 bool conv_up_phase_taken(const Ctx& c, const ConvW& w, const Act& x, const Act* x2, const ConvOpts& o) {
   if (!o.up || c.f32 || x.split || x2 || !w.wphase || w.KH != 3 || w.KW != 3 || o.stride != 1 || o.pad != 1 || o.asym ||
       o.resid || o.out_f32 || o.ln_fold || w.geglu || o.act != ACT_NONE)
     return false;
-  if ((x.H * x.W) % 256 != 0 || w.N % 8 != 0 || (o.out && o.out_ld % 8 != 0)) return false;
+  if (w.N % 8 != 0 || (o.out && o.out_ld % 8 != 0)) return false;
+  const int hw = x.H * x.W;
+  if (hw % 256 != 0 &&
+      !(hw % 32 == 0 && (x.B * hw) % 256 == 0 && !o.rowvec && up_phase_direct(x, o.out ? o.out_ld : w.N)))
+    return false;
   const char* e = getenv("CYCLEDIFF_UP_PHASE");
   return !(e && e[0] == '0');
 }
@@ -304,10 +314,17 @@
   else if (!o.out && o.want_stats) y.stats_buf = (float*)c.arena->alloc((size_t)(p.M / 32) * 2 * w.N * sizeof(float));
   p.stats = y.stats_buf;
   y.stats = y.stats_buf;
+  p.zeros = c.zeros; p.tile = o.tile;
+  if (up_phase_direct(x, y.ld)) {
+    p.up_direct = 1;
+    if ((x.H * x.W) % 256 != 0) p.up_phase = 2;
+    p.out = y.p; p.out_ld = y.ld;
+    launch_conv_gemm(c.st, p);
+    return y;
+  }
   const size_t mk = c.arena->mark();
   bf16_t* tmp = (bf16_t*)c.arena->alloc((size_t)p.M * w.N * 2);
   p.out = tmp; p.out_ld = w.N;
-  p.zeros = c.zeros; p.tile = o.tile;
   launch_conv_gemm(c.st, p);
   launch_up_phase_reorder(c.st, tmp, y.p, x.B, x.H, x.W, w.N, y.ld);
   c.arena->release(mk);
diff --git a/cycle-diffusion_amd/csrc/kernels.h b/cycle-diffusion_amd/csrc/kernels.h
--- a/cycle-diffusion_amd/csrc/kernels.h
+++ b/cycle-diffusion_amd/csrc/kernels.h
@@ -142,6 +142,7 @@
   int dbg = 0;
   int up_phase = 0;
   int w_ps = 0;
+  int up_direct = 0;
 };
 constexpr int kProbeWords = 48;
 extern thread_local unsigned long long* g_conv_probe;
@@ -160,6 +161,8 @@
   int splitk = 1;
   int chm = 0;
   int tile_group = 0;
+  int up_phase = 0;
+  int up_direct = 0;
 };
 GemmLaunchInfo conv_gemm_last_launch();
 void launch_up_phase_weights(hipStream_t st, const bf16_t* w, bf16_t* out, int Npad, int Cpad);
diff --git a/cycle-diffusion_amd/csrc/nets_ho_vae.hip b/cycle-diffusion_amd/csrc/nets_ho_vae.hip
--- a/cycle-diffusion_amd/csrc/nets_ho_vae.hip
+++ b/cycle-diffusion_amd/csrc/nets_ho_vae.hip
@@ -214,7 +214,10 @@
       d_blk_[l].push_back(mk_rn(params, "decoder.up." + std::to_string(l) + ".block." + std::to_string(b), bin, bout));
       bin = bout;
     }
-    if (l != 0) d_up_[l] = mk_conv(params, "decoder.up." + std::to_string(l) + ".upsample.conv", bin, bin, 3);
+    if (l != 0) {
+      d_up_[l] = mk_conv(params, "decoder.up." + std::to_string(l) + ".upsample.conv", bin, bin, 3);
+      params.add_up_phase(d_up_[l]);
+    }
   }
   d_no_ = mk_gn(params, "decoder.norm_out", bin);
   d_out_ = mk_conv(params, "decoder.conv_out", out_ch_, bin, 3);
@@ -264,7 +267,10 @@
   h = rn_fwd(c, d_m2_, h, nullptr, nullptr, 0, true);
   for (int l = nlev_ - 1; l >= 0; --l) {
     for (auto& r : d_blk_[l]) h = rn_fwd(c, r, h, nullptr, nullptr, 0, true);
-    if (d_up_[l]) { ConvOpts ou; ou.up = true; ou.want_stats = true; h = conv_fwd(c, *d_up_[l], h, nullptr, ou); }
+    if (d_up_[l]) {
+      params.refresh_up_phase(c.st, d_up_[l]);
+      ConvOpts ou; ou.up = true; ou.want_stats = true; h = conv_fwd(c, *d_up_[l], h, nullptr, ou);
+    }
   }
   Act n = groupnorm_fwd(c, d_no_, h, nullptr, true);
   ConvOpts oo; oo.out_f32 = true; oo.out = img; oo.out_ld = out_ch_;
diff --git a/include/cyclediff.h b/include/cyclediff.h
--- a/include/cyclediff.h
+++ b/include/cyclediff.h
@@ -135,6 +135,7 @@
                     const float* bias, const float* rowvec, const float* resid, int act, int tile, float* y,
                     float* stats);
 int cd_op_last_gemm_config(cd_handle h, int* tile_id, int* bk, int* splitk, int* chm, int* tile_group);
+int cd_op_last_gemm_up_phase(cd_handle h, int* up_phase, int* up_direct);
 int cd_op_up_phase_reorder(cd_handle h, const float* x, int B, int C, int H, int W, float* y);
 int cd_op_groupnorm(cd_handle h, const float* x, int B, int C, int H, int W, int G, float eps,
                     const float* gamma, const float* beta, const float* film, int silu, float* y);
```

Measured after the change: 3.604 images/s (median of 6 runs). No clear change (+0.9%).
